# Skylarking/MARL

Hardware: AMD Instinct MI355X
Metric: env_steps_per_sec (higher is better)
Workload: dtype f32 (bf16x6 split products, fp32 accumulate)

## Files before the change

include/marl_hip.h:

```cpp
#ifndef MARL_HIP_H
#define MARL_HIP_H
#include <stddef.h>
#ifdef __cplusplus
extern "C" {
#endif

typedef struct {
  const float* p0; long ld0; int k0;
  const float* p1; long ld1; int k1;
  const int* idx; int nhot; int hot_w;
  int nid;
  const float* m0; long ldm0;
  long rpe0, bs0, off0;
  long rpei, bsi, offi;
  const int* emap0;
} marl_src_t;

typedef struct {
  int groups;
  long gs_x0, gs_x1, gs_w, gs_b, gs_y, gs_m0;
} marl_group_t;

typedef struct {
  const float *fc1_w, *fc1_b;
// ... 33 lines not shown
int marl_agent_unroll_bwd(const marl_agent_weights_t* w, const float* dq, const int* dq_idx,
                          const float* dq_val, const int* dq_idx2, const float* dq_val2, int dq_gdiv, const float* dhs,
                          const float* saved, const float* hs, float* dxp, float* dh0,
                          const marl_agent_grads_t* g, float* ws, size_t ws_bytes,
                          int B, int T, int N, int A, void* stream);

int marl_q_gather(const float* q, const int* idx, const float* avail, float mask_val, float* out,
                  long rows, int A, void* stream);
int marl_q_masked_max(const float* q, const float* avail, float mask_val, float* out_max, int* out_arg,
                      long rows, int A, void* stream);
int marl_q_double_select(const float* q_sel, const float* q_val, const float* avail, float mask_val,
                         float* out_val, int* out_arg, long rows, int A, void* stream);
int marl_q_scatter(float* dq, const int* idx1, const float* g1, const int* idx2, const float* g2,
                   long rows, int A, int gdiv, void* stream);
int marl_vec_add(const float* a, const float* b, float* out, long n, void* stream);
int marl_agent_sum(const float* in, long ld_in, float* out, long ld_out, long rows, int N, int D, void* stream);
int marl_agent_bcast(const float* in, long ld_in, float* out, long ld_out, long rows, int N, int D, int accumulate,
                     void* stream);

int marl_qmix_mix_fwd(const float* hy, long ldh, const float* b2, const float* w22, const float* b22, const float* q,
                      float* q_tot, long rows, int N, int E, void* stream);
int marl_qmix_mix_bwd(const float* hy, long ldh, const float* q, const float* dq_tot, const float* w22, float* dhy,
                      float* db2, float* dq, long rows, int N, int E, void* stream);
int marl_qmix_tail_fwd(const marl_src_t* s, long rows, int S, const float* Wb1, long ldb1, const float* bb1, const float* Wh,
                       long ldwh, const float* bh, float* hy, long ldhy, int c_b1, int c_h, void* stream);

typedef struct {
  const float *w1, *w1_b;
  const float *b1, *b1_b;
  const float *w2, *w2_b;
  const float *h, *h_b;
  const float *b2_w, *b2_b;
} marl_qmix_weights_t;
int marl_qmix_fused_supported(int N, int S, int E);
size_t marl_qmix_fused_workspace(long rows, int N, int S);
int marl_qmix_fused_fwd(const marl_qmix_weights_t* w, const marl_src_t* s, const float* q, float* q_tot,
                        long rows, int N, int S, int E, void* stream);
int marl_qmix_fused_bwd(const marl_qmix_weights_t* w, const marl_src_t* s, const float* q, const float* dq_tot,
                        float* dq, const marl_qmix_weights_t* grads, float* ws, size_t ws_bytes, long rows,
                        int N, int S, int E, void* stream);
int marl_qmix_fused_loss_bwd(const marl_qmix_weights_t* w, const marl_src_t* s, const float* q, const float* q_tot_tgt,
                             const float* r, const float* term, const float* padded, float gamma, float* q_tot,
                             float* dq, const marl_qmix_weights_t* grads, float* loss2, float* ws, size_t ws_bytes,
                             long rows, int N, int S, int E, void* stream);
int marl_qmix_fused_fwd_x6(const marl_qmix_weights_t* w, const marl_src_t* s, const float* q, float* q_tot,
                           long rows, int N, int S, int E, void* stream);
int marl_qmix_fused_bwd_x6(const marl_qmix_weights_t* w, const marl_src_t* s, const float* q, const float* dq_tot,
                           float* dq, const marl_qmix_weights_t* grads, float* ws, size_t ws_bytes, long rows,
                           int N, int S, int E, void* stream);
int marl_qmix_fused_loss_bwd_x6(const marl_qmix_weights_t* w, const marl_src_t* s, const float* q, const float* q_tot_tgt,
                                const float* r, const float* term, const float* padded, float gamma, float* q_tot,
                                float* dq, const marl_qmix_weights_t* grads, float* loss2, float* ws, size_t ws_bytes,
                                long rows, int N, int S, int E, void* stream);

int marl_qmix_wide_supported(int N, int S, int E);
const char* marl_qmix_wide_fwd_kernel(long rows, int N, int S, int flags);
size_t marl_qmix_wide_workspace(long rows, int N, int S, int backward);
int marl_qmix_wide_fwd(const marl_qmix_weights_t* w, const marl_src_t* s, const float* q, float* q_tot, float* ws,
                       size_t ws_bytes, long rows, int N, int S, int E, int flags, void* stream);
int marl_qmix_wide_bwd(const marl_qmix_weights_t* w, const marl_src_t* s, const float* q, const float* dq_tot, float* dq,
                       const marl_qmix_weights_t* grads, float* ws, size_t ws_bytes, long rows, int N, int S, int E,
                       int flags, void* stream);
int marl_qmix_wide_loss_bwd(const marl_qmix_weights_t* w, const marl_src_t* s, const float* q, const float* q_tot_tgt,
                            const float* r, const float* term, const float* padded, float gamma, float* q_tot, float* dq,
                            const marl_qmix_weights_t* grads, float* loss2, float* ws, size_t ws_bytes, long rows,
                            int N, int S, int E, int flags, void* stream);

typedef struct {
  const float *w1, *b1;
  const float *w2, *b2;
  const float *w3, *b3;
  long gs_w1, gs_b1, gs_w2, gs_b2, gs_w3, gs_b3;
} marl_mlp3_weights_t;
int marl_mlp3_supported(const marl_src_t* x, int K1, int H1, int H2, int N3, int groups);
int marl_mlp3_fwd(const marl_mlp3_weights_t* w, const marl_src_t* x, float* Y, long ldy, long gs_y,
                  long M, int K1, int N3, int groups, void* stream);
size_t marl_mlp3_bwd_workspace(long M, int K1, int N3, int groups);
int marl_mlp3_bwd(const marl_mlp3_weights_t* w, const marl_src_t* x, const float* dY, long lddy, long gs_dy,
                  const marl_mlp3_weights_t* grads, float* ws, size_t ws_bytes, long M, int K1, int N3,
                  int groups, void* stream);
size_t marl_mlp3_save_floats(long M, int three, int groups);
int marl_mlp3_needs_kept(const marl_src_t* x, int K1, int N3);
int marl_mlp3_fwd_save(const marl_mlp3_weights_t* w, const marl_src_t* x, float* Y, long ldy, long gs_y,
                       float* hsave, size_t hsave_floats, long M, int K1, int N3, int groups, void* stream);
int marl_mlp3_bwd_saved(const marl_mlp3_weights_t* w, const marl_src_t* x, const float* dY, long lddy, long gs_dy,
                        const marl_mlp3_weights_t* grads, float* ws, size_t ws_bytes, const float* hsave,
                        size_t hsave_floats, long M, int K1, int N3, int groups, void* stream);

int marl_agent_unroll_x6_supported(int B, int T, int N, int O, int A, int last_action, int reuse_network);
int marl_agent_unroll_x6_plain_r6(int B, int T, int N, int O, int A, int last_action, int reuse_network, int cu_budget);
int marl_agent_unroll_fwd_x6(const marl_agent_weights_t* w, const float* obs, long obs_bs, int obs_t0,
                             const int* ufed, long u_bs, int u_t0, const int* ep_len, const int* ep_map,
                             const float* h0, float* q, float* hs, float* h_last, float* saved, int B, int T, int N,
                             int O, int A, int last_action, int reuse_network, int cu_budget, float* gi_out,
                             const float* gi_in, void* stream);

#define MARL_UNROLL_SAVED 1
#define MARL_UNROLL_GI_OUT 2
#define MARL_UNROLL_GI_IN 4
#define MARL_UNROLL_HS 8
#define MARL_UNROLL_OBS_ALIGNED 16
#define MARL_UNROLL_H_ALIGNED 32
#define MARL_UNROLL_F32_PIPE 0
#define MARL_UNROLL_F32_MULTI 1
#define MARL_UNROLL_X6 2
#define MARL_UNROLL_X6_R6 3
#define MARL_UNROLL_IN_ELEMENT 0
#define MARL_UNROLL_IN_VECTOR 1
#define MARL_UNROLL_IN_HALF 2
#define MARL_UNROLL_IN_W2L 3
int marl_agent_unroll_fwd_plan(int x6, int B, int T, int N, int O, int A, int last_action, int reuse_network, int cu_budget,
                               int flags, int* plan);

int marl_agent_unroll_bwd_x6_supported(int B, int T, int N, int A, int sparse_dq);
size_t marl_agent_bwd_x6_workspace(int B, int N, int A);
int marl_agent_unroll_bwd_x6(const marl_agent_weights_t* w, const int* dq_idx, const float* dq_val, const int* dq_idx2,
                             const float* dq_val2, int dq_gdiv, const float* dhs, const float* saved, float* dxp, float* dh0,
                             const marl_agent_grads_t* g, float* ws, size_t ws_bytes, int B, int T, int N, int A, void* stream);

// ... 12 lines not shown
  const float *enc2_w, *enc2_b;
  const float* q0_w; long q0_ld; int q0_s;
  const float *q2_w, *q2_b;
  const float *q4_w, *q4_b;
} marl_qtran_weights_t;
int marl_qtran_supported(int N, int A, int AE);
int marl_qtran_head_fwd(const marl_qtran_weights_t* w, const float* hidden, const int* u, const float* sp, float* out,
                        float* s1, float* e2, float* y1, float* y2, long BT, int N, int A, int AE, void* stream);
int marl_qtran_head_fwd2(const marl_qtran_weights_t* w, const float* hidden, const int* u, const int* u2, const float* sp,
                         float* out, float* out2, float* s1, float* e2, float* y1, float* y2, long BT, int N, int A, int AE,
                         void* stream);
size_t marl_qtran_bwd_workspace(long BT, int AE);
int marl_qtran_head_bwd(const marl_qtran_weights_t* w, const float* hidden, const int* u, const float* d_out,
                        const float* y1, const float* y2, float* dy1, float* dy2, float* de2, float* dhidden,
                        int accumulate, float* d_enc0_w, float* d_enc0_b, float* d_enc2_b, float* ws, size_t ws_bytes,
                        long BT, int N, int A, int AE, void* stream);

int marl_qtran_state_parts_supported(int S);
int marl_qtran_state_parts(const marl_src_t* s, long BT, int S, int nsets, const float* W0, long ldw0, const float* b0, float* sp0,
                           const float* W1, long ldw1, const float* b1, float* sp1, void* stream);
int marl_qtran_wgrad_rows_supported(int S, int AE);
size_t marl_qtran_wgrad_rows_workspace(int S, int AE);
int marl_qtran_wgrad_rows(const marl_src_t* s, const float* s1, const float* e2, const float* y1, const float* y2,
                          const float* d_out, const float* dy1, const float* dy2, const float* de2, float* d_q0_w, long ld_q0,
                          float* d_q0_b, float* d_q2_w, float* d_q2_b, float* d_q4_w, float* d_q4_b, float* d_enc2_w, float* ws,
                          size_t ws_bytes, long BT, int S, int AE, void* stream);
#define MARL_QTRAN_PLAN_FWD 0
#define MARL_QTRAN_PLAN_FWD2 1
#define MARL_QTRAN_PLAN_BWD 2
#define MARL_QTRAN_PLAN_STATE_PARTS 3
#define MARL_QTRAN_PLAN_QMIX_TAIL 4
#define MARL_QTRAN_PLAN_WGRAD_ROWS 5
int marl_qtran_plan(int what, long BT, int N, int A, int AE, int S, int nsets, int* plan);

int marl_qplex_mix_fwd(const float* w_raw, const float* v, const float* q, const float* max_q,
                       const float* key, const float* ag, const float* ac, float* v_tot, float* a_tot,
                       float* lam_out, long rows, int N, int K, int weighted_head, int minus_one,
                       void* stream);
int marl_qplex_mix_bwd(const float* w_raw, const float* q, const float* max_q, const float* key,
                       const float* ag, const float* ac, const float* g, float* dq, float* dw_raw,
                       float* dv, float* dkey, float* dag, float* dac, long rows, int N, int K,
                       int weighted_head, int minus_one, void* stream);

int marl_first_terminated_len(const float* term, long ld, int E, int T, int* out, void* stream);

int marl_replay_gather(const long long* idx, int B, int T, int N, int A, const int* u_src, const float* r_src,
                       const float* term_src, const float* padded_src, const int* length_src, const int* won_src,
                       const float* avail_src, int* o_map, int* u, int* u_act, float* r, float* term, float* padded,
                       int* length, int* won, float* avail_next, float* avail_cur, void* stream);

int marl_td_loss(const float* q_tot, const float* q_tot_tgt, const float* r, const float* term,
                 const float* padded, float gamma, float* dq_tot, float* out2, float* ws, long rows,
                 void* stream);
int marl_qtran_loss(const float* jq, const float* jq_tgt, const float* v, const float* jq_hat,
                    const float* qsum_opt, const float* qsum_nopt, const float* r, const float* term,
                    const float* padded, float gamma, float lam_opt, float lam_nopt, float* d_jq,
                    float* d_v, float* d_qsum_opt, float* d_qsum_nopt, float* out4, float* ws, long rows,
                    void* stream);
size_t marl_loss_workspace(long rows);

int marl_qatten_supported(const marl_src_t* s, int N, int U, int H);
int marl_qatten_plan(long rows, int N, int U, int H, int* plan);
int marl_qatten_mix_fwd(const marl_src_t* s, const float* hy, long ldh, const float* q, float scale, float* q_tot,
                        long rows, int N, int U, int H, void* stream);
int marl_qatten_mix_bwd(const marl_src_t* s, const float* hy, long ldh, const float* q, float scale, const float* dq_tot,
                        float* dq, float* dhy, long lddh, long rows, int N, int U, int H, void* stream);
int marl_qatten_loss_bwd(const marl_src_t* s, const float* hy, long ldh, const float* q, float scale,
                         const float* q_tot_tgt, const float* r, const float* term, const float* padded, float gamma,
                         float* q_tot, float* dq, float* dhy, long lddh, float* dq_tot, float* out2, float* ws, long rows,
                         int N, int U, int H, void* stream);

int marl_lica_supported(int N, int A, int E);
int marl_lica_plan(long rows, int N, int A, int E, int* plan);
int marl_lica_mix_fwd(const float* hy, long ldh, const float* x, const int* u, float* q, long rows, int N, int A, int E,
                      void* stream);
int marl_lica_mix_bwd(const float* hy, long ldh, const float* x, const int* u, const float* dq, float* dhy, long lddh, float* dx,
                      long rows, int N, int A, int E, void* stream);
int marl_lica_loss_bwd(const float* hy, long ldh, const int* u, const float* q_tgt, const float* r, const float* term,
                       const float* padded, float gamma, float* q, float* dhy, long lddh, float* dq_tot, float* out2, float* ws,
                       long rows, int N, int A, int E, void* stream);

int marl_td_lambda_returns(const float* q_next_tot, const float* r, const float* term, const float* padded,
                           float gamma, float lambda, float* ret, int B, int T, void* stream);

int marl_iql_loss_bwd(const float* q, const int* u, const float* q_sel, const float* q_tgt, const float* avail_next,
                      const float* ret, const float* r, const float* term, const float* padded, float gamma, float mask_val,
                      float* dq_val, float* q_taken, float* q_next, float* out2, float* ws, int B, int T, int N, int A,
                      void* stream);
int marl_iql_select(const float* q, const int* u, const float* q_sel, const float* q_tgt, const float* avail_next,
                    const float* padded, float mask_val, float* q_taken, float* q_next_bnt, int B, int T, int N, int A,
                    void* stream);

int marl_policy_probs(const float* logits, const float* avail, float eps, float* pi, long rows, int A, void* stream);
int marl_policy_loss_bwd(const float* logits, const float* avail, const int* u, const float* G, const float* v,
                         const float* padded, float eps, float* dlogits, float* logp, float* out2, float* ws, long rows,
                         int N, int A, void* stream);
int marl_policy_loss_bwd_ex(const float* logits, const float* avail, const int* u, const float* G, const float* v,
                            const float* padded, float eps, float beta, float* dlogits, float* logp, float* ent, float* out3,
                            float* ws, long rows, int N, int A, void* stream);
int marl_policy_sample(const float* logits, const float* avail, long avail_es, const int* alive, float eps,
                       unsigned rseed, int env0, const int* tg, int tg0, int* act_out, long act_es,
                       int E, int N, int A, void* stream);

int marl_ppo_loss_bwd(const float* logits, const float* avail, const int* u, const float* adv, const float* logp_old,
                      const float* padded, float eps, float beta, float clip, float* dlogits, float* logp, float* ent,
                      float* out4, float* ws, long rows, int N, int A, void* stream);
int marl_masked_standardize(const float* x, const float* padded, float* out, float* stats3, float* ws, long rows, void* stream);

int marl_policy_probs_bwd(const float* logits, const float* avail, const float* gpi, const float* q_pi, const float* padded,
                          float eps, float beta, float* dlogits, float* ent, float* out3, float* ws, long rows, int N, int A,
                          void* stream);

int marl_coma_onehot_cols(const float* W, long ldw, int col0, float* Wt, int C, int D, void* stream);
int marl_coma_fc1_fwd(const float* pre_s, const float* Wt, const int* u, float* h1, int B, int T, int N, int A, int D,
                      void* stream);
size_t marl_coma_fc1_bwd_workspace(int B, int T, int N, int A, int D);
int marl_coma_fc1_bwd(const float* dh1, const float* h1, const int* u, float* dpre, float* dsum, float* dW, long lddw,
                      int col0, float* ws, size_t ws_bytes, int B, int T, int N, int A, int D, void* stream);
int marl_coma_q_taken(const float* q, const int* u, float* out, int shift, int B, int T, int N, int A, void* stream);
int marl_coma_loss_bwd(const float* logits, const float* avail, const float* q, const int* u, const float* G,
                       const float* padded, float eps, float beta, float* dlogits, float* dq, float* logp, float* ent,
                       float* adv, float* q_taken, float* out_c2, float* out_a3, float* ws, int B, int T, int N, int A,
                       void* stream);
// ... 187 lines not shown
```

marl_amd/algorithm/common.py:

```python
from __future__ import annotations

import copy
import numbers
import os
import warnings
import weakref

import numpy as np
import torch

from .. import ops, experiments
from ..hostutil import FlatParams, DeviceBatch, AsyncInt, Scratch, require_cuda
from ..network.mixer import x6_mode
from ..rollout import EpisodeBatch

MASK_BIG = -9999999.0
MASK_QTRAN_EVAL = -999999.0
N_STATS = 4


class FlatView:

    def __init__(self, flat, params, start):
        self.params = list(params)
        self.offsets = []
        off = 0
        for p in self.params:
            self.offsets.append(off)
            off += (p.numel() + 3) // 4 * 4
        self.n = off
        self.flat = flat[start:start + self.n]


class LearnerParams(FlatParams):

    def __init__(self, params, device):
        params = list(params)
        super().__init__(params, device, with_grad=False)
        self.gradx = torch.zeros(self.n + N_STATS, dtype=torch.float32, device=device)
        self.grad = self.gradx[:self.n]
        self.stats = self.gradx[self.n:]
        for p, off in zip(self.params, self.offsets):
            p.grad = self.grad[off:off + p.numel()].view(p.shape)

    def zero_grad(self):
        self.gradx.zero_()


class FusedOptimizer:

    def __init__(self, flat: LearnerParams, kind, lr, clip):
        if kind not in ("RMS", "Adam"):
            raise ValueError("optimizer {} not recognised.".format(kind))
        self.flat, self.kind, self.lr, self.clip = flat, kind, lr, clip
        dev = flat.flat.device
        self.s1 = torch.zeros(flat.n, device=dev)
        self.s2 = torch.zeros(flat.n, device=dev) if kind == "Adam" else None
        self.sumsq = torch.zeros(1, device=dev)
        self.t = 0
        self.param_groups = [{"params": flat.params, "lr": lr}]

    def zero_grad(self):
        self.flat.zero_grad()

    def step(self, den=None):
# ... 30 lines not shown
        for k, t in self._target_flats().items():
            sd[k] = t.detach().cpu().clone()
        return sd

    def load_resume_state(self, sd):
        if sd["alg"] != self.args.alg or sd["n_params"] != int(self._flat.n):
            raise ValueError("resume state of a different learner (%s, %d parameters)" % (sd["alg"], sd["n_params"]))
        self._flat.flat.copy_(sd["params"])
        for k, t in self._target_flats().items():
            t.copy_(sd[k])
        self.optimizer.load_state_dict(sd["optimizer"])
        self.sync_replicas()

    def save_resume(self, path):
        torch.save(self.resume_state(), path)

    def load_resume(self, path):
        self.load_resume_state(torch.load(path, map_location="cpu"))


class LossReadback:

    class Handle:
        __slots__ = ("buf", "event", "fn", "_v")

        def __init__(self, buf, event, fn):
            self.buf, self.event, self.fn, self._v = buf, event, fn, None

        def __float__(self):
            if self._v is None:
                self.event.synchronize()
                self._v = float(self.fn(self.buf))
            return self._v

    RING = 8

    def __init__(self, args):
        self.lazy = bool(getattr(args, "lazy_loss", False))
        self.slots, self.k = [], 0

    def read(self, stats, fn):
        if not self.lazy:
            return float(fn(stats.cpu()))
        if len(self.slots) < self.RING:
            self.slots.append(torch.empty(stats.numel(), dtype=stats.dtype).pin_memory())
        buf = self.slots[self.k % self.RING]
        self.k += 1
        buf.copy_(stats, non_blocking=True)
        ev = torch.cuda.Event()
        ev.record()
        return LossReadback.Handle(buf, ev, fn)


def td_lambda_of(args):
    lam = getattr(args, "td_lambda", None)
    if lam is None:
        return None
    if isinstance(lam, bool) or not isinstance(lam, numbers.Real) or not 0.0 <= lam <= 1.0:
        raise ValueError("td_lambda must be None or a number in [0, 1], got %r" % (lam,))
    return float(lam)


class Learner(ResumeMixin):
    _full_len_streak = 0
    n_stats, den_slot = 2, 1
    extra_nets = ()
    launch_ahead = True
    replay_graphs = True

    def _begin(self, mac, args, name):
        self.td_lambda = td_lambda_of(args)
        self._td_dbg = {}
        self.max_episode_len = args.episode_limit
        self.gamma = args.gamma
        self.lr = args.lr
        self.model_dir = args.model_dir + '/' + args.alg + '/' + args.map
        self.args = args
        self.device = require_cuda(name)

        self.eval_net = mac
        self.eval_net.cuda()
        self.target_net = copy.deepcopy(mac)

    def _ready(self, needs_avail):
        args = self.args
        self.optimizer = FusedOptimizer(self._flat, args.optimizer, self.lr, args.grad_norm_clip)
        self._buf = Scratch()
        self.reducer = GradReducer()
        self.pair = PairedUnroll(x6=x6_mode(args))
        self.loss_readback = LossReadback(args)
        self.graphs = GraphedUpdate.from_args(args) if self.replay_graphs else None
        self.needs_avail = needs_avail
        self.last_stats = None
        self.sync_replicas()

    def _update_targets(self):
        self.target_net.agent._flat.flat.copy_(self.eval_net.agent._flat.flat)
        if self.mixer is not None and self.mixer._flat.n:
            self.target_mixer._flat.flat.copy_(self.mixer._flat.flat)

    def _g(self, name, shape, dt=torch.float32):
        return self._buf.get(name, shape, self.device, dt)

    def _td_inputs(self, db, q_next_tot):
        lam = self.td_lambda = td_lambda_of(self.args)
        if lam is None:
            self._td_dbg = {}
            return db.r, self.gamma
        G = self._g("td_ret", (db.B * db.T,))
        ops.td_lambda_returns(q_next_tot, db.r, db.term, db.padded, self.gamma, lam, G, db.B, db.T)
        self._td_dbg = {"td_targets": G}
        return G, 0.0

    def get_max_episode_len(self, batch):
        T = DeviceBatch.first_terminated_len(torch.as_tensor(np.asarray(batch['terminated'])), self.args.episode_limit)
        for key in batch.keys():
            batch[key] = batch[key][:, :T]
        return batch, T

    def _device_batch(self, rec, index, small):
        term = (small if small is not None else rec).term
        if not (term.is_cuda and term.dtype == torch.float32 and term.shape[0] > 0) or self._full_len_streak < 2 \
                or not self.launch_ahead:
            db = DeviceBatch.from_record_auto(rec, self.args, reducer=self.reducer, index=index, small=small)
            full = db.T == min(rec.T, self.args.episode_limit)
            self._full_len_streak = self._full_len_streak + 1 if full else 0
            return db
        db, pending = DeviceBatch.from_record_begin(rec, self.args, reducer=self.reducer, index=index, small=small)
        self.max_episode_len = db.T
        self._forward_backward(db)
        T = pending()
        if T == db.T:
            return None
        self._full_len_streak = 0
        return DeviceBatch.from_record(rec, self.args, T=T, index=index, small=small)

    def train(self, batch, train_step):
        ring = batch.ring if isinstance(batch, EpisodeBatch) else None
        if self.graphs is not None and ring is not None and self.graphs.run(self, ring, batch.index):
            db = None
        elif isinstance(batch, DeviceBatch):
            db = batch
        elif ring is not None:
            prep = self.graphs.prepared if self.graphs is not None else None
            if prep is not None:
                self.graphs.prepared = None
                db = DeviceBatch.from_record(ring, self.args, T=prep[1], index=batch.index, small=prep[0])
            else:
                small = ring.select_small(batch.index, avail_cur=self.needs_avail)
                db = self._device_batch(ring, batch.index, small)
        elif isinstance(batch, EpisodeBatch) and batch.record is not None:
            db = self._device_batch(batch.record, None, None)
        else:
            T = None
            if self.reducer.enabled:
                T = DeviceBatch.first_terminated_len(torch.as_tensor(np.asarray(batch['terminated'])),
                                                     self.args.episode_limit, reducer=self.reducer)
            db = DeviceBatch.from_dict(batch, self.args, self.device, T=T)
        if db is not None:
            self.max_episode_len = db.T
            self._forward_backward(db)
        return self._finish_update(train_step)

    def _loss_fn(self):
        return lambda s: s[0] / s[1]

    def _finish_update(self, train_step):
        self.reducer.allreduce_(self._flat.gradx)
        stats = self._flat.stats
        self.optimizer.step(den=stats[self.den_slot:self.den_slot + 1])
        if train_step > 0 and train_step % self.args.target_update_cycle == 0:
            self._update_targets()
        self.last_stats = stats
        return self.loss_readback.read(stats[:self.n_stats], self._loss_fn())

    def _file_nets(self):
        return (("mixer",) if self.mixer is not None else ()) + self.extra_nets

    def save_models(self, train_step):
        num = str(train_step // self.args.save_cycle)
        if not os.path.exists(self.model_dir):
            os.makedirs(self.model_dir)
        self.eval_net.save_models(self.model_dir + '/' + num + '_rnn_net_params.pkl')
        for name in self._file_nets():
            torch.save({k: v.detach().cpu() for k, v in getattr(self, name).state_dict().items()},
                       self.model_dir + '/' + num + '_' + name + '_net_params.pkl')

    def load_models(self):
        paths = [self.model_dir + '/' + name + '_net_params.pkl' for name in ("rnn",) + self._file_nets()]
        if not os.path.exists(paths[0]):
            raise Exception("No model!")
        self.eval_net.load_models(paths[0])
        for name, path in zip(self._file_nets(), paths[1:]):
            getattr(self, name).load_state_dict(torch.load(path, map_location='cpu'))
        self.sync_replicas()
        print('Successfully load the model: ' + ' and '.join(paths))


def agent_backward(mac, db, which, saved, hs, dq, dhs, buf, dq_idx=None, dq_val=None, dq_idx2=None, dq_val2=None, dq_gdiv=1):
    args = mac.args
    B, T, N, A, O = db.B, db.T, db.N, db.A, db.O
    H = args.rnn_hidden_dim
    M = B * T * N
# ... 86 lines not shown
        with torch.cuda.stream(self.side):
            side()
        main()
        cur.wait_stream(self.side)

    def _step_us(self, rt):
        if self.x6:
            return 1.5 if rt <= 1 else 2.75 if rt <= 2 else 1.74 * rt
        return 3.3 if rt <= 1 else 1.3 + 2.1 * rt

    def chain_split(self, rows, T, obs_dim):
        if not self.chain or not self.applies(rows, T):
            return None
        if self.forced_split is not None:
            return (self.forced_split, 256 - self.forced_split) if self.forced_split > 0 else None
        tiles = (rows + 15) // 16
        cap = 8 if self.x6 else max(1, min(8, 2048 // (4 * max(obs_dim, 4))))
        ceil = lambda a, b: -(-a // b)
        plain = self._step_us(ceil(tiles, 128)) + 0.6 * self._step_us(ceil(tiles, 256))
        best = None
        for cu_a in (128, 144, 160, 176, 192):
            cu_b = 256 - cu_a
            rt_a, rt_b = ceil(tiles, cu_a), ceil(tiles, cu_b)
            if rt_a > cap or rt_b > cap:
                continue
            cost = max(1.6 * self._step_us(rt_a), self._step_us(rt_b))
            if best is None or cost < best[0]:
                best = (cost, cu_a, cu_b)
        if best is None or best[0] > 0.9 * plain:
            return None
        return best[1], best[2]

    def run_chain(self, rows, T, obs_dim, first, cont, second):
        split = self.chain_split(rows, T, obs_dim) if cont is not None else None
        if split is None:
            self.run(rows, T, first, second)
            if cont is not None:
                cont(256)
            return
        cu_a, cu_b = split
        self._fork(lambda: (first(cu_a), cont(cu_a)), lambda: second(cu_b))


class GraphedUpdate:

    WARMUP = 2
    AUTO_MAX_EPISODES = 1536

    def __init__(self, auto=False):
        self.entries = {}
        self.disabled = False
        self.auto = bool(auto)
        self.replays = 0

    @staticmethod
    def from_args(args):
        mode = getattr(args, "hip_graph", None)
        if mode is None or mode == "auto":
            return GraphedUpdate(auto=True)
        return GraphedUpdate() if mode else None

    SCHEDULE_ARGS = ("gemm_mode", "mixer_dtype", "mixer_wgrad_dtype", "double_q", "no_loss_fold", "lazy_loss", "gamma",
                     "two_hyper_layers", "last_action", "reuse_network", "td_lambda")

    @staticmethod
    def _schedule_key(args):
        return (experiments.generation,) + tuple(repr(getattr(args, k, None)) for k in GraphedUpdate.SCHEDULE_ARGS)

    def run(self, learner, ring, index):
        self.prepared = None
        if self.disabled:
            return False
        args = learner.args
        if self.auto and int(index.numel()) > self.AUTO_MAX_EPISODES:
            return False
        if ring.T != args.episode_limit or int(index.numel()) != int(args.batch_size):
            return False
        key = (id(ring), int(index.numel()), ring.T)
        e = self.entries.get(key)
        if e is not None and e["ring"]() is not ring:
            e = None
        dev = ring.obs.device
        if e is None:
            idx = index.to(device=dev, dtype=torch.long).clone()
            small = ring.select_small(idx, avail_cur=getattr(learner, "needs_avail", False))
            db = DeviceBatch.from_record(ring, args, T=min(ring.T, args.episode_limit), index=idx, small=small)
            fused = getattr(small, "avail_next", None) is not None and db.T == ring.T
            e = self.entries[key] = dict(ring=weakref.ref(ring), idx=idx, small=small, db=db, calls=0, graph=None, streak=0,
                                         fused=fused, avail_next=None if fused else db.avail_next.clone(),
                                         u_act=None if fused else db.u_act.clone())
            if not fused:
                db.avail_next, db.u_act = e["avail_next"], e["u_act"]
            e["T"] = db.T
        idx, small, db = e["idx"], e["small"], e["db"]
        idx.copy_(index)
        db.o_map.copy_(idx)
        ring.select_small(idx, out=small)
        if e["graph"] is not None and (e["ws_gen"] != ops.WS.gen or e["sched_key"] != self._schedule_key(args)):
            e["graph"], e["ws_keep"], e["calls"] = None, None, 0
        pending = None
        term = small.term
        if e["graph"] is not None and e["streak"] >= 2 and term.is_cuda and term.dtype == torch.float32 and term.shape[0] > 0:
            out = ops.first_terminated_len(term, args.episode_limit)
            r = learner.reducer
            if r is not None and r.enabled:
                r.dist.all_reduce(out, op=r.dist.ReduceOp.MAX, group=r.group)
            pending = AsyncInt(out)
            T = e["T"]
        else:
            T = DeviceBatch.first_terminated_len(term, args.episode_limit, reducer=learner.reducer)
            if T != e["T"]:
                e["streak"] = 0
                self.prepared = (small, T)
                return False
            e["streak"] += 1
        if not e["fused"]:
            torch.clamp(small.u[:, :T], min=0, out=e["u_act"])
            e["avail_next"].view(small.E, T, small.N, small.A).copy_(small.avail_next[:, :T] if small.avail is None else small.avail[:, 1:T + 1])
        if getattr(small, "avail_cur", None) is None:
            db.__dict__.pop("_avail", None)
# ... 32 lines not shown
```

marl_amd/algorithm/q_learner.py:

```python
from __future__ import annotations

import copy

import numpy as np
import torch

from .. import ops, experiments
from ..hostutil import flatten_module
from ..network.mixer import VDNMixer, QMixMixer, DMAQer, QattenMixer
from .common import MASK_BIG, LearnerParams, FlatView, Learner, agent_backward


class QLearner(Learner):
    def __init__(self, mac, args):
        self._begin(mac, args, "QLearner")
        if args.alg == 'vdn':
            self.mixer = VDNMixer(args)
        elif args.alg == 'qmix':
            self.mixer = QMixMixer(args)
        elif args.alg == 'qplex':
            self.mixer = DMAQer(args)
        elif args.alg == 'qatten':
            self.mixer = QattenMixer(args)
        else:
            raise ValueError("Mixer {} not recognised.".format(args.alg))
        self.target_mixer = copy.deepcopy(self.mixer)
        self.params = list(mac.parameters()) + list(self.mixer.parameters())
        self.cuda()
        self._ready(needs_avail=args.alg == 'qplex')

    def sync_replicas(self):
        o = self.optimizer
        self.reducer.broadcast_(self._flat.flat, self.target_net.agent._flat.flat,
                                self.target_mixer._flat.flat if self.target_mixer._flat.n else None, o.s1, o.s2)

    def cuda(self):
        dev = self.device
        self.mixer.to(dev)
        self.target_mixer.to(dev)
        self.eval_net.agent.to(dev)
        self._flat = LearnerParams(self.params, dev)
        self.eval_net.agent._flat = FlatView(self._flat.flat, self.eval_net.agent.parameters(), 0)
        self.mixer._flat = FlatView(self._flat.flat, self.mixer.parameters(), self.eval_net.agent._flat.n)
        self.eval_net._dev = dev
        self.target_net._dev = dev
        self.target_net.agent.to(dev)
        flatten_module(self.target_net.agent, dev)
        flatten_module(self.target_mixer, dev)

    def _unrolls(self, db, keep_hs=False):
        a, g = self.args, self._g
        B, T, N, A, H = db.B, db.T, db.N, db.A, a.rnn_hidden_dim
        q_evals, saved = g("q_evals", (B, T, N, A)), g("saved", ops.saved_shape(T, B, N))
        h_last, h_scr = g("h_last", (B * N, H)), g("h_scr", (B * N, H))
        q_tgt, q_en = g("q_tgt", (B, T, N, A)), g("q_en", (B, T, N, A))
        hs = hs_en = hs_tgt = None
        if keep_hs:
            hs, hs_tgt = g("hs", (B, T, N, H)), g("hs_tgt", (B, T, N, H))
            hs_en = g("hs_en", (B, T, N, H)) if a.double_q else None
        (oc, oc_bs, oc_t0), (on, on_bs, on_t0) = db.o_cur, db.o_next

        emap = getattr(db, 'o_map', None)
        cont, gi = None, None
        if a.double_q:
            shifted = on is oc and on_bs == oc_bs and on_t0 == oc_t0 + 1
            split = self.pair.chain_split(B * N, T, a.obs_shape)
            if shifted and ((self.eval_net.unroll_x6(B, T, oc) and experiments.get("fwd_xs") != 0) or
                            ops.agent_unroll_reuse_supported(B, T, N, a.obs_shape, A, split[0] if split else 256)):
                gi = g("gi", ops.saved_shape(T, B, N, planes=3))
            cont = lambda cu: self.eval_net.unroll(on, on_bs, on_t0, db.u_fed, db.u_bs, 0, B, T, q_en, hs_en, h_scr, None, h0=h_last,
                                                   ep_len=db.ep_len, ep_map=emap, cu_budget=cu, gi_in=gi)
        self.pair.run_chain(B * N, T, a.obs_shape,
                            lambda cu: self.eval_net.unroll(oc, oc_bs, oc_t0, db.u_fed, db.u_bs, -1, B, T, q_evals, hs, h_last, saved,
                                                            h0=None, ep_len=db.ep_len, ep_map=emap, cu_budget=cu, gi_out=gi),
                            cont,
                            lambda cu: self.target_net.unroll(on, on_bs, on_t0, db.u_fed, db.u_bs, 0, B, T, q_tgt, hs_tgt, None, None,
                                                              h0=None, ep_len=db.ep_len, ep_map=emap, cu_budget=cu))
        return q_evals, q_en, q_tgt, saved, (hs, hs_en, hs_tgt)

    def _select(self, db, q_evals, q_en, q_tgt):
        R, A, g = db.B * db.T * db.N, db.A, self._g
        q_chosen, q_tgt_chosen = g("q_chosen", (R,)), g("q_tgt_chosen", (R,))
        ops.q_gather(q_evals, db.u_act.reshape(-1), q_chosen, R, A)
        cur_max = None
        if self.args.double_q:
            cur_max = g("cur_max", (R,), torch.int32)
            ops.q_double_select(q_en, q_tgt, db.avail_next, MASK_BIG, q_tgt_chosen, cur_max, R, A)
        else:
            ops.q_masked_max(q_tgt, db.avail_next, MASK_BIG, q_tgt_chosen, None, R, A)
        return q_chosen, q_tgt_chosen, cur_max

    def _mix(self, db, q_evals, q_tgt, q_chosen, q_tgt_chosen, cur_max):
        a, g = self.args, self._g
        N, BT, A = db.N, db.B * db.T, db.A
        R = BT * N
        ctx, fold = {}, False
        qc, qtc = q_chosen.view(BT, N), q_tgt_chosen.view(BT, N)
        if a.alg == 'qplex':
            max_q = g("max_q", (R,))
            ops.q_masked_max(q_evals, db.avail, MASK_BIG, max_q, None, R, A)
            v_tot, a_tot = self.mixer.hip_forward(qc, db.s, BT, u_idx=db.u_taken.reshape(-1), max_q=max_q.view(BT, N), ctx=ctx)
            q_tot = g("q_tot", (BT,))
            ops.vec_add(v_tot, a_tot, q_tot, BT)
            if a.double_q:
                tgt_max = g("tgt_max", (R,))
                ops.q_masked_max(q_tgt, db.avail_next, MASK_BIG, tgt_max, None, R, A)
                vt, at = self.target_mixer.hip_forward(qtc, db.s_next, BT, u_idx=cur_max, max_q=tgt_max.view(BT, N), tag="t")
                q_tot_tgt = g("q_tot_tgt", (BT,))
                ops.vec_add(vt, at, q_tot_tgt, BT)
            else:
                q_tot_tgt, _ = self.target_mixer.hip_forward(qtc, db.s_next, BT, tag="t")
        else:
            fold = a.alg in ('qmix', 'qatten') and getattr(self.mixer, "loss_backward_fused", None) is not None and \
                self.mixer.loss_backward_fused(db.s) and not getattr(a, "no_loss_fold", False)
            q_tot = g("q_tot", (BT,)) if fold else self.mixer.hip_forward(qc, db.s, BT, ctx=ctx)
            q_tot_tgt = self.target_mixer.hip_forward(qtc, db.s_next, BT, tag="t")
        return q_tot, q_tot_tgt, ctx, fold

    def _loss_backward(self, db, q_chosen, q_tot, q_tot_tgt, ctx, fold):
        BT = db.B * db.T
        r, gamma = self._td_inputs(db, q_tot_tgt)
        if fold:
            return self.mixer.hip_loss_backward(q_chosen.view(BT, db.N), db.s, BT, q_tot_tgt, r, db.term, db.padded, gamma,
                                                self._flat.stats[:2], q_tot=q_tot)
        dq_tot = self._g("dq_tot", (BT,))
        ops.td_loss(q_tot, q_tot_tgt, r, db.term, db.padded, gamma, dq_tot, self._flat.stats[:2], BT)
        return self.mixer.hip_backward(ctx, dq_tot, BT)

    def _forward_backward(self, db):
        q_evals, q_en, q_tgt, saved, _ = self._unrolls(db)
        q_chosen, q_tgt_chosen, cur_max = self._select(db, q_evals, q_en, q_tgt)
        q_tot, q_tot_tgt, ctx, fold = self._mix(db, q_evals, q_tgt, q_chosen, q_tgt_chosen, cur_max)
        self._flat.zero_grad()
        dq_chosen = self._loss_backward(db, q_chosen, q_tot, q_tot_tgt, ctx, fold)
        agent_backward(self.eval_net, db, "cur", saved, None, None, None, self._buf,
                       dq_idx=db.u_act.reshape(-1), dq_val=dq_chosen.reshape(-1).contiguous())
        self._dbg = dict(q_evals=q_evals, q_targets=q_tgt, q_tot=q_tot, q_tot_target=q_tot_tgt, **self._td_dbg)

    def get_q_and_q_tot_table(self):
        one = {'o': np.ones((1, 1, 2, 1)), 's': np.ones((1, 1, 1)), 'o_next': np.ones((1, 1, 2, 1)),
               'u_onehot': np.zeros((1, 1, 2, 3)), 'avail_u': np.ones((1, 1, 2, 3))}
        self.eval_net.init_hidden(1)
        q_values, _ = self.eval_net.get_current_q_values(one, 1)
        qv = q_values.cpu()
        q_table_i, q_table_j = qv[0, 0, 0].numpy(), qv[0, 0, 1].numpy()
        q_tot_table = np.zeros((3, 3))
        s = torch.ones(1, 1, 1)
        for i in range(3):
            for j in range(3):
                chosen = torch.stack((qv[:, :, 0, i], qv[:, :, 1, j]), dim=1).view(1, 1, 2)
                if self.args.alg == 'qplex':
                    v_tot = self.mixer(chosen, s, is_v=True)
                    onehot = torch.zeros(1, 1, 2, 3)
                    onehot[0, 0, 0, i] = 1
                    onehot[0, 0, 1, j] = 1
                    a_tot = self.mixer(chosen, s, actions=onehot, max_q_i=qv.max(dim=3)[0], is_v=False)
                    q_tot_table[i, j] = float(v_tot.item() + a_tot.item())
                else:
                    q_tot_table[i, j] = self.mixer(chosen, s).item()
        return q_tot_table, q_table_i, q_table_j
```

marl_amd/common/replaybuffer.py:

```python
from __future__ import annotations

import threading

import numpy as np
import torch

from ..env.synthetic_smac import EpisodeRecord
from ..rollout import EpisodeBatch
from ..hostutil import h2d_async


class ReplayBuffer:
    def __init__(self, args):
        self.args = args
        self.n_actions = args.n_actions
        self.n_agents = args.n_agents
        self.state_shape = args.state_shape
        self.obs_shape = args.obs_shape
        self.size = args.buffer_size
        self.episode_limit = args.episode_limit
        self.current_idx = 0
        self.current_size = 0
        self.buffers = None
        self.record = None
# ... 16 lines not shown

    def next_slot_record(self, E, T, N, O, S, A, device):
        if self.buffers is not None:
            return None
        with self.lock:
            i0 = self._peek_contiguous(E)
            if i0 is None:
                return None
            if self.record is None:
                self.record = EpisodeRecord(self.size, T, N, O, S, A, device)
            r = self.record
            if (r.T, r.N, r.O, r.S, r.A) != (T, N, O, S, A):
                return None
            view = r.slice(i0, i0 + E)
            view.sink_slot = i0
            return view

    def store_episode(self, episode_batch):
        rec = getattr(episode_batch, "record", None)
        batch_size = rec.E if rec is not None else episode_batch['o'].shape[0]
        with self.lock:
            idxs = self._get_storage_idx(inc=batch_size)
            if rec is not None and self.buffers is None:
                if self.record is None:
                    self.record = EpisodeRecord(self.size, rec.T, rec.N, rec.O, rec.S, rec.A, rec.obs.device)
                first = int(np.atleast_1d(idxs)[0])
                if rec.obs.data_ptr() == self.record.obs[first].data_ptr() and getattr(rec, "sink_slot", -1) == first:
                    return
                if getattr(rec, "sink_slot", None) is not None:
                    rec = rec.clone()
                idx_t = torch.as_tensor(np.atleast_1d(idxs), dtype=torch.long, device=rec.obs.device)
                rec.copy_into(self.record, idx_t)
                return
            if self.record is not None:
                raise ValueError("this ReplayBuffer holds device records; store EpisodeBatch objects")
            if self.buffers is None:
                self._alloc_host()
            src = episode_batch.numpy() if isinstance(episode_batch, EpisodeBatch) else episode_batch
            for k in self.buffers:
                v = src[k]
                self.buffers[k][idxs] = v.cpu().numpy() if isinstance(v, torch.Tensor) else v

    def sample(self, batch_size, exclude=None):
        if exclude is not None and exclude[0] < self.current_size:
            lo, cnt = int(exclude[0]), int(min(exclude[1], self.current_size - exclude[0]))
            if self.current_size - cnt <= 0:
                raise ValueError("every stored episode is being overwritten: nothing to sample")
            idx = np.random.randint(0, self.current_size - cnt, batch_size)
            idx = np.where(idx >= lo, idx + cnt, idx)
        else:
            idx = np.random.randint(0, self.current_size, batch_size)
        if self.record is not None:
            idx_t = h2d_async(idx, self.record.obs.device, torch.long)
            return EpisodeBatch(ring=self.record, index=idx_t)
        return {k: self.buffers[k][idx] for k in self.buffers}

    def _get_storage_idx(self, inc=None):
        inc = inc or 1
        if self.current_idx + inc <= self.size:
            idx = np.arange(self.current_idx, self.current_idx + inc)
            self.current_idx += inc
        elif self.current_idx < self.size:
            overflow = inc - (self.size - self.current_idx)
            idx = np.concatenate([np.arange(self.current_idx, self.size), np.arange(0, overflow)])
            self.current_idx = overflow
        else:
            idx = np.arange(0, inc)
            self.current_idx = inc
        self.current_size = min(self.size, self.current_size + inc)
        if inc == 1:
            idx = idx[0]
        return idx
```

marl_amd/csrc/mixers.hip:

```cpp
#include "common.h"
#include "sums.h"
#include "row_tile.h"
#include "../../include/marl_hip.h"

namespace {
namespace rt = row_tile;

constexpr int TPB = 256;
static_assert(TPB == SUMS_TPB, "the loss kernels launch sums.h's workgroup size");
inline int nblk(long n, int cap = 65535 * 16) {
  long b = (n + TPB - 1) / TPB;
  if (b > cap) b = cap;
  if (b < 1) b = 1;
  return (int)b;
}

__global__ void q_gather_kernel(const float* q, const int* idx, const float* avail, float mask_val, float* out,
                                long rows, int A) {
  for (long r = (long)blockIdx.x * TPB + threadIdx.x; r < rows; r += (long)gridDim.x * TPB) {
    const int a = idx[r];
    float v = 0.f;
    if (a >= 0) v = (avail && avail[r * A + a] == 0.f) ? mask_val : q[r * A + a];
    out[r] = v;
  }
// ... 318 lines not shown
    tile_in(ags, ag + r0 * KN, nr * KN, (long)QR * KN);
    tile_in(acs, ac + r0 * KN, nr * KN, (long)QR * KN);
    tile_in(keys, key + r0 * K, nr * K, (long)QR * K);
    for (int e = threadIdx.x; e < nr * N; e += TPB) {
      const int rl = e / N;
      const long gi = r0 * N + e;
      const float gr = g[r0 + rl];
      const float wr = w_raw[gi];
      const float w = fabsf(wr) + 1e-10f;
      const float qi = q[gi];
      dq[gi] = weighted ? gr * w : gr;
      dw_raw[gi] = weighted ? gr * qi * (wr > 0.f ? 1.f : (wr < 0.f ? -1.f : 0.f)) : 0.f;
      dv[gi] = weighted ? gr : 0.f;
      const float mi = max_q[gi];
      float adv;
      {
#pragma clang fp contract(off)
        adv = weighted ? (w * qi - w * mi) : (qi - mi);
      }
      dls[e] = gr * adv;
    }
    __syncthreads();
    for (int e = threadIdx.x; e < nr * K; e += TPB) {
      const int rl = e / K;
      const float kr = keys[e];
      const float kk = fabsf(kr) + 1e-10f;
      const float sg = kr > 0.f ? 1.f : (kr < 0.f ? -1.f : 0.f);
      float dk = 0.f;
      for (int i = 0; i < N; ++i) {
        const float dlam = dls[rl * N + i];
        const float sa = sigmoidf_(ags[e * N + i]);
        const float sc = sigmoidf_(acs[e * N + i]);
        dk += dlam * sa * sc * sg;
        ags[e * N + i] = dlam * kk * sc * sa * (1.f - sa);
        acs[e * N + i] = dlam * kk * sa * sc * (1.f - sc);
      }
      keys[e] = dk;
    }
    __syncthreads();
    tile_out(dag + r0 * KN, ags, nr * KN);
    tile_out(dac + r0 * KN, acs, nr * KN);
    tile_out(dkey + r0 * K, keys, nr * K);
    __syncthreads();
  }
}

inline int qplex_tile_rows(int N, int K, const void* a, const void* b, const void* c) {
  if (!aligned16(a) || !aligned16(b) || !aligned16(c)) return 0;
  for (int qr = 128; qr >= 32; qr >>= 1)
    if ((size_t)qr * (2 * K * N + K + 2 * N) * 4 <= 64 * 1024) return qr;
  return 0;
}

__global__ void td_loss_kernel(const float* q_tot, const float* q_tgt, const float* r, const float* term,
                               const float* padded, float gamma, float* dq_tot, float* ws, long rows) {
  float acc[2] = {0.f, 0.f};
  for (long i = (long)blockIdx.x * TPB + threadIdx.x; i < rows; i += (long)gridDim.x * TPB) {
    const float mask = 1.f - padded[i];
    const float target = r[i] + gamma * q_tgt[i] * (1.f - term[i]);
    const float td = target - q_tot[i];
    const float mtd = mask * td;
    acc[0] += mtd * mtd;
    acc[1] += mask;
    dq_tot[i] = -2.f * mask * mtd;
  }
  block_partials<2>(acc, ws);
}

__global__ void qtran_loss_kernel(const float* jq, const float* jq_tgt, const float* v, const float* jq_hat,
                                  const float* qs_opt, const float* qs_nopt, const float* r, const float* term,
                                  const float* padded, float gamma, float lam_opt, float lam_nopt, float* d_jq,
                                  float* d_v, float* d_qs_opt, float* d_qs_nopt, float* ws, long rows) {
  float acc[4] = {0.f, 0.f, 0.f, 0.f};
  for (long i = (long)blockIdx.x * TPB + threadIdx.x; i < rows; i += (long)gridDim.x * TPB) {
    const float mask = 1.f - padded[i];
    const float y = r[i] + gamma * jq_tgt[i] * (1.f - term[i]);
    const float td = (jq[i] - y) * mask;
    const float opt = (qs_opt[i] - jq_hat[i] + v[i]) * mask;
    float nraw = qs_nopt[i] - jq[i] + v[i];
    nraw = nraw < 0.f ? nraw : 0.f;
    const float nopt = nraw * mask;
    acc[0] += td * td; acc[1] += opt * opt; acc[2] += nopt * nopt; acc[3] += mask;
    d_jq[i] = 2.f * mask * td;
    const float go = lam_opt * 2.f * mask * opt, gn = lam_nopt * 2.f * mask * nopt;
    d_v[i] = go + gn;
    d_qs_opt[i] = go;
    d_qs_nopt[i] = gn;
  }
  block_partials<4>(acc, ws);
}

}

extern "C" int marl_q_gather(const float* q, const int* idx, const float* avail, float mask_val, float* out,
                             long rows, int A, void* stream) {
  if (rows <= 0) return 0;
  hipLaunchKernelGGL(q_gather_kernel, dim3(nblk(rows)), dim3(TPB), 0, (hipStream_t)stream, q, idx, avail, mask_val,
                     out, rows, A);
  MARL_CHECK_LAUNCH();
  return 0;
}

extern "C" int marl_q_masked_max(const float* q, const float* avail, float mask_val, float* out_max, int* out_arg,
                                 long rows, int A, void* stream) {
  if (rows <= 0) return 0;
  const rt::Plan pl = rt::plan(rows, A, 2, 64 * 1024, 2048, {q, avail});
  if (pl.tiled && pl.vec && rows >= 4096) {
    hipLaunchKernelGGL(q_masked_max_tiled_kernel, dim3((unsigned)pl.blocks), dim3(256), pl.lds_bytes, (hipStream_t)stream, q, avail,
                       mask_val, out_max, out_arg, rows, A);
    MARL_CHECK_LAUNCH();
    return 0;
  }
  hipLaunchKernelGGL(q_masked_max_kernel, dim3(nblk(rows)), dim3(TPB), 0, (hipStream_t)stream, q, avail, mask_val,
                     out_max, out_arg, rows, A);
  MARL_CHECK_LAUNCH();
  return 0;
}
// ... 163 lines not shown
  for (int i = blockIdx.y * 1024 + threadIdx.x; i < TNA && i < (blockIdx.y + 1) * 1024; i += TPB) ao[i] = av[i];
  if (a.avail_cur) {
    const int NA = a.N * a.A;
    const long live = (long)a.length_src[e] * NA;
    const float* ac = av - NA;
    float* co = a.avail_cur + (long)b * TNA;
    for (int i = blockIdx.y * 1024 + threadIdx.x; i < TNA && i < (blockIdx.y + 1) * 1024; i += TPB) co[i] = i < live ? ac[i] : 0.f;
  }
  if (blockIdx.y != 0) return;
  const int TN = a.T * a.N;
  for (int i = threadIdx.x; i < TN; i += TPB) {
    const int v = a.u_src[e * TN + i];
    a.u[(long)b * TN + i] = v;
    a.u_act[(long)b * TN + i] = v < 0 ? 0 : v;
  }
  for (int i = threadIdx.x; i < a.T; i += TPB) {
    a.r[(long)b * a.T + i] = a.r_src[e * a.T + i];
    a.term[(long)b * a.T + i] = a.term_src[e * a.T + i];
    a.padded[(long)b * a.T + i] = a.padded_src[e * a.T + i];
  }
  if (threadIdx.x == 0) {
    a.o_map[b] = (int)e;
    a.length[b] = a.length_src[e];
    a.won[b] = a.won_src[e];
  }
}
}

extern "C" int marl_replay_gather(const long long* idx, int B, int T, int N, int A, const int* u_src, const float* r_src,
                                  const float* term_src, const float* padded_src, const int* length_src,
                                  const int* won_src, const float* avail_src, int* o_map, int* u, int* u_act, float* r,
                                  float* term, float* padded, int* length, int* won, float* avail_next, float* avail_cur,
                                  void* stream) {
  if (B <= 0 || T <= 0) return 0;
  GatherArgs a;
  a.idx = idx; a.u_src = u_src; a.length_src = length_src; a.won_src = won_src;
  a.r_src = r_src; a.term_src = term_src; a.padded_src = padded_src; a.avail_src = avail_src;
  a.o_map = o_map; a.u = u; a.u_act = u_act; a.length = length; a.won = won;
  a.r = r; a.term = term; a.padded = padded; a.avail_next = avail_next; a.avail_cur = avail_cur;
  a.B = B; a.T = T; a.N = N; a.A = A;
  const int chunks = (T * N * A + 1023) / 1024;
  hipLaunchKernelGGL(replay_gather_kernel, dim3((unsigned)B, (unsigned)(chunks > 0 ? chunks : 1)), dim3(TPB), 0, (hipStream_t)stream, a);
  MARL_CHECK_LAUNCH();
  return 0;
}

extern "C" size_t marl_loss_workspace(long rows) { return (size_t)rt::PARTIAL_ROWS * 4 * sizeof(float); }

extern "C" int marl_td_loss(const float* q_tot, const float* q_tot_tgt, const float* r, const float* term,
                            const float* padded, float gamma, float* dq_tot, float* out2, float* ws, long rows,
                            void* stream) {
  if (rows <= 0) return 0;
  const int nb = rt::partial_blocks(rows);
  hipLaunchKernelGGL(td_loss_kernel, dim3(nb), dim3(TPB), 0, (hipStream_t)stream, q_tot, q_tot_tgt, r, term, padded,
                     gamma, dq_tot, ws, rows);
  MARL_CHECK_LAUNCH();
  hipLaunchKernelGGL(finish_sums_kernel, dim3(1), dim3(TPB), 0, (hipStream_t)stream, (const float*)ws, nb, 2, out2);
  MARL_CHECK_LAUNCH();
  return 0;
}

extern "C" int marl_qtran_loss(const float* jq, const float* jq_tgt, const float* v, const float* jq_hat,
                               const float* qsum_opt, const float* qsum_nopt, const float* r, const float* term,
                               const float* padded, float gamma, float lam_opt, float lam_nopt, float* d_jq,
                               float* d_v, float* d_qsum_opt, float* d_qsum_nopt, float* out4, float* ws, long rows,
                               void* stream) {
  if (rows <= 0) return 0;
  const int nb = rt::partial_blocks(rows);
  hipLaunchKernelGGL(qtran_loss_kernel, dim3(nb), dim3(TPB), 0, (hipStream_t)stream, jq, jq_tgt, v, jq_hat, qsum_opt,
                     qsum_nopt, r, term, padded, gamma, lam_opt, lam_nopt, d_jq, d_v, d_qsum_opt, d_qsum_nopt, ws,
                     rows);
  MARL_CHECK_LAUNCH();
  hipLaunchKernelGGL(finish_sums_kernel, dim3(1), dim3(TPB), 0, (hipStream_t)stream, (const float*)ws, nb, 4, out4);
  MARL_CHECK_LAUNCH();
  return 0;
}
```

marl_amd/csrc/qatten.hip:

```cpp
#include "common.h"
#include "sums.h"
#include "row_tile.h"
#include "../../include/marl_hip.h"

#pragma clang fp contract(off)

namespace {
namespace rt = row_tile;

constexpr int TPB = SUMS_TPB;
constexpr int MAXN = 16, MAXU = 64, MAXH = 8;
constexpr int MAX_TILE = 64;
constexpr size_t LDS_CAP = 76 * 1024;

enum { MODE_FWD = 0, MODE_BWD = 1, MODE_LOSS = 2 };

struct Tile { int TR, SP, HP; size_t lds; };
inline Tile tile_of(int N, int U, int H) {
  Tile t;
  t.SP = (N * U) | 1;
  t.HP = (H * U + H + 1) | 1;
  const size_t row = (size_t)(2 + t.SP + t.HP + N + H * N + H + N + 1) * sizeof(float);
  long tr = (long)(LDS_CAP / row);
  if (tr > MAX_TILE) tr = MAX_TILE;
  if (tr > TPB / H) tr = TPB / H;
  t.TR = (int)(tr < 1 ? 1 : tr);
  t.lds = row * t.TR;
  return t;
}

struct QaArgs {
  ConcatSrc s;
  const float* hy; long ldh;
  const float* q;
  float scale;
  const float* g_in;
  const float *q_tgt, *r, *term, *padded;
  float gamma;
  float* q_tot;
  float* dq;
  float* dhy; long lddh;
  float* dq_tot;
  float* ws;
  long rows;
  int N, U, H, TR, SP, HP;
};

struct Chunk { int lo, cnt; bool vec; };
__device__ __forceinline__ Chunk chunk_of(const float* g, int n, int j) {
  int head = (int)((4 - ((reinterpret_cast<uintptr_t>(g) >> 2) & 3)) & 3);
  head = head < n ? head : n;
  Chunk c;
  c.lo = j ? head + 4 * (j - 1) : 0;
  c.cnt = j ? (n - c.lo < 4 ? n - c.lo : 4) : head;
  if (c.cnt < 0) c.cnt = 0;
  c.vec = j && c.cnt == 4;
  return c;
}
__device__ __forceinline__ int chunks_of(int n) { return 1 + (n + 3) / 4; }

template <class F>
__device__ __forceinline__ void tile_in(float* lds, int pitch, const float* base, F off_of, int n, int nr) {
  const int CH = chunks_of(n), items = nr * CH;
  for (int it0 = threadIdx.x; it0 < items; it0 += 4 * TPB) {
    f32x4 v[4];
    Chunk c[4];
    int at[4];
#pragma unroll
    for (int u = 0; u < 4; ++u) {
      const int it = it0 + u * TPB;
      c[u].cnt = 0; c[u].lo = 0; c[u].vec = false; at[u] = 0;
      v[u] = (f32x4){0.f, 0.f, 0.f, 0.f};
      if (it < items) {
        const int rl = it / CH, j = it - rl * CH;
        const long off = off_of(rl);
        const float* g = base + (off < 0 ? 0 : off);
        c[u] = chunk_of(g, n, j);
        at[u] = rl * pitch + c[u].lo;
        if (off >= 0) {
          if (c[u].vec) v[u] = *reinterpret_cast<const f32x4*>(g + c[u].lo);
          else
#pragma unroll
            for (int e = 0; e < 4; ++e) if (e < c[u].cnt) v[u][e] = g[c[u].lo + e];
        }
      }
    }
#pragma unroll
    for (int u = 0; u < 4; ++u)
#pragma unroll
      for (int e = 0; e < 4; ++e) if (e < c[u].cnt) lds[at[u] + e] = v[u][e];
  }
}
__device__ __forceinline__ void tile_out(float* g0, long ld, const float* lds, int pitch, int n, int nr) {
  const int CH = chunks_of(n), items = nr * CH;
  for (int it = threadIdx.x; it < items; it += TPB) {
    const int rl = it / CH, j = it - rl * CH;
    float* g = g0 + rl * ld;
    const Chunk c = chunk_of(g, n, j);
    const float* d = lds + rl * pitch + c.lo;
    if (c.vec) *reinterpret_cast<f32x4*>(g + c.lo) = (f32x4){d[0], d[1], d[2], d[3]};
    else
      for (int e = 0; e < c.cnt; ++e) g[c.lo + e] = d[e];
  }
}

__device__ __forceinline__ float head_fwd(const float* p, const float* u, const float* q, float scale, int N, int U, float (&lam)[MAXN]) {
#pragma unroll
  for (int i = 0; i < MAXN; ++i) lam[i] = 0.f;
#pragma unroll 4
  for (int k = 0; k < U; ++k) {
    const float pk = p[k];
#pragma unroll
    for (int i = 0; i < MAXN; ++i)
      if (i < N) lam[i] += pk * u[i * U + k];
  }
  float mx = 0.f;
#pragma unroll
  for (int i = 0; i < MAXN; ++i)
    if (i < N) {
      lam[i] = scale * lam[i];
      mx = (i == 0 || lam[i] > mx) ? lam[i] : mx;
    }
  float sum = 0.f;
#pragma unroll
  for (int i = 0; i < MAXN; ++i)
    if (i < N) { lam[i] = expf(lam[i] - mx); sum += lam[i]; }
  float y = 0.f;
#pragma unroll
  for (int i = 0; i < MAXN; ++i)
    if (i < N) { lam[i] = lam[i] / sum; y += lam[i] * q[i]; }
  return y;
}

__device__ __forceinline__ float head_bwd(float* p, const float* u, const float* q, float scale, int N, int U, float g, float w, float y,
                                          float (&lam)[MAXN]) {
  const float ga = g * fabsf(w);
#pragma unroll
  for (int i = 0; i < MAXN; ++i)
    if (i < N) lam[i] = ga * lam[i] * (q[i] - y);
#pragma unroll 4
  for (int k = 0; k < U; ++k) {
    float d = 0.f;
#pragma unroll
    for (int i = 0; i < MAXN; ++i)
      if (i < N) d += lam[i] * u[i * U + k];
    p[k] = scale * d;
  }
  return g * y * (w > 0.f ? 1.f : (w < 0.f ? -1.f : 0.f));
}

template <int MODE>
__global__ __launch_bounds__(TPB) void qatten_kernel(QaArgs a) {
  extern __shared__ __attribute__((aligned(16))) float qa_smem[];
  const int N = a.N, U = a.U, H = a.H, TR = a.TR, SP = a.SP, HP = a.HP;
  const int NU = N * U, HU = H * U;
  long* Ro = reinterpret_cast<long*>(qa_smem);
  float* Ss = qa_smem + 2 * TR;
  float* Hs = Ss + (size_t)TR * SP;
  float* Qs = Hs + (size_t)TR * HP;
  float* WL = Qs + TR * N;
  float* Ys = WL + TR * H * N;
  float* Dq = Ys + TR * H;
  float* Gs = Dq + TR * N;
  const int tid = threadIdx.x;
  float acc[2] = {0.f, 0.f};
  for (long r0 = (long)blockIdx.x * TR; r0 < a.rows; r0 += (long)gridDim.x * TR) {
    const int nr = (int)(a.rows - r0 < TR ? a.rows - r0 : TR);
    for (int rl = tid; rl < nr; rl += TPB) {
      const ConcatRow cr = concat_row(a.s, r0 + rl);
      Ro[rl] = cr.ok0 ? cr.r0 * a.s.ld0 : -1;
    }
    __syncthreads();
    tile_in(Ss, SP, a.s.p0, [&](int rl) { return Ro[rl]; }, NU, nr);
    tile_in(Hs, HP, a.hy + r0 * a.ldh, [&](int rl) { return rl * a.ldh; }, HU + H + 1, nr);
    for (int e = tid; e < nr * N; e += TPB) Qs[e] = a.q[r0 * N + e];
    __syncthreads();
    const bool act = tid < nr * H;
    const int rl = tid / H, h = tid - rl * H;
    float lam[MAXN];
    float y = 0.f, w = 0.f;
    if (act) {
      y = head_fwd(Hs + rl * HP + h * U, Ss + rl * SP, Qs + rl * N, a.scale, N, U, lam);
      w = Hs[rl * HP + HU + h];
      Ys[tid] = y;
      if (MODE != MODE_FWD) {
        const float aw = fabsf(w);
#pragma unroll
        for (int i = 0; i < MAXN; ++i)
          if (i < N) WL[tid * N + i] = aw * lam[i];
      }
    }
    __syncthreads();
    if (tid < nr) {
      const long r = r0 + tid;
      float g = 0.f;
      if (MODE != MODE_BWD) {
        float qt = 0.f;
        for (int hh = 0; hh < H; ++hh) qt += fabsf(Hs[tid * HP + HU + hh]) * Ys[tid * H + hh];
        qt += Hs[tid * HP + HU + H];
        if (a.q_tot) a.q_tot[r] = qt;
        if (MODE == MODE_LOSS) {
#pragma clang fp contract(fast)
          const float mask = 1.f - a.padded[r];
          const float target = a.r[r] + a.gamma * a.q_tgt[r] * (1.f - a.term[r]);
          const float td = target - qt;
          const float mtd = mask * td;
          acc[0] += mtd * mtd;
          acc[1] += mask;
          g = -2.f * mask * mtd;
          a.dq_tot[r] = g;
        }
      } else {
        g = a.g_in[r];
      }
      if (MODE != MODE_FWD) Gs[tid] = g;
    }
    if (MODE != MODE_FWD) {
      __syncthreads();
      if (act) Hs[rl * HP + HU + h] = head_bwd(Hs + rl * HP + h * U, Ss + rl * SP, Qs + rl * N, a.scale, N, U, Gs[rl], w, y, lam);
      for (int e = tid; e < nr * N; e += TPB) {
        const int row = e / N, i = e - row * N;
        float ai = 0.f;
        for (int hh = 0; hh < H; ++hh) ai += WL[(row * H + hh) * N + i];
        Dq[e] = Gs[row] * ai;
      }
      __syncthreads();
      tile_out(a.dhy + r0 * a.lddh, a.lddh, Hs, HP, HU + H, nr);
      for (int e = tid; e < nr * N; e += TPB) a.dq[r0 * N + e] = Dq[e];
    }
    __syncthreads();
  }
  if (MODE == MODE_LOSS) block_partials<2>(acc, a.ws);
}

inline bool shape_ok(int N, int U, int H) { return N >= 1 && N <= MAXN && U >= 1 && U <= MAXU && H >= 1 && H <= MAXH; }
inline bool src_ok(const marl_src_t* s, int N, int U) {
  return s && s->p0 && s->k0 >= N * U && s->ld0 >= N * U && !s->k1 && !s->nhot && !s->nid && !s->m0 && s->rpe0 >= 0 &&
         (!s->emap0 || s->rpe0 > 0) && (reinterpret_cast<uintptr_t>(s->p0) & 3) == 0;
}
inline ConcatSrc state_src(const marl_src_t* s) {
  ConcatSrc c = {};
  c.p0 = s->p0; c.ld0 = s->ld0; c.k0 = s->k0;
  c.rpe0 = s->rpe0; c.bs0 = s->bs0; c.off0 = s->off0;
  c.fd0 = make_fastdiv((unsigned)(s->rpe0 > 0 ? s->rpe0 : 1));
  c.fdi = make_fastdiv(1); c.fdn = make_fastdiv(1);
  c.emap0 = s->emap0;
  return c;
}
inline int grid_of(long rows, int TR) {
  const long t = (rows + TR - 1) / TR;
  return (int)(t > rt::PARTIAL_ROWS ? rt::PARTIAL_ROWS : t);
}

template <int MODE>
int launch(QaArgs& a, const marl_src_t* s, hipStream_t stream) {
  if (!shape_ok(a.N, a.U, a.H) || !src_ok(s, a.N, a.U) || a.rows >= (1L << 31) || !a.hy || !a.q || a.ldh < a.H * a.U + a.H + 1)
    return (int)hipErrorInvalidValue;
  if (MODE != MODE_FWD && (!a.dq || !a.dhy || a.lddh < a.H * a.U + a.H)) return (int)hipErrorInvalidValue;
  const Tile t = tile_of(a.N, a.U, a.H);
  a.s = state_src(s);
  a.TR = t.TR; a.SP = t.SP; a.HP = t.HP;
  const void* fn = (const void*)qatten_kernel<MODE>;
  hipError_t e = hipFuncSetAttribute(fn, hipFuncAttributeMaxDynamicSharedMemorySize, (int)t.lds);
  if (e != hipSuccess) return (int)e;
  void* kargs[] = {(void*)&a};
  e = hipLaunchKernel(fn, dim3((unsigned)grid_of(a.rows, t.TR)), dim3(TPB), kargs, t.lds, stream);
  if (e != hipSuccess) return (int)e;
  MARL_CHECK_LAUNCH();
  return 0;
}

}

extern "C" int marl_qatten_supported(const marl_src_t* s, int N, int U, int H) { return shape_ok(N, U, H) && src_ok(s, N, U) ? 1 : 0; }

extern "C" int marl_qatten_plan(long rows, int N, int U, int H, int* plan) {
  if (!shape_ok(N, U, H) || rows >= (1L << 31)) return (int)hipErrorInvalidValue;
  for (int i = 0; i < 4; ++i) plan[i] = 0;
  if (rows <= 0) return 0;
  const Tile t = tile_of(N, U, H);
  plan[0] = t.TR;
  plan[1] = grid_of(rows, t.TR);
  plan[2] = (int)t.lds;
  const long tiles = (rows + t.TR - 1) / t.TR;
  plan[3] = (int)((tiles + plan[1] - 1) / plan[1]);
  return 0;
}

extern "C" int marl_qatten_mix_fwd(const marl_src_t* s, const float* hy, long ldh, const float* q, float scale, float* q_tot,
                                   long rows, int N, int U, int H, void* stream) {
  if (rows <= 0) return 0;
  if (!q_tot) return (int)hipErrorInvalidValue;
  QaArgs a = {};
  a.hy = hy; a.ldh = ldh; a.q = q; a.scale = scale; a.q_tot = q_tot; a.rows = rows; a.N = N; a.U = U; a.H = H;
  return launch<MODE_FWD>(a, s, (hipStream_t)stream);
}

extern "C" int marl_qatten_mix_bwd(const marl_src_t* s, const float* hy, long ldh, const float* q, float scale, const float* dq_tot,
                                   float* dq, float* dhy, long lddh, long rows, int N, int U, int H, void* stream) {
  if (rows <= 0) return 0;
  if (!dq_tot) return (int)hipErrorInvalidValue;
  QaArgs a = {};
  a.hy = hy; a.ldh = ldh; a.q = q; a.scale = scale; a.g_in = dq_tot; a.dq = dq; a.dhy = dhy; a.lddh = lddh;
  a.rows = rows; a.N = N; a.U = U; a.H = H;
  return launch<MODE_BWD>(a, s, (hipStream_t)stream);
}

extern "C" int marl_qatten_loss_bwd(const marl_src_t* s, const float* hy, long ldh, const float* q, float scale,
                                    const float* q_tot_tgt, const float* r, const float* term, const float* padded, float gamma,
                                    float* q_tot, float* dq, float* dhy, long lddh, float* dq_tot, float* out2, float* ws, long rows,
                                    int N, int U, int H, void* stream) {
  if (rows <= 0) return 0;
  if (!q_tot_tgt || !r || !term || !padded || !dq_tot || !out2 || !ws) return (int)hipErrorInvalidValue;
  QaArgs a = {};
  a.hy = hy; a.ldh = ldh; a.q = q; a.scale = scale; a.q_tgt = q_tot_tgt; a.r = r; a.term = term; a.padded = padded; a.gamma = gamma;
  a.q_tot = q_tot; a.dq = dq; a.dhy = dhy; a.lddh = lddh; a.dq_tot = dq_tot; a.ws = ws;
  a.rows = rows; a.N = N; a.U = U; a.H = H;
  const int rc = launch<MODE_LOSS>(a, s, (hipStream_t)stream);
  if (rc) return rc;
  hipLaunchKernelGGL(finish_sums_kernel, dim3(1), dim3(TPB), 0, (hipStream_t)stream, (const float*)ws, grid_of(rows, a.TR), 2, out2);
  MARL_CHECK_LAUNCH();
  return 0;
}
```

marl_amd/csrc/qmix_fused.hip:

```cpp
#include "x6.h"
#include "../../include/marl_hip.h"

namespace {

constexpr int E = 32;
constexpr int KCQ = 8;
constexpr int SS = 128 + 4;
constexpr int NAG = 5;
constexpr int PP = 136;

struct QmixArgs {
  const float *W[4], *Bv[4];
  const float *wb2, *bb2;
  ConcatSrc s;
  const float* q;
  const float* g;
  float* q_tot;
  float* dq;
  float* ws;
  const float *lr, *lterm, *lpadded, *lq_tgt;
  float gamma;
  long rows;
  int N, S, C;
};

__host__ __device__ inline long qmix_slab_floats(int C, int S) { return (long)C * (S + 1) + (E + 1) + 2; }

template <int CTRL>
__device__ __forceinline__ float dpp(float v) {
  return __builtin_bit_cast(float, __builtin_amdgcn_update_dpp(0, __builtin_bit_cast(int, v), CTRL, 0xf, 0xf, true));
}
constexpr int DPP_XOR1 = 0xB1, DPP_XOR2 = 0x4E;
constexpr int DPP_HALF_MIRROR = 0x141, DPP_MIRROR = 0x140;
constexpr int DPP_ROR4 = 0x124, DPP_ROR8 = 0x128;
template <int EW>
__device__ __forceinline__ float group_sum(float v) {
  if (EW == 4) v += dpp<DPP_ROR4>(v);
  v += dpp<DPP_ROR8>(v);
  return v;
}
template <int EW>
__device__ __forceinline__ float e_sum(float v) {
  v += dpp<DPP_XOR1>(v);
  v += dpp<DPP_XOR2>(v);
  if (EW == 8) v += dpp<DPP_HALF_MIRROR>(v);
  return v;
}
__device__ __forceinline__ float row_sum(float v) {
  v += dpp<DPP_XOR1>(v);
  v += dpp<DPP_XOR2>(v);
  v += dpp<DPP_HALF_MIRROR>(v);
  v += dpp<DPP_MIRROR>(v);
  return v;
}
__device__ __forceinline__ float sign_clamp(float x, float lo) { return __builtin_amdgcn_fmed3f(x * 0x1p126f, lo, 1.0f); }

template <bool BWD, int NW, bool LOSS = false, bool X6 = false>
__global__ __launch_bounds__(64 * NW, 2) void qmix_fused_kernel(QmixArgs a) {
  static_assert(!LOSS || BWD, "the loss is folded into the backward kernel");
  static_assert(!X6 || NW == 8, "the split variant runs eight waves (two column tiles per wave: 96 registers of pre-split weights)");
  constexpr int QNT = 64 * NW, EW = 32 / NW, GPT = 16 / EW, TPW = 8 / GPT, LT = TPW - 1;
  constexpr int SRAW = X6 ? 2 * 3 * 16 * PP * 2 : 2 * 16 * SS * 4;
  __shared__ __attribute__((aligned(16))) char Sraw[SRAW];
  float (*Ss)[16 * SS] = reinterpret_cast<float (*)[16 * SS]>(Sraw);
  short* const Sp = reinterpret_cast<short*>(Sraw);
  constexpr int PLN = 16 * PP, PBUF = 3 * PLN;
  constexpr int KR = (X6 && BWD) ? (LOSS ? 2 : 3) : 4;
  constexpr int KL = 4 - KR;
  __shared__ __attribute__((aligned(16))) i32x4 WL[KL ? NW * TPW * KL * 3 * 64 : 1];
  __shared__ __attribute__((aligned(16))) float Qt2[2][8][16];
  __shared__ __attribute__((aligned(16))) float QT[NW][16];
  __shared__ __attribute__((aligned(16))) float DQP[NW][NAG][16];
  __shared__ __attribute__((aligned(16))) float Gs2[2][16];
  __shared__ __attribute__((aligned(16))) float Ls2[2][4][16];
  const int tid = threadIdx.x, lane = tid & 63, wave = tid >> 6;
  const int q4 = lane >> 4, m = lane & 15;
  const int el = m & (EW - 1), gl = m / EW, e = EW * wave + el;
  const int N = a.N, S = a.S, C = a.C, NE = N * E;
  const bool ones = S < 128;

  f32x4 wq[X6 ? 1 : TPW][X6 ? 1 : KCQ];
  F3 wq6[X6 ? TPW : 1][X6 ? KR : 1];
  float bias[TPW];
  int grp[TPW];
#pragma unroll
  for (int c = 0; c < TPW; ++c) {
    const int g = GPT * c + gl;
    grp[c] = g;
    const float *Wp = nullptr, *Bp = nullptr;
    if (g < NAG) { if (g < N) { Wp = a.W[0] + (long)(g * E + e) * S; Bp = a.Bv[0] + g * E + e; } }
    else { Wp = a.W[g - NAG + 1] + (long)e * S; Bp = a.Bv[g - NAG + 1] + e; }
    bias[c] = Bp ? *Bp : 0.f;
    if (X6) {
#pragma unroll
      for (int kc = 0; kc < 4; ++kc) {
        float v[8];
#pragma unroll
        for (int jj = 0; jj < 8; ++jj) {
          const int kk = 32 * kc + 8 * q4 + jj;
          v[jj] = (Wp && kk < S) ? Wp[kk] : 0.f;
        }
        const F3 f = split8((f32x4){v[0], v[1], v[2], v[3]}, (f32x4){v[4], v[5], v[6], v[7]});
        if (kc < KR) wq6[c][kc < KR ? kc : 0] = f;
        else { i32x4* wl = WL + (((wave * TPW + c) * (KL ? KL : 1) + (kc - KR)) * 3) * 64 + lane; wl[0] = f.h; wl[64] = f.m; wl[128] = f.l; }
      }
    } else {
#pragma unroll
      for (int kc = 0; kc < KCQ; ++kc)
#pragma unroll
        for (int i = 0; i < 4; ++i) {
          const int kk = 16 * kc + 4 * q4 + i;
          wq[c][kc][i] = (Wp && kk < S) ? Wp[kk] : 0.f;
// ... 41 lines not shown
  const FastDiv fd = a.s.fd0;
  const int* emap = a.s.emap0;
  const float* sp0 = a.s.p0 + (fc4 < S ? fc4 : 0);
  const long ld = a.s.ld0, blk = (long)a.s.bs0 * a.s.ld0;
  auto map_one = [&](int tile, int i, int& pe, int& pw) {
    unsigned row = (unsigned)tile * 16u + (unsigned)(fr + (QNT / 32) * i);
    row = row < last_row ? row : last_row;
    const unsigned ep = rpe ? fastdiv(row, fd) : 0u;
    pw = (int)(row - ep * rpe) + roff;
    pe = (int)ep;
    if (emap) pe = emap[ep];
  };
  auto map_issue = [&](int tile) {
    map_one(tile, 0, pe0, pw0);
    if (NPF > 1) map_one(tile, 1, pe1, pw1);
  };
  auto fetch_one = [&](int pe, int pw) {
    f32x4 v = *reinterpret_cast<const f32x4*>(sp0 + ((long)pe * blk + (long)pw * ld));
    if (BWD) {
#pragma unroll
      for (int j = 0; j < 4; ++j) v[j] = (ones_lane && j == ones_j) ? 1.f : v[j];
    }
    return v;
  };
  auto fetch = [&](int) {
    pf[0] = fetch_one(pe0, pw0);
    if (NPF > 1) pf[NPF - 1] = fetch_one(pe1, pw1);
  };
  auto stash = [&](int buf) {
#pragma unroll
    for (int i = 0; i < NPF; ++i) {
      if (X6) {
        const F3h f = split4(pf[i]);
        short* p = Sp + buf * PBUF + (fr + (QNT / 32) * i) * PP + fc4;
        *reinterpret_cast<i32x2*>(p) = f.h;
        *reinterpret_cast<i32x2*>(p + PLN) = f.m;
        *reinterpret_cast<i32x2*>(p + 2 * PLN) = f.l;
      } else *reinterpret_cast<f32x4*>(&Ss[buf][(fr + (QNT / 32) * i) * SS + fc4]) = pf[i];
    }
  };
  float pq = 0.f, pg = 0.f, pl[4] = {0.f, 0.f, 0.f, 0.f};
  const int qr = tid / N, qn = tid - qr * N;
  auto fetch_qg = [&](int tile) {
    pq = 0.f; pg = 0.f;
    if (tid < 16 * N) {
      const int row = tile * 16 + qr;
      if (row < nrows) pq = a.q[(unsigned)(row * N + qn)];
    }
    if (BWD && tid >= 192 && tid < 208) {
      const int row = tile * 16 + (tid - 192);
      if (LOSS) {
        pl[0] = pl[1] = pl[3] = 0.f; pl[2] = 1.f;
        if (row < nrows) { pl[0] = a.lr[row]; pl[1] = a.lterm[row]; pl[2] = a.lpadded[row]; pl[3] = a.lq_tgt[row]; }
      } else if (row < nrows) pg = a.g[row];
    }
  };
  auto flush_dq = [&](int prow0) {
    if (tid < 16 * N) {
      float v = 0.f;
#pragma unroll
      for (int w = 0; w < NW; ++w) v += DQP[w][qn][qr];
      if (prow0 + qr < nrows) a.dq[(unsigned)((prow0 + qr) * N + qn)] = v;
    }
  };
  int tile = blockIdx.x;
  if (tile < tiles) {
    map_issue(tile); fetch(tile); fetch_qg(tile);
    if (tile + (int)gridDim.x < tiles) map_issue(tile + gridDim.x);
    stash(0);
  }
  int buf = 0;
  int prow0 = -1;
  ST_DECL(8);
  __syncthreads();
  for (; tile < tiles; tile += gridDim.x, buf ^= 1) {
    const int row0 = tile * 16;
    if (tid < 16 * N) Qt2[buf][qn][qr] = pq;
    if (BWD && tid >= 192 && tid < 208) {
      if (LOSS) {
#pragma unroll
        for (int k = 0; k < 4; ++k) Ls2[buf][k][tid - 192] = pl[k];
      } else Gs2[buf][tid - 192] = pg;
    }
    const int nt = tile + gridDim.x;
    if (nt < tiles) {
      fetch(nt); fetch_qg(nt);
      if (nt + (int)gridDim.x < tiles) map_issue(nt + gridDim.x);
    }
    ST_MARK(0);
    WG_BARRIER();
    ST_MARK(1);
    if (BWD && prow0 >= 0) flush_dq(prow0);
    f32x4 acc[TPW];
#pragma unroll
    for (int c = 0; c < TPW; ++c) acc[c] = (f32x4){bias[c], bias[c], bias[c], bias[c]};
    if (X6) {
      f32x4 accb[TPW];
#pragma unroll
      for (int c = 0; c < TPW; ++c) accb[c] = (f32x4){0.f, 0.f, 0.f, 0.f};
      const short* sp = Sp + buf * PBUF + m * PP + 8 * q4;
#pragma unroll
      for (int kc = 0; kc < 4; ++kc) {
        F3 xa;
        xa.h = *reinterpret_cast<const i32x4*>(sp + 32 * kc);
        xa.m = *reinterpret_cast<const i32x4*>(sp + PLN + 32 * kc);
        xa.l = *reinterpret_cast<const i32x4*>(sp + 2 * PLN + 32 * kc);
        F3 wk[TPW];
#pragma unroll
        for (int c = 0; c < TPW; ++c) {
          if (kc < KR) wk[c] = wq6[c][kc < KR ? kc : 0];
          else { const i32x4* wl = WL + (((wave * TPW + c) * (KL ? KL : 1) + (kc - KR)) * 3) * 64 + lane; wk[c].h = wl[0]; wk[c].m = wl[64]; wk[c].l = wl[128]; }
        }
#define OP(p_, q_) _Pragma("unroll") for (int c = 0; c < TPW; ++c) { if (kc & 1) accb[c] = mm(xa.p_, wk[c].q_, accb[c]); else acc[c] = mm(xa.p_, wk[c].q_, acc[c]); }
        OP(m, m) OP(h, l) OP(l, h) OP(h, m) OP(m, h) OP(h, h)
#undef OP
      }
#pragma unroll
      for (int c = 0; c < TPW; ++c) acc[c] += accb[c];
    } else {
      const float* sr = &Ss[buf][m * SS + 4 * q4];
#pragma unroll
      for (int kc = 0; kc < KCQ; ++kc) {
        const f32x4 a4 = *reinterpret_cast<const f32x4*>(sr + 16 * kc);
#pragma unroll
        for (int i = 0; i < 4; ++i)
#pragma unroll
          for (int c = 0; c < TPW; ++c) acc[c] = mfma16(a4[i], wq[c][kc][i], acc[c]);
      }
    }
    ST_MARK(2);
    __builtin_amdgcn_sched_barrier(0);
    f32x4 qv[TPW];
    f32x4 p = {0.f, 0.f, 0.f, 0.f};
#pragma unroll
    for (int c = 0; c <= MT; ++c) {
      qv[c] = *reinterpret_cast<const f32x4*>(&Qt2[buf][grp[c]][4 * q4]);
#pragma unroll
      for (int i = 0; i < 4; ++i) {
        const float av = acc[c][i];
        const float x = c < MT ? fabsf(av) : __builtin_bit_cast(float, __builtin_bit_cast(unsigned, av) & absmask);
        p[i] = c == 0 ? x * qv[c][i] : fmaf(x, qv[c][i], p[i]);
      }
    }
    f32x4 ex, hid, t4;
#pragma unroll
    for (int i = 0; i < 4; ++i) {
      p[i] = group_sum<EW>(p[i]);
      ex[i] = __expf(p[i]);
      hid[i] = p[i] > 0.f ? p[i] : ex[i] - 1.f;
      const float z = is6 ? fabsf(acc[LT][i]) : fmaxf(acc[LT][i], 0.f);
      t4[i] = row_sum(z * (is6 ? hid[i] : cw));
    }
    if (m == 0) *reinterpret_cast<f32x4*>(&QT[wave][4 * q4]) = t4;
    ST_MARK(3);
    WG_BARRIER();
    ST_MARK(4);
    if (!BWD) {
      if (tid < 16) {
        float tot = 0.f;
#pragma unroll
        for (int w = 0; w < NW; ++w) tot += QT[w][tid];
        if (row0 + tid < nrows) a.q_tot[row0 + tid] = tot + bb2;
      }
      ST_MARK(5);
    } else {
      f32x4 qt = *reinterpret_cast<const f32x4*>(&QT[0][4 * q4]);
#pragma unroll
      for (int w = 1; w < NW; ++w) qt += *reinterpret_cast<const f32x4*>(&QT[w][4 * q4]);
      f32x4 gr;
      if (LOSS) {
        const f32x4 lr = *reinterpret_cast<const f32x4*>(&Ls2[buf][0][4 * q4]);
        const f32x4 lt = *reinterpret_cast<const f32x4*>(&Ls2[buf][1][4 * q4]);
        const f32x4 lp = *reinterpret_cast<const f32x4*>(&Ls2[buf][2][4 * q4]);
        const f32x4 lq = *reinterpret_cast<const f32x4*>(&Ls2[buf][3][4 * q4]);
#pragma unroll
        for (int i = 0; i < 4; ++i) {
          qt[i] += bb2;
          const float mask = 1.f - lp[i];
          const float target = lr[i] + a.gamma * lq[i] * (1.f - lt[i]);
          const float mtd = mask * (target - qt[i]);
          gr[i] = -2.f * mask * mtd;
          acc_ln += mtd * mtd; acc_lm += mask;
        }
        if (a.q_tot && wave == 0 && m == 0) {
          if (row0 + 16 <= nrows) *reinterpret_cast<f32x4*>(&a.q_tot[row0 + 4 * q4]) = qt;
          else {
#pragma unroll
            for (int i = 0; i < 4; ++i) if (row0 + 4 * q4 + i < nrows) a.q_tot[row0 + 4 * q4 + i] = qt[i];
          }
        }
      } else gr = *reinterpret_cast<const f32x4*>(&Gs2[buf][4 * q4]);
      f32x4 dpre, dhy[TPW];
#pragma unroll
      for (int i = 0; i < 4; ++i) {
        const float w2 = group_sum<EW>(is6 ? fabsf(acc[LT][i]) : 0.f);
        dpre[i] = gr[i] * w2 * (p[i] > 0.f ? 1.f : ex[i]);
        acc_wb2 += gr[i] * fmaxf(acc[LT][i], 0.f);
        acc_bb2 += gr[i];
      }
#pragma unroll
      for (int c = 0; c < TPW; ++c) {
        const bool lo_all = GPT * c + GPT - 1 <= NAG, hi_all = GPT * c > NAG;
#pragma unroll
        for (int i = 0; i < 4; ++i) {
          float x, y;
          if (lo_all) { x = qv[c][i]; y = dpre[i]; }
          else if (hi_all) { x = gr[i]; y = is6 ? hid[i] : wb2e; }
          else {
            const bool lo = grp[c] <= NAG;
            x = lo ? qv[c][i] : gr[i];
            y = lo ? dpre[i] : (is6 ? hid[i] : wb2e);
          }
          dhy[c][i] = (x * y) * sign_clamp(acc[c][i], lo_c[c]);
        }
        if (!ones) sbW[c] += dhy[c][0] + dhy[c][1] + dhy[c][2] + dhy[c][3];
        if (GPT * c < NAG) {
          f32x4 d4;
#pragma unroll
          for (int i = 0; i < 4; ++i) d4[i] = e_sum<EW>(fabsf(acc[c][i]) * dpre[i]);
          if (el == 0 && grp[c] < N) *reinterpret_cast<f32x4*>(&DQP[wave][grp[c]][4 * q4]) = d4;
        }
      }
      ST_MARK(5);
      __builtin_amdgcn_sched_barrier(0);
      if (X6) {
        typedef __attribute__((address_space(3))) s16x4 lds_s16x4;
        F3h dA[TPW];
#pragma unroll
        for (int c = 0; c < TPW; ++c) dA[c] = split4(dhy[c]);
        const short* tb = Sp + buf * PBUF + (4 * q4 + (m >> 2)) * PP + 4 * (m & 3);
#pragma unroll
        for (int kc = 0; kc < KCQ; ++kc) {
          F3h sb;
          sb.h = __builtin_bit_cast(i32x2, __builtin_amdgcn_ds_read_tr16_b64_v4i16((lds_s16x4*)(tb + 16 * kc)));
          sb.m = __builtin_bit_cast(i32x2, __builtin_amdgcn_ds_read_tr16_b64_v4i16((lds_s16x4*)(tb + PLN + 16 * kc)));
// ... 113 lines not shown
  c.idx = nullptr; c.nhot = 0; c.hot_w = 0; c.nid = 0; c.m0 = nullptr; c.ldm0 = 0;
  c.rpe0 = s->rpe0; c.bs0 = s->bs0; c.off0 = s->off0; c.rpei = 0; c.bsi = 0; c.offi = 0;
  c.fd0 = make_fastdiv((unsigned)(s->rpe0 > 0 ? s->rpe0 : 1));
  c.fdi = make_fastdiv(1); c.fdn = make_fastdiv(1);
  c.emap0 = s->emap0;
  return c;
}

inline int fill(QmixArgs& a, const marl_qmix_weights_t* w, const marl_src_t* s, const float* q, long rows, int N, int S) {
  a.W[0] = w->w1; a.Bv[0] = w->w1_b; a.W[1] = w->b1; a.Bv[1] = w->b1_b; a.W[2] = w->w2; a.Bv[2] = w->w2_b;
  a.W[3] = w->h; a.Bv[3] = w->h_b; a.wb2 = w->b2_w; a.bb2 = w->b2_b;
  a.s = state_src(s);
  if (a.s.k0 != S || s->k1 || s->nhot || s->nid || s->m0 || (a.s.ld0 % 4) || ((uintptr_t)a.s.p0 & 15)) return 1;
  a.q = q; a.rows = rows; a.N = N; a.S = S; a.C = N * E + 3 * E;
  return 0;
}

inline unsigned grid_for(long rows, int per_cu = 1) {
  long tiles = (rows + 15) / 16;
  return (unsigned)(tiles < 256 * per_cu ? tiles : 256 * per_cu);
}

}

extern "C" int marl_qmix_fused_supported(int N, int S, int Eq) { return supported(N, S, Eq) ? 1 : 0; }

extern "C" size_t marl_qmix_fused_workspace(long rows, int N, int S) {
  return (size_t)grid_for(rows) * qmix_slab_floats(N * E + 3 * E, S) * sizeof(float);
}

static int qmix_fwd_impl(const marl_qmix_weights_t* w, const marl_src_t* s, const float* q, float* q_tot,
                         long rows, int N, int S, int Eq, bool x6, void* stream) {
  if (rows <= 0) return 0;
  if (!supported(N, S, Eq)) return (int)hipErrorInvalidValue;
  QmixArgs a;
  if (fill(a, w, s, q, rows, N, S)) return (int)hipErrorInvalidValue;
  a.g = nullptr; a.q_tot = q_tot; a.dq = nullptr; a.ws = nullptr;
  a.lr = a.lterm = a.lpadded = a.lq_tgt = nullptr; a.gamma = 0.f;
  if (x6) hipLaunchKernelGGL((qmix_fused_kernel<false, 8, false, true>), dim3(grid_for(rows, 1)), dim3(512), 0, (hipStream_t)stream, a);
  else hipLaunchKernelGGL((qmix_fused_kernel<false, 4>), dim3(grid_for(rows, 2)), dim3(256), 0, (hipStream_t)stream, a);
  MARL_CHECK_LAUNCH();
  return 0;
}
extern "C" int marl_qmix_fused_fwd(const marl_qmix_weights_t* w, const marl_src_t* s, const float* q, float* q_tot,
                                   long rows, int N, int S, int Eq, void* stream) {
  return qmix_fwd_impl(w, s, q, q_tot, rows, N, S, Eq, false, stream);
}
extern "C" int marl_qmix_fused_fwd_x6(const marl_qmix_weights_t* w, const marl_src_t* s, const float* q, float* q_tot,
                                      long rows, int N, int S, int Eq, void* stream) {
  return qmix_fwd_impl(w, s, q, q_tot, rows, N, S, Eq, true, stream);
}

static int qmix_bwd_launch(QmixArgs& a, const marl_qmix_weights_t* grads, float* loss2, float* ws, long rows, int N, int S,
                           bool loss, bool x6, hipStream_t st) {
  const unsigned nwg = grid_for(rows);
  if (x6) {
    if (loss) hipLaunchKernelGGL((qmix_fused_kernel<true, 8, true, true>), dim3(nwg), dim3(512), 0, st, a);
    else hipLaunchKernelGGL((qmix_fused_kernel<true, 8, false, true>), dim3(nwg), dim3(512), 0, st, a);
  } else if (loss) hipLaunchKernelGGL((qmix_fused_kernel<true, 8, true>), dim3(nwg), dim3(512), 0, st, a);
  else hipLaunchKernelGGL((qmix_fused_kernel<true, 8, false>), dim3(nwg), dim3(512), 0, st, a);
  MARL_CHECK_LAUNCH();
  QmixRedArgs r;
  r.ws = ws; r.nwg = (int)nwg; r.N = N; r.S = S; r.C = a.C; r.loss2 = loss2;
  r.dW[0] = const_cast<float*>(grads->w1); r.dB[0] = const_cast<float*>(grads->w1_b);
  r.dW[1] = const_cast<float*>(grads->b1); r.dB[1] = const_cast<float*>(grads->b1_b);
  r.dW[2] = const_cast<float*>(grads->w2); r.dB[2] = const_cast<float*>(grads->w2_b);
  r.dW[3] = const_cast<float*>(grads->h); r.dB[3] = const_cast<float*>(grads->h_b);
  r.dwb2 = const_cast<float*>(grads->b2_w); r.dbb2 = const_cast<float*>(grads->b2_b);
  const long slab = qmix_slab_floats(a.C, S);
  hipLaunchKernelGGL(qmix_fused_reduce_kernel, dim3((unsigned)((slab + 63) / 64)), dim3(64 * RSG), 0, st, r);
  MARL_CHECK_LAUNCH();
  return 0;
}

static int qmix_bwd_impl(const marl_qmix_weights_t* w, const marl_src_t* s, const float* q, const float* dq_tot, float* dq,
                         const marl_qmix_weights_t* grads, float* ws, size_t ws_bytes, long rows, int N, int S, int Eq, bool x6,
                         void* stream) {
  if (rows <= 0) return 0;
  if (!supported(N, S, Eq)) return (int)hipErrorInvalidValue;
  if (ws_bytes < marl_qmix_fused_workspace(rows, N, S)) return (int)hipErrorInvalidValue;
  QmixArgs a;
  if (fill(a, w, s, q, rows, N, S)) return (int)hipErrorInvalidValue;
  a.g = dq_tot; a.q_tot = nullptr; a.dq = dq; a.ws = ws;
  a.lr = a.lterm = a.lpadded = a.lq_tgt = nullptr; a.gamma = 0.f;
  return qmix_bwd_launch(a, grads, nullptr, ws, rows, N, S, false, x6, (hipStream_t)stream);
}
extern "C" int marl_qmix_fused_bwd(const marl_qmix_weights_t* w, const marl_src_t* s, const float* q,
                                   const float* dq_tot, float* dq, const marl_qmix_weights_t* grads, float* ws,
                                   size_t ws_bytes, long rows, int N, int S, int Eq, void* stream) {
  return qmix_bwd_impl(w, s, q, dq_tot, dq, grads, ws, ws_bytes, rows, N, S, Eq, false, stream);
}
extern "C" int marl_qmix_fused_bwd_x6(const marl_qmix_weights_t* w, const marl_src_t* s, const float* q,
                                      const float* dq_tot, float* dq, const marl_qmix_weights_t* grads, float* ws,
                                      size_t ws_bytes, long rows, int N, int S, int Eq, void* stream) {
  return qmix_bwd_impl(w, s, q, dq_tot, dq, grads, ws, ws_bytes, rows, N, S, Eq, true, stream);
}

static int qmix_loss_bwd_impl(const marl_qmix_weights_t* w, const marl_src_t* s, const float* q,
                              const float* q_tot_tgt, const float* r, const float* term, const float* padded,
                              float gamma, float* q_tot, float* dq, const marl_qmix_weights_t* grads,
                              float* loss2, float* ws, size_t ws_bytes, long rows, int N, int S, int Eq, bool x6,
                              void* stream) {
  if (rows <= 0) return 0;
  if (!supported(N, S, Eq) || !q_tot_tgt || !r || !term || !padded || !loss2) return (int)hipErrorInvalidValue;
  if (reinterpret_cast<uintptr_t>(q_tot) & 15) return (int)hipErrorInvalidValue;
  if (ws_bytes < marl_qmix_fused_workspace(rows, N, S)) return (int)hipErrorInvalidValue;
  QmixArgs a;
  if (fill(a, w, s, q, rows, N, S)) return (int)hipErrorInvalidValue;
  a.g = nullptr; a.q_tot = q_tot; a.dq = dq; a.ws = ws;
  a.lr = r; a.lterm = term; a.lpadded = padded; a.lq_tgt = q_tot_tgt; a.gamma = gamma;
  return qmix_bwd_launch(a, grads, loss2, ws, rows, N, S, true, x6, (hipStream_t)stream);
}
extern "C" int marl_qmix_fused_loss_bwd(const marl_qmix_weights_t* w, const marl_src_t* s, const float* q,
                                        const float* q_tot_tgt, const float* r, const float* term, const float* padded,
                                        float gamma, float* q_tot, float* dq, const marl_qmix_weights_t* grads,
                                        float* loss2, float* ws, size_t ws_bytes, long rows, int N, int S, int Eq,
                                        void* stream) {
  return qmix_loss_bwd_impl(w, s, q, q_tot_tgt, r, term, padded, gamma, q_tot, dq, grads, loss2, ws, ws_bytes, rows, N, S, Eq, false, stream);
}
extern "C" int marl_qmix_fused_loss_bwd_x6(const marl_qmix_weights_t* w, const marl_src_t* s, const float* q,
                                           const float* q_tot_tgt, const float* r, const float* term, const float* padded,
                                           float gamma, float* q_tot, float* dq, const marl_qmix_weights_t* grads,
                                           float* loss2, float* ws, size_t ws_bytes, long rows, int N, int S, int Eq,
                                           void* stream) {
  return qmix_loss_bwd_impl(w, s, q, q_tot_tgt, r, term, padded, gamma, q_tot, dq, grads, loss2, ws, ws_bytes, rows, N, S, Eq, true, stream);
}
```

marl_amd/csrc/qmix_wide.hip:

```cpp
#include "common.h"
#include <cstdlib>
#include "../../include/marl_hip.h"

namespace {

constexpr int E = 32;
constexpr int NW = 8;

typedef __bf16 bf16x8_t __attribute__((ext_vector_type(8)));

struct WideArgs {
  const float* Wp;
  const float* Bc;
  const float *wb2, *bb2;
  ConcatSrc s;
  const float* q;
  const float* g;
  float* q_tot;
  float* dq;
  float* dhy;
  float* slab;
  const float *lr, *lterm, *lpadded, *lq_tgt;
  float gamma;
  long rows;
  int N, S, C, NCT, KC;
};

struct PackArgs {
  const float* W[4]; const float* Bv[4];
  float* Wp; float* Bc;
  int N, S, C, NCT, KC, bf;
};

__device__ __forceinline__ void seg_of(int col, int NE, int& seg, int& r) {
  if (col < NE) { seg = 0; r = col; }
  else if (col < NE + E) { seg = 1; r = col - NE; }
  else if (col < NE + 2 * E) { seg = 2; r = col - NE - E; }
  else { seg = 3; r = col - NE - 2 * E; }
}

__global__ __launch_bounds__(256) void qmix_pack_kernel(PackArgs a) {
  const int NE = a.N * E;
  const long total = (long)a.NCT * a.KC * 64;
  for (long e = (long)blockIdx.x * 256 + threadIdx.x; e < total; e += (long)gridDim.x * 256) {
    const int l = (int)(e & 63);
    const long tc = e >> 6;
    const int ct = (int)(tc / a.KC), kc = (int)(tc - (long)ct * a.KC);
    const int col = 16 * ct + (l & 15), qq = l >> 4;
    int seg = 0, r = 0;
    const bool okc = col < a.C;
    if (okc) seg_of(col, NE, seg, r);
    const float* Wr = okc ? a.W[seg] + (long)r * a.S : nullptr;
    if (a.bf) {
      bf16x8_t v;
#pragma unroll
      for (int j = 0; j < 8; ++j) {
        const int k = 32 * kc + 8 * qq + j;
        v[j] = (__bf16)((okc && k < a.S) ? Wr[k] : 0.f);
      }
      *reinterpret_cast<bf16x8_t*>(a.Wp + e * 4) = v;
    } else {
      f32x4 v;
#pragma unroll
      for (int i = 0; i < 4; ++i) {
        const int k = 16 * kc + 4 * qq + i;
        v[i] = (okc && k < a.S) ? Wr[k] : 0.f;
      }
      *reinterpret_cast<f32x4*>(a.Wp + e * 4) = v;
    }
  }
  for (int c = blockIdx.x * 256 + threadIdx.x; c < a.C; c += gridDim.x * 256) {
    int seg, r;
    seg_of(c, NE, seg, r);
    a.Bc[c] = a.Bv[seg][r];
  }
}

__device__ __forceinline__ float sgn(float x) { return x > 0.f ? 1.f : (x < 0.f ? -1.f : 0.f); }
__device__ __forceinline__ float sum16(float v) {
  v += __shfl_xor(v, 1, 64); v += __shfl_xor(v, 2, 64); v += __shfl_xor(v, 4, 64); v += __shfl_xor(v, 8, 64);
  return v;
}
template <int CTRL>
__device__ __forceinline__ float dpp_f(float v) {
  return __builtin_bit_cast(float, __builtin_amdgcn_update_dpp(0, __builtin_bit_cast(int, v), CTRL, 0xf, 0xf, true));
}
__device__ __forceinline__ float row_sum16(float v) {
  v += dpp_f<0xB1>(v);
  v += dpp_f<0x4E>(v);
  v += dpp_f<0x141>(v);
  v += dpp_f<0x140>(v);
  return v;
}
__device__ __forceinline__ float sum32(float v) { v = sum16(v); v += __shfl_xor(v, 16, 64); return v; }

constexpr int NCTM = 26;
constexpr int RB = 16 * NW;

__host__ __device__ inline size_t wide_lds(int NCT) {
  return (size_t)(2 * NCT * 256 + RB * 16 + RB + 4 * RB + NW * (E + 3)) * 4;
}

template <bool BWD, bool BF, int NCTT, bool LOSS = false>
__global__ __launch_bounds__(64 * NW, 2) void qmix_wide_kernel(WideArgs a) {
  static_assert(!LOSS || BWD, "the loss is folded into the backward kernel");
  extern __shared__ __attribute__((aligned(16))) float smem[];
  const int tid = threadIdx.x, lane = tid & 63, wave = __builtin_amdgcn_readfirstlane(tid >> 6);
  const int q4 = lane >> 4, m = lane & 15;
  const int S = a.S, C = a.C, KC = a.KC;
  const int NCT = NCTT > 0 ? NCTT : a.NCT;
  const int N = NCTT > 0 ? (NCTT - 6) / 2 : a.N;
  float* Wl[2] = {smem, smem + NCT * 256};
  float* Qs = smem + 2 * NCT * 256;
  float* Gs = Qs + RB * 16;
  float* Ls = Gs + RB;
  float* red = Ls + 4 * RB;
  const f32x4* Wp4 = reinterpret_cast<const f32x4*>(a.Wp);
  const int witems = NCT * 64;
  const int S4x4 = ((S + 3) >> 2) * 4;
  const float wb2lo = a.wb2[m], wb2hi = a.wb2[16 + m];
  const float bb2 = a.bb2[0];
  float acc_wb2[2] = {0.f, 0.f}, acc_bb2 = 0.f;
  float acc_ln = 0.f, acc_lm = 0.f;
  const long nblk = (a.rows + RB - 1) / RB;

  f32x4 wpf[4];
  auto wfetch = [&](int kc) {
#pragma unroll
    for (int i = 0; i < 4; ++i) {
      int e = tid + 64 * NW * i;
      if (e > witems - 1) e = witems - 1;
      wpf[i] = Wp4[((long)(e >> 6) * KC + kc) * 64 + (e & 63)];
    }
  };
  auto wstash = [&](int b) {
#pragma unroll
    for (int i = 0; i < 4; ++i) {
      const int e = tid + 64 * NW * i;
      if (e < witems) *reinterpret_cast<f32x4*>(Wl[b] + e * 4) = wpf[i];
    }
  };

  for (long blk = blockIdx.x; blk < nblk; blk += gridDim.x) {
    const long row0 = blk * RB;
    const long rowm = row0 + 16 * wave + m;
    const long rowc = rowm < a.rows ? rowm : a.rows - 1;
    const ConcatRow cr = concat_row(a.s, rowc);
    const float* srow = a.s.p0 + cr.r0 * a.s.ld0;
    auto aload = [&](f32x4 (&v)[2], int kc) __attribute__((always_inline)) {
      if (BF) {
        const int k0 = 32 * kc + 8 * q4;
        v[0] = k0 < S4x4 ? *reinterpret_cast<const f32x4*>(srow + k0) : (f32x4){0.f, 0.f, 0.f, 0.f};
        v[1] = k0 + 4 < S4x4 ? *reinterpret_cast<const f32x4*>(srow + k0 + 4) : (f32x4){0.f, 0.f, 0.f, 0.f};
      } else {
        const int k0 = 16 * kc + 4 * q4;
        v[0] = k0 < S4x4 ? *reinterpret_cast<const f32x4*>(srow + k0) : (f32x4){0.f, 0.f, 0.f, 0.f};
      }
    };
    for (int e = tid; e < RB * N; e += 64 * NW) {
      const long row = row0 + e / N;
      Qs[(e / N) * 16 + e % N] = row < a.rows ? a.q[row * N + e % N] : 0.f;
    }
    if (BWD && tid < RB) {
      const long row = row0 + tid;
      if (LOSS) {
        const bool ok = row < a.rows;
        Ls[tid] = ok ? a.lr[row] : 0.f; Ls[RB + tid] = ok ? a.lterm[row] : 0.f;
        Ls[2 * RB + tid] = ok ? a.lpadded[row] : 1.f; Ls[3 * RB + tid] = ok ? a.lq_tgt[row] : 0.f;
      } else Gs[tid] = row < a.rows ? a.g[row] : 0.f;
    }

    f32x4 acc[NCTM];
#pragma unroll
    for (int ct = 0; ct < NCTM; ++ct) {
      const float bv = ct < NCT ? a.Bc[16 * ct + m] : 0.f;
      acc[ct] = (f32x4){bv, bv, bv, bv};
    }
    f32x4 a0[2], a1[2], a2[2], a3[2];
    const int KCm = KC - 1;
    wfetch(0);
    aload(a0, 0);
    aload(a1, 1 < KCm ? 1 : KCm);
    aload(a2, 2 < KCm ? 2 : KCm);
    wstash(0);
    if (KC > 1) wfetch(1);
    auto mac = [&](const f32x4 (&av)[2], int b) __attribute__((always_inline)) {
      const float* wl = Wl[b] + lane * 4;
      if (BF) {
        bf16x8_t a8;
        const bf16x4_t lo = __builtin_convertvector(av[0], bf16x4_t), hi = __builtin_convertvector(av[1], bf16x4_t);
#pragma unroll
        for (int i = 0; i < 4; ++i) { a8[i] = lo[i]; a8[4 + i] = hi[i]; }
#pragma unroll
        for (int ct = 0; ct < NCTM; ++ct)
          if (ct < NCT) {
            const bf16x8_t w8 = *reinterpret_cast<const bf16x8_t*>(wl + ct * 256);
            acc[ct] = __builtin_amdgcn_mfma_f32_16x16x32_bf16(a8, w8, acc[ct], 0, 0, 0);
          }
      } else {
#pragma unroll
        for (int ct = 0; ct < NCTM; ++ct)
          if (ct < NCT) {
            const f32x4 w4 = *reinterpret_cast<const f32x4*>(wl + ct * 256);
            acc[ct] = mfma16x4(av[0], w4, acc[ct]);
          }
      }
    };
#define WIDE_STEP(CUR, NXT3, c_)                                                    \
    if ((c_) < KC) {                                                                \
      WG_BARRIER();           \
      if ((c_) + 1 < KC) wstash(((c_) + 1) & 1);                                    \
      if ((c_) + 2 < KC) wfetch((c_) + 2);                                          \
      aload(NXT3, (c_) + 3 < KCm ? (c_) + 3 : KCm);                                 \
      mac(CUR, (c_) & 1);                                                           \
    }
    for (int kc = 0; kc < KC; kc += 4) {
      WIDE_STEP(a0, a3, kc)
      WIDE_STEP(a1, a0, kc + 1)
      WIDE_STEP(a2, a1, kc + 2)
      WIDE_STEP(a3, a2, kc + 3)
    }
// ... 9 lines not shown
      if (ct < 2 * N) {
#pragma unroll
        for (int i = 0; i < 4; ++i) pa[ct & 1][i] += qrow[i * 16 + (ct >> 1)] * fabsf(acc[ct][i]);
      }
    f32x4 tb1[2], tw2[2], th[2];
#pragma unroll
    for (int ct = 0; ct < NCTM; ++ct) {
      const int rel = ct - 2 * N;
      if (rel == 0) tb1[0] = acc[ct]; else if (rel == 1) tb1[1] = acc[ct];
      else if (rel == 2) tw2[0] = acc[ct]; else if (rel == 3) tw2[1] = acc[ct];
      else if (rel == 4) th[0] = acc[ct]; else if (rel == 5) th[1] = acc[ct];
    }
    float dpre[2][4], hidv[2][4], tot[4], gr[4] = {0.f, 0.f, 0.f, 0.f};
    auto mix_pass = [&](const bool with_grad) __attribute__((always_inline)) {
#pragma unroll
      for (int i = 0; i < 4; ++i) tot[i] = 0.f;
#pragma unroll
      for (int h = 0; h < 2; ++h)
#pragma unroll
        for (int i = 0; i < 4; ++i) {
          const float ae = pa[h][i] + tb1[h][i];
          const float ex = __expf(ae);
          const float hid = ae > 0.f ? ae : ex - 1.f;
          const float w2 = fabsf(tw2[h][i]), hb = fmaxf(th[h][i], 0.f);
          tot[i] += hid * w2 + hb * (h ? wb2hi : wb2lo);
          if (with_grad) {
            dpre[h][i] = gr[i] * w2 * (ae > 0.f ? 1.f : ex);
            hidv[h][i] = hid;
            acc_wb2[h] += gr[i] * hb;
          }
        }
    };
    const long rbase = row0 + 16 * wave + 4 * q4;
    if (BWD && !LOSS) {
#pragma unroll
      for (int i = 0; i < 4; ++i) gr[i] = Gs[16 * wave + 4 * q4 + i];
    }
    mix_pass(BWD && !LOSS);
    if (!BWD) {
#pragma unroll
      for (int i = 0; i < 4; ++i) {
        const float t = sum16(tot[i]);
        if (m == 0 && rbase + i < a.rows) a.q_tot[rbase + i] = t + bb2;
      }
    } else {
      if (LOSS) {
#pragma unroll
        for (int i = 0; i < 4; ++i) {
          const int rl = 16 * wave + 4 * q4 + i;
          const float qt = sum16(tot[i]) + bb2;
          const float mask = 1.f - Ls[2 * RB + rl];
          const float target = Ls[rl] + a.gamma * Ls[3 * RB + rl] * (1.f - Ls[RB + rl]);
          const float mtd = mask * (target - qt);
          gr[i] = -2.f * mask * mtd;
          if (m == 0) {
            acc_ln += mtd * mtd; acc_lm += mask;
            if (a.q_tot && rbase + i < a.rows) a.q_tot[rbase + i] = qt;
          }
        }
        mix_pass(true);
      }
#pragma unroll
      for (int i = 0; i < 4; ++i)
        if (m == 0) acc_bb2 += gr[i];
#pragma unroll
      for (int ct = 0; ct < NCTM; ++ct) {
        if (ct >= NCT) continue;
        const int rel = ct - 2 * N, h = ct & 1;
        f32x4 v;
        if (rel < 0) {
          float dqp[4];
#pragma unroll
          for (int i = 0; i < 4; ++i) {
            const float o = acc[ct][i];
            v[i] = qrow[i * 16 + (ct >> 1)] * dpre[h][i] * sgn(o);
            dqp[i] = fabsf(o) * dpre[h][i];
          }
          if (h == 1) {
#pragma unroll
            for (int i = 0; i < 4; ++i) {
              const float t = sum16(dqp[i] + fabsf(acc[ct - 1 < 0 ? 0 : ct - 1][i]) * dpre[0][i]);
              if (m == 0 && rbase + i < a.rows) a.dq[(rbase + i) * N + (ct >> 1)] = t;
            }
          }
        } else if (rel < 2) {
#pragma unroll
          for (int i = 0; i < 4; ++i) v[i] = dpre[h][i];
        } else if (rel < 4) {
#pragma unroll
          for (int i = 0; i < 4; ++i) v[i] = gr[i] * hidv[h][i] * sgn(acc[ct][i]);
        } else {
#pragma unroll
          for (int i = 0; i < 4; ++i) v[i] = acc[ct][i] > 0.f ? gr[i] * (h ? wb2hi : wb2lo) : 0.f;
        }
#pragma unroll
        for (int i = 0; i < 4; ++i)
          if (rbase + i < a.rows) a.dhy[(rbase + i) * C + 16 * ct + m] = v[i];
      }
    }
    WG_BARRIER();
  }
  if (BWD) {
#pragma unroll
    for (int h = 0; h < 2; ++h) {
      acc_wb2[h] += __shfl_xor(acc_wb2[h], 16, 64);
      acc_wb2[h] += __shfl_xor(acc_wb2[h], 32, 64);
    }
    acc_bb2 += __shfl_xor(acc_bb2, 16, 64);
    acc_bb2 += __shfl_xor(acc_bb2, 32, 64);
// ... 486 lines not shown
    else if (k == 16 * a.KT) a.dB[seg][r] += s;
  } else if (e < n1 + E + 3) {
    const long t = e - n1;
    if (t < E) a.dwb2[t] += s;
    else if (t == E) a.dbb2[0] += s;
    else if (a.loss2) a.loss2[t - E - 1] += s;
  }
}

inline bool supported(int N, int S, int Eq) {
  const int C = N * E + 3 * E;
  return Eq == E && N >= 1 && N <= 16 && C <= 16 * NCTM && S >= 4 && S <= 384;
}
inline ConcatSrc state_src(const marl_src_t* s) {
  ConcatSrc c;
  c.p0 = s->p0; c.ld0 = s->ld0; c.k0 = s->k0; c.p1 = nullptr; c.ld1 = 0; c.k1 = 0;
  c.idx = nullptr; c.nhot = 0; c.hot_w = 0; c.nid = 0; c.m0 = nullptr; c.ldm0 = 0;
  c.rpe0 = s->rpe0; c.bs0 = s->bs0; c.off0 = s->off0; c.rpei = 0; c.bsi = 0; c.offi = 0;
  c.fd0 = make_fastdiv((unsigned)(s->rpe0 > 0 ? s->rpe0 : 1));
  c.fdi = make_fastdiv(1); c.fdn = make_fastdiv(1);
  c.emap0 = s->emap0;
  return c;
}
inline bool src_ok(const marl_src_t* s, int S) {
  return s->p0 && s->k0 == S && !s->k1 && !s->nhot && !s->nid && !s->m0 && (s->ld0 % 4 == 0) && s->ld0 >= (S + 3) / 4 * 4 &&
         ((reinterpret_cast<uintptr_t>(s->p0) & 15) == 0);
}
inline int kc_of(int S, bool bf) { return bf ? (S + 31) / 32 : (S + 15) / 16; }
inline size_t packed_floats(int N, int S) {
  const int C = N * E + 3 * E, NCT = (C + 15) / 16;
  return (size_t)NCT * ((S + 15) / 16) * 256 + (size_t)((C + 3) / 4 * 4);
}
inline int wg_groups(int C) { return ((C + 15) / 16 + WNT - 1) / WNT; }
inline int wg_slabs(long rows) { long n = (rows + 8 * WCH - 1) / (8 * WCH); if (n > 64) n = 64; return (int)(n < 1 ? 1 : n); }
inline unsigned grid_for(long rows) {
  const long nblk = (rows + RB - 1) / RB;
  return (unsigned)(nblk < 256 ? nblk : 256);
}

int pack(const marl_qmix_weights_t* w, int N, int S, bool bf, float* ws, hipStream_t st, WideArgs& a) {
  PackArgs p;
  p.W[0] = w->w1; p.Bv[0] = w->w1_b; p.W[1] = w->b1; p.Bv[1] = w->b1_b; p.W[2] = w->w2; p.Bv[2] = w->w2_b;
  p.W[3] = w->h; p.Bv[3] = w->h_b;
  p.N = N; p.S = S; p.C = N * E + 3 * E; p.NCT = (p.C + 15) / 16; p.KC = kc_of(S, bf); p.bf = bf ? 1 : 0;
  p.Wp = ws; p.Bc = ws + (size_t)p.NCT * ((S + 15) / 16) * 256;
  const long total = (long)p.NCT * p.KC * 64;
  hipLaunchKernelGGL(qmix_pack_kernel, dim3((unsigned)((total + 255) / 256)), dim3(256), 0, st, p);
  MARL_CHECK_LAUNCH();
  a.Wp = p.Wp; a.Bc = p.Bc; a.wb2 = w->b2_w; a.bb2 = w->b2_b;
  a.N = N; a.S = S; a.C = p.C; a.NCT = p.NCT; a.KC = p.KC;
  return 0;
}

template <typename K>
int launch_main(K fn, const WideArgs& a, unsigned grid, bool bf, hipStream_t st) {
  (void)bf;
  const size_t lds = wide_lds(a.NCT);
  if (lds > 160 * 1024) return (int)hipErrorInvalidValue;
  hipError_t e = hipFuncSetAttribute((const void*)fn, hipFuncAttributeMaxDynamicSharedMemorySize, (int)lds);
  if (e != hipSuccess) return (int)e;
  void* kargs[] = {(void*)&a};
  e = hipLaunchKernel((const void*)fn, dim3(grid), dim3(64 * NW), kargs, lds, st);
  if (e != hipSuccess) return (int)e;
  MARL_CHECK_LAUNCH();
  return 0;
}

}

ST_DEFINE_SETTER(marl_debug_stamps_wide)

extern "C" int marl_qmix_wide_supported(int N, int S, int Eq) { return supported(N, S, Eq) ? 1 : 0; }

extern "C" size_t marl_qmix_wide_workspace(long rows, int N, int S, int backward) {
  const int C = N * E + 3 * E;
  size_t f = packed_floats(N, S);
  if (backward) {
    const int KT = (S + 15) / 16;
    f += (size_t)rows * C + (size_t)wg_slabs(rows) * C * (16 * KT + 1) + (size_t)256 * (E + 3) + 64;
  }
  return f * sizeof(float);
}

extern "C" const char* marl_qmix_wide_fwd_kernel(long rows, int N, int S, int flags) {
  const bool bf = (flags & 1) != 0;
  const bool res_off = !marl_switches()->wide_res;
  if (bf && N == 10 && (S + 31) / 32 == 11 && rows >= 128L * 16 * 16 && !res_off) return "qmix_wide_res_fwd_kernel";
  return "qmix_wide_kernel<false";
}

extern "C" int marl_qmix_wide_fwd(const marl_qmix_weights_t* w, const marl_src_t* s, const float* q, float* q_tot,
                                  float* ws, size_t ws_bytes, long rows, int N, int S, int Eq, int flags, void* stream) {
  if (rows <= 0) return 0;
  if (!supported(N, S, Eq) || !src_ok(s, S)) return (int)hipErrorInvalidValue;
  if (ws_bytes < marl_qmix_wide_workspace(rows, N, S, 0) || (reinterpret_cast<uintptr_t>(ws) & 15)) return (int)hipErrorInvalidValue;
  const bool bf = (flags & 1) != 0;
  hipStream_t st = (hipStream_t)stream;
  const bool res_off = !marl_switches()->wide_res;
  WideArgs a = {};
  int rc = pack(w, N, S, bf, ws, st, a);
  if (rc) return rc;
  a.s = state_src(s); a.q = q; a.q_tot = q_tot; a.rows = rows;
  const unsigned grid = grid_for(rows);
  if (bf && N == 10 && a.KC == 11 && rows >= 128L * 16 * 16 && !res_off) {
    const size_t lds = (size_t)(13 * 11 * 256 + NW * 256 + 13 * 16) * 4;
    hipError_t e = hipMemsetAsync(q_tot, 0, (size_t)rows * sizeof(float), st);
    if (e != hipSuccess) return (int)e;
    e = hipFuncSetAttribute((const void*)qmix_wide_res_fwd_kernel<13, 11>, hipFuncAttributeMaxDynamicSharedMemorySize, (int)lds);
    if (e != hipSuccess) return (int)e;
    void* kargs[] = {(void*)&a};
    e = hipLaunchKernel((const void*)qmix_wide_res_fwd_kernel<13, 11>, dim3(256), dim3(64 * NW), kargs, lds, st);
    if (e != hipSuccess) return (int)e;
    MARL_CHECK_LAUNCH();
    return 0;
  }
  if (a.NCT == NCTM) return bf ? launch_main(qmix_wide_kernel<false, true, NCTM>, a, grid, true, st)
                               : launch_main(qmix_wide_kernel<false, false, NCTM>, a, grid, false, st);
  return bf ? launch_main(qmix_wide_kernel<false, true, 0>, a, grid, true, st)
            : launch_main(qmix_wide_kernel<false, false, 0>, a, grid, false, st);
}

struct WideLoss { const float *q_tot_tgt, *r, *term, *padded; float gamma; float* q_tot; float* loss2; };

static int wide_bwd_impl(const marl_qmix_weights_t* w, const marl_src_t* s, const float* q, const float* dq_tot, const WideLoss* L,
                         float* dq, const marl_qmix_weights_t* grads, float* ws, size_t ws_bytes, long rows,
                         int N, int S, int Eq, int flags, void* stream) {
  if (rows <= 0) return 0;
  if (!supported(N, S, Eq) || !src_ok(s, S)) return (int)hipErrorInvalidValue;
  if (ws_bytes < marl_qmix_wide_workspace(rows, N, S, 1) || (reinterpret_cast<uintptr_t>(ws) & 15)) return (int)hipErrorInvalidValue;
  const bool bf = (flags & 1) != 0;
  hipStream_t st = (hipStream_t)stream;
  WideArgs a = {};
  int rc = pack(w, N, S, bf, ws, st, a);
  if (rc) return rc;
  const int C = a.C, KT = (S + 15) / 16;
  float* dhy = ws + (packed_floats(N, S) + 15) / 16 * 16;
  const int nslab = wg_slabs(rows);
  float* wslab = dhy + (size_t)rows * C;
  float* bslab = wslab + (size_t)nslab * C * (16 * KT + 1);
  a.s = state_src(s); a.q = q; a.g = dq_tot; a.dq = dq; a.dhy = dhy; a.slab = bslab; a.rows = rows;
  if (L) { a.lr = L->r; a.lterm = L->term; a.lpadded = L->padded; a.lq_tgt = L->q_tot_tgt; a.gamma = L->gamma; a.q_tot = L->q_tot; }
  const unsigned grid = grid_for(rows);
  if (L) {
    if (a.NCT == NCTM) rc = bf ? launch_main(qmix_wide_kernel<true, true, NCTM, true>, a, grid, true, st)
                               : launch_main(qmix_wide_kernel<true, false, NCTM, true>, a, grid, false, st);
    else rc = bf ? launch_main(qmix_wide_kernel<true, true, 0, true>, a, grid, true, st)
                 : launch_main(qmix_wide_kernel<true, false, 0, true>, a, grid, false, st);
  } else {
    if (a.NCT == NCTM) rc = bf ? launch_main(qmix_wide_kernel<true, true, NCTM>, a, grid, true, st)
                               : launch_main(qmix_wide_kernel<true, false, NCTM>, a, grid, false, st);
    else rc = bf ? launch_main(qmix_wide_kernel<true, true, 0>, a, grid, true, st)
                 : launch_main(qmix_wide_kernel<true, false, 0>, a, grid, false, st);
  }
  if (rc) return rc;
  WideWgArgs g;
  g.dhy = dhy; g.s = a.s; g.ws = wslab; g.rows = rows; g.S = S; g.C = C; g.KT = KT; g.nslab = nslab;
  if (bf && (flags & 2)) {
    size_t lds = (size_t)2 * WCH * (wgb_gb() + wgb_xb(KT)) + 2 * WCH * sizeof(long);
    const size_t red = (size_t)WCH * 16 * WNT * sizeof(float);
    if (lds < red) lds = red;
    hipError_t e = hipFuncSetAttribute((const void*)qmix_wide_wgrad_bf16_kernel, hipFuncAttributeMaxDynamicSharedMemorySize, (int)lds);
    if (e != hipSuccess) return (int)e;
    hipLaunchKernelGGL(qmix_wide_wgrad_bf16_kernel, dim3(nslab, wg_groups(C)), dim3(64 * NW), lds, st, g);
    MARL_CHECK_LAUNCH();
  } else {
    const size_t lds = (size_t)2 * WCH * (wg_gp() + wg_xp(KT)) * sizeof(float) + 2 * WCH * sizeof(long);
    hipError_t e = hipFuncSetAttribute((const void*)qmix_wide_wgrad_kernel, hipFuncAttributeMaxDynamicSharedMemorySize, (int)lds);
    if (e != hipSuccess) return (int)e;
    hipLaunchKernelGGL(qmix_wide_wgrad_kernel, dim3(nslab, wg_groups(C)), dim3(64 * NW), lds, st, g);
    MARL_CHECK_LAUNCH();
  }
  WideRedArgs r;
  r.ws = wslab; r.slab2 = bslab; r.nslab = nslab; r.nwg = (int)grid; r.N = N; r.S = S; r.C = C; r.KT = KT;
  r.loss2 = L ? L->loss2 : nullptr;
  r.dW[0] = const_cast<float*>(grads->w1); r.dB[0] = const_cast<float*>(grads->w1_b);
  r.dW[1] = const_cast<float*>(grads->b1); r.dB[1] = const_cast<float*>(grads->b1_b);
  r.dW[2] = const_cast<float*>(grads->w2); r.dB[2] = const_cast<float*>(grads->w2_b);
  r.dW[3] = const_cast<float*>(grads->h); r.dB[3] = const_cast<float*>(grads->h_b);
  r.dwb2 = const_cast<float*>(grads->b2_w); r.dbb2 = const_cast<float*>(grads->b2_b);
  const long total = (long)C * (16 * KT + 1) + E + 3;
  hipLaunchKernelGGL(qmix_wide_reduce_kernel, dim3((unsigned)((total + 63) / 64)), dim3(64 * RSG), 0, st, r);
  MARL_CHECK_LAUNCH();
  return 0;
}

extern "C" int marl_qmix_wide_bwd(const marl_qmix_weights_t* w, const marl_src_t* s, const float* q, const float* dq_tot,
                                  float* dq, const marl_qmix_weights_t* grads, float* ws, size_t ws_bytes, long rows,
                                  int N, int S, int Eq, int flags, void* stream) {
  return wide_bwd_impl(w, s, q, dq_tot, nullptr, dq, grads, ws, ws_bytes, rows, N, S, Eq, flags, stream);
}

extern "C" int marl_qmix_wide_loss_bwd(const marl_qmix_weights_t* w, const marl_src_t* s, const float* q, const float* q_tot_tgt,
                                       const float* r, const float* term, const float* padded, float gamma, float* q_tot,
                                       float* dq, const marl_qmix_weights_t* grads, float* loss2, float* ws, size_t ws_bytes,
                                       long rows, int N, int S, int Eq, int flags, void* stream) {
  if (!q_tot_tgt || !r || !term || !padded || !loss2) return (int)hipErrorInvalidValue;
  WideLoss L = {q_tot_tgt, r, term, padded, gamma, q_tot, loss2};
  return wide_bwd_impl(w, s, q, nullptr, &L, dq, grads, ws, ws_bytes, rows, N, S, Eq, flags, stream);
}
```

marl_amd/experiments.py:

```python
from __future__ import annotations

import contextlib
import os
import warnings

LIB_DEFAULTS = {"fwd_xs": 1, "fwd_w2l": 1, "bwd_pipe_max_rt": 4, "wgrad_tall": 1, "wide_res": 1, "rollout_v1": 0, "unroll_r6": 1}
HOST_DEFAULTS = {"no_pair": 0, "no_chain": 0, "chain_split": None, "mlp3_keep": 1, "x6_bwd_min_wg": 1, "force_reducer": 0}


def _env_int(name, default):
    v = os.environ.get("MARL_" + name.upper())
    if v is None or v == "":
        return default
    try:
        return int(v)
    except ValueError:
        warnings.warn("MARL_%s=%r ignored (want an integer)" % (name.upper(), v))
        return default


_lib_values = {k: _env_int(k, d) for k, d in LIB_DEFAULTS.items()}
_host_values = {k: _env_int(k, d) for k, d in HOST_DEFAULTS.items()}
if _host_values["chain_split"] is not None and not (_host_values["chain_split"] == 0 or
                                                      (8 <= _host_values["chain_split"] <= 248 and _host_values["chain_split"] % 8 == 0)):
    warnings.warn("MARL_CHAIN_SPLIT=%r ignored (want 0 or a multiple of 8 in 8..248)" % _host_values["chain_split"])
    _host_values["chain_split"] = None
_applied = None
generation = 0


def apply(lib):
    global _applied
    _applied = lib
    for k, v in _lib_values.items():
        if v != LIB_DEFAULTS[k]:
            rc = lib.marl_experiment_set(k.encode(), int(v))
            assert rc == 0, "marl_experiment_set(%s) failed" % k


def get(name):
    if name in _host_values:
        return _host_values[name]
    if name in _lib_values:
        if _applied is not None:
            _lib_values[name] = int(_applied.marl_experiment_get(name.encode()))
        return _lib_values[name]
    raise KeyError(name)


def set(name, value):
    global generation
    generation += 1
    if name in _host_values:
        _host_values[name] = value
        return
    if name not in _lib_values:
        raise KeyError(name)
    _lib_values[name] = int(value)
    from . import _lib
    rc = _lib.load().marl_experiment_set(name.encode(), int(value))
# ... 14 lines not shown
```

marl_amd/hostutil.py:

```python
from __future__ import annotations

import weakref

import numpy as np
import torch
import torch.nn as nn

from . import ops


def require_cuda(what="the MARL hot path"):
    if not torch.cuda.is_available():
        raise RuntimeError("%s runs only on the MI355X HIP kernels (no CPU fallback); "
                           "torch.cuda.is_available() is False" % what)
    return torch.device("cuda", torch.cuda.current_device())


class FlatParams:

    def __init__(self, params, device, with_grad=True):
        self.params = list(params)
        self.offsets = []
        off = 0
        for p in self.params:
            self.offsets.append(off)
            off += (p.numel() + 3) // 4 * 4
        n = off
        self.flat = torch.zeros(n, dtype=torch.float32, device=device)
        self.grad = torch.zeros(n, dtype=torch.float32, device=device) if with_grad else None
        for p, off in zip(self.params, self.offsets):
            k = p.numel()
            self.flat[off:off + k].copy_(p.data.reshape(-1).to(device=device, dtype=torch.float32))
            p.data = self.flat[off:off + k].view(p.shape)
            if with_grad:
                p.grad = self.grad[off:off + k].view(p.shape)
        self.n = n

    def zero_grad(self):
        self.grad.zero_()


class Scratch:

    def __init__(self):
        self.d = {}

    def get(self, name, shape, device, dtype=torch.float32, zero=False):
        key = (name, tuple(shape), dtype)
        t = self.d.get(key)
        if t is None or t.device != device:
            t = (torch.zeros if zero else torch.empty)(*shape, dtype=dtype, device=device)
            self.d[key] = t
        return t

    def get_flat(self, name, n, device):
        key = (name, "flat")
        t = self.d.get(key)
        if t is None or t.device != device or t.numel() < n:
            if t is not None:
                ops.WS.retire()
            t = torch.empty(max(int(n), 1), dtype=torch.float32, device=device)
            self.d[key] = t
        return t

    def get_rows(self, name, rows, width, device):
        ld = (width + 3) // 4 * 4
        return self.get(name, (rows, ld), device)[:, :width]


_STRUCTS = weakref.WeakKeyDictionary()


def _struct_hit(owner, name, tensors=None):
    c = _STRUCTS.get(owner, {}).get(name)
    if c is not None and [q.data_ptr() for q in (c[0] if tensors is None else tensors)] == c[1]:
        return c[2]
    return None


def _struct_store(owner, name, tensors, w):
    _STRUCTS.setdefault(owner, {})[name] = (tensors, [q.data_ptr() if q.is_cuda else None for q in tensors], w)
    return w


def cached_struct(owner, name, tensors, build):
    tensors = list(tensors)
    w = _struct_hit(owner, name, tensors)
    return w if w is not None else _struct_store(owner, name, tensors, build())


def cached_module_struct(module, name, build, buffers=False):
    w = _struct_hit(module, name)
    if w is not None:
        return w
    if next(module.parameters()).device.type != "cuda":
        module.to(require_cuda("RNNQNet"))
    tracked = dict(module.named_parameters())
    for v in tracked.values():
        if not v.data.is_contiguous():
            v.data = v.data.contiguous()
    tensors = {k: v.data for k, v in tracked.items()}
    if buffers:
        tracked.update(module.named_buffers())
        tensors.update(module.named_buffers())
    return _struct_store(module, name, list(tracked.values()), build(tensors))

# ... 57 lines not shown
        ev = torch.cuda.Event()
        ev.record()
        slot[1] = ev
        return out


_PINNED = _PinnedRing()


def h2d_async(arr, device, dtype):
    if torch.device(device).type != "cuda":
        return torch.as_tensor(np.asarray(arr), dtype=dtype, device=device)
    return _PINNED.to_device(arr, device, dtype)


class AsyncInt:
    _side = {}
    _bufs = {}

    def __init__(self, dev_tensor):
        cur = torch.cuda.current_stream()
        key = dev_tensor.device
        side = AsyncInt._side.get(key)
        if side is None:
            side = AsyncInt._side[key] = torch.cuda.Stream(device=key)
            AsyncInt._bufs[key] = [[torch.empty(1, dtype=dev_tensor.dtype).pin_memory() for _ in range(8)], 0]
        ring = AsyncInt._bufs[key]
        self.buf = ring[0][ring[1] % 8]
        ring[1] += 1
        ready = torch.cuda.Event()
        ready.record(cur)
        with torch.cuda.stream(side):
            side.wait_event(ready)
            self.buf.copy_(dev_tensor, non_blocking=True)
            self.done = torch.cuda.Event()
            self.done.record(side)

    def wait(self):
        self.done.synchronize()
        return int(self.buf[0])


def onehot_to_index(u_onehot):
    s = u_onehot.sum(-1)
    idx = u_onehot.argmax(-1).to(torch.int32)
    return torch.where(s > 0, idx, torch.full_like(idx, -1)).contiguous()


class DeviceBatch:

    def __init__(self):
        self.extra = {}
        self.ep_len = None

    @staticmethod
    def first_terminated_len(term, episode_limit, reducer=None):
        dist_on = reducer is not None and reducer.enabled
        if term.is_cuda and term.dtype == torch.float32 and term.shape[0] > 0:
            out = ops.first_terminated_len(term, episode_limit)
            if dist_on:
                reducer.dist.all_reduce(out, op=reducer.dist.ReduceOp.MAX, group=reducer.group)
            m = int(out.item())
            return m if m > 0 else episode_limit
        t = (term.reshape(term.shape[0], -1)[:, :episode_limit] == 1)
        anyt = t.any(dim=1)
        first = t.to(torch.int32).argmax(dim=1) + 1
        m = int(torch.where(anyt, first, torch.zeros_like(first)).max().item()) if t.shape[0] > 0 else 0
        if dist_on:
            m = reducer.max_int(m, torch.device("cuda", torch.cuda.current_device()) if torch.cuda.is_available()
                                else torch.device("cpu"))
        return m if m > 0 else episode_limit

    @classmethod
    def from_dict(cls, batch, args, device, T=None):
        self = cls()
        N, O, S, A = args.n_agents, args.obs_shape, args.state_shape, args.n_actions
        term_full = to_dev(batch["terminated"], device)
        if T is None:
            T = cls.first_terminated_len(term_full, args.episode_limit)
        B = term_full.shape[0]
        self.B, self.T, self.N, self.O, self.S, self.A = B, T, N, O, S, A
        cut = lambda k, dt=torch.float32: to_dev(batch[k][:, :T], device, dt)
        o, o_next = cut("o"), cut("o_next")
        self.o_cur = (o, T * N, 0)
        self.o_next = (o_next, T * N, 0)
        def rows16(x):
            x = x.view(B * T, S)
            if S % 4 == 0:
                return x
            buf = torch.zeros(B * T, (S + 3) // 4 * 4, dtype=x.dtype, device=x.device)
            buf[:, :S] = x
            return buf[:, :S]
        self.s = rows16(cut("s"))
        self.s_next = rows16(cut("s_next"))
        self.u_act = cut("u", torch.int32).view(B, T, N)
        if "u_idx" in batch:
            self.u_fed = cut("u_idx", torch.int32).view(B, T, N)
        else:
            self.u_fed = onehot_to_index(cut("u_onehot")).view(B, T, N)
        self.u_bs = T * N
        self.u_taken = self.u_fed
        self.r = cut("r").view(B * T)
        self.term = term_full[:, :T].contiguous().view(B * T)
        self.padded = cut("padded").view(B * T)
        self.avail = cut("avail_u").view(B * T * N, A)
        self.avail_next = cut("avail_u_next").view(B * T * N, A)
# ... 107 lines not shown
```

marl_amd/network/mixer.py:

```python
from __future__ import annotations

import os

import numpy as np
import torch
import torch.nn as nn

from .. import ops
from ..hostutil import Lin, Scratch, cached_struct, lin_of, require_cuda, to_dev, onehot_to_index


class _Precision:

    def _bf16(self):
        return getattr(self.args, "mixer_dtype", "fp32") == "bf16"

    def _x6mode(self):
        return x6_mode(self.args)

    def _wgrad_bf16(self):
        return self._bf16() and getattr(self.args, "mixer_wgrad_dtype", "bf16") != "fp32"

    def _lin(self, module):
        return lin_of(module, self._bf16())
# ... 103 lines not shown
            ops.qmix_wide_fwd(self._fused_struct(), xs, q, qtot, rows, N, a.state_shape, E, bf16=self._bf16())
            if ctx is not None:
                ctx.update(q=q, s=s, wide=True)
            return qtot
        wid = N * E + 3 * E
        hy = self._s.get("hy" + tag, (rows, wid), dev)
        b2 = self._s.get("b2" + tag, (rows, 1), dev)
        qtot = self._s.get("qtot" + tag, (rows,), dev)
        hw1 = hw2 = None
        if a.two_hyper_layers:
            kept, hid = {}, {}
            for name, seq, cols in (("w1", self.hyper_w1, slice(0, N * E)), ("w2", self.hyper_w2, slice(N * E + E, N * E + 2 * E))):
                wh = self._fused_hyper(seq, xs)
                if wh is not None:
                    w, G, n3g = wh
                    hs = None
                    if ctx is not None:
                        hs = kept[name] = self._s.get_flat("hs_" + name, ops.mlp3_save_floats(rows, False, G), dev)
                    ops.mlp3_fwd(w, xs, hy[:, cols], rows, a.state_shape, n3g, G, hsave=hs)
                    continue
                l0, l2 = _linears(seq)
                hbuf = hid[name] = self._s.get("h" + name + tag, (rows, HH), dev)
                self._lin(l0).fwd(xs, hbuf, rows, act=1)
                self._lin(l2).fwd(ops.src(hbuf), hy[:, cols], rows)
            hw1, hw2 = hid.get("w1"), hid.get("w2")
        else:
            self._lin(self.hyper_w1).fwd(xs, hy[:, :N * E], rows)
            self._lin(self.hyper_w2).fwd(xs, hy[:, N * E + E:N * E + 2 * E], rows)
        b20, b22 = _linears(self.hyper_b2)
        tail = self._tail_ok(s)
        if tail:
            ops.qmix_tail_fwd(s, rows, a.state_shape, self.hyper_b1.weight.data, self.hyper_b1.bias.data, b20.weight.data,
                              b20.bias.data, hy, N * E, N * E + 2 * E)
            ops.qmix_mix_fwd(hy, None, q, qtot, rows, N, E, w22=b22.weight.data, b22=b22.bias.data)
        else:
            self._lin(self.hyper_b1).fwd(xs, hy[:, N * E:N * E + E], rows)
            self._lin(b20).fwd(xs, hy[:, N * E + 2 * E:], rows, act=1)
            self._lin(b22).fwd(ops.src(hy[:, N * E + 2 * E:]), b2, rows)
            ops.qmix_mix_fwd(hy, b2, q, qtot, rows, N, E)
        if ctx is not None:
            ctx.update(hy=hy, q=q, s=s, hw1=hw1, hw2=hw2, kept=kept if a.two_hyper_layers else {}, tail=tail)
        return qtot

    def _tail_ok(self, s):
        a = self.args
        return (not self._bf16() and not getattr(self, "no_fused", False)
                and ops.qmix_tail_supported(a.state_shape, a.qmix_hidden_dim, s)
                and self.hyper_b1.weight.data.data_ptr() % 4 == 0)

    def loss_backward_fused(self, s):
        xs = ops.src(s)
        return self._fused_ok(xs) or self._wide_ok(xs)

    def hip_loss_backward(self, q, s, rows, q_tot_tgt, r, term, padded, gamma, loss2, q_tot=None):
        a = self.args
        N, E = a.n_agents, a.qmix_hidden_dim
        dq = self._s.get("dq", (rows, N), q.device)
        xs = ops.src(s)
        if self._fused_ok(xs):
            ops.qmix_fused_loss_bwd(self._fused_struct(), xs, q, q_tot_tgt, r, term, padded, gamma, q_tot, dq,
                                    self._fused_struct(grad=True), loss2, rows, N, a.state_shape, E, x6=self._x6mode())
        else:
            ops.qmix_wide_loss_bwd(self._fused_struct(), xs, q, q_tot_tgt, r, term, padded, gamma, q_tot, dq,
                                   self._fused_struct(grad=True), loss2, rows, N, a.state_shape, E, bf16=self._bf16(),
                                   wgrad_bf16=self._wgrad_bf16())
        return dq

    def hip_backward(self, ctx, dq_tot, rows):
        a = self.args
        N, E, HH = a.n_agents, a.qmix_hidden_dim, a.hyper_hidden_dim
        if ctx.get("fused"):
            q, s = ctx["q"], ctx["s"]
            dq = self._s.get("dq", (rows, N), q.device)
            ops.qmix_fused_bwd(self._fused_struct(), ops.src(s), q, dq_tot, dq,
                               self._fused_struct(grad=True), rows, N, a.state_shape, E, x6=self._x6mode())
            return dq
        if ctx.get("wide"):
            q, s = ctx["q"], ctx["s"]
            dq = self._s.get("dq", (rows, N), q.device)
            ops.qmix_wide_bwd(self._fused_struct(), ops.src(s), q, dq_tot, dq, self._fused_struct(grad=True), rows, N,
                              a.state_shape, E, bf16=self._bf16(), wgrad_bf16=self._wgrad_bf16())
            return dq
        hy, q, s = ctx["hy"], ctx["q"], ctx["s"]
        dev = q.device
        dhy = self._s.get("dhy", hy.shape, dev)
        db2 = self._s.get("db2", (rows, 1), dev)
        dq = self._s.get("dq", (rows, N), dev)
        b20, b22 = _linears(self.hyper_b2)
        ops.qmix_mix_bwd(hy, q, dq_tot, dhy, db2, dq, rows, N, E, w22=b22.weight.data if ctx.get("tail") else None)
        xs = ops.src(s)
        hb, dhb = hy[:, N * E + 2 * E:], dhy[:, N * E + 2 * E:]
        self._lin(b22).wgrad(db2, ops.src(hb), rows)
        if not ctx.get("tail"):
            self._lin(b22).bwd_x(db2, dhb, rows)
        self._lin(b20).wgrad(dhb, xs, rows, Yact=hb)
        self._lin(self.hyper_b1).wgrad(dhy[:, N * E:N * E + E], xs, rows)
        if a.two_hyper_layers:
            for name, seq, hbuf, cols in (("w1", self.hyper_w1, ctx["hw1"], slice(0, N * E)),
                                          ("w2", self.hyper_w2, ctx["hw2"], slice(N * E + E, N * E + 2 * E))):
                hs = ctx["kept"].get(name)
                if hs is not None:
                    wh, gh = self._fused_hyper(seq, xs), self._fused_hyper(seq, xs, grad=True)
                    if wh is None or gh is None:
                        raise RuntimeError("QMixMixer: the fused hypernet head %r kept its activations in the forward but its "
                                           "backward cannot be launched (.grad tensors missing / not contiguous / not 16-byte "
                                           "aligned, or MARL_MLP3_KEEP changed between forward and backward)" % name)
                    w, G, n3g = wh
                    ops.mlp3_bwd(w, xs, dhy[:, cols], gh[0], rows, a.state_shape, n3g, G, hsave=hs)
                    continue
                l0, l2 = _linears(seq)
                self._lin(l2).wgrad(dhy[:, cols], ops.src(hbuf), rows)
                dh = self._s.get("dhw", (rows, HH), dev)
                self._lin(l2).bwd_x(dhy[:, cols], dh, rows)
                self._lin(l0).wgrad(dh, xs, rows, Yact=hbuf)
        else:
            self._lin(self.hyper_w1).wgrad(dhy[:, :N * E], xs, rows)
            self._lin(self.hyper_w2).wgrad(dhy[:, N * E + E:N * E + 2 * E], xs, rows)
        return dq
# ... 326 lines not shown
        self._lin(w0).fwd(xs, hw, rows, act=1)
        self._lin(w2).fwd(ops.src(hw), hy[:, H * U:H * U + H], rows)
        c0, c2 = _linears(self.const)
        self._lin(c0).fwd(xs, hc, rows, act=1)
        self._lin(c2).fwd(ops.src(hc), hy[:, H * U + H:], rows)
        return dict(s=s, hy=hy, hq=hq, e=e, hw=hw, hc=hc)

    def _dense_backward(self, ctx, dhy, dc, rows):
        N, U, H, D, HE = self._dims()
        dev = dhy.device
        xs = ops.src(ctx["s"])
        for seq, hbuf, dout, width in ((self.const, ctx["hc"], dc.view(rows, 1), D),
                                       (self.head_weight, ctx["hw"], dhy[:, H * U:H * U + H], HE)):
            l0, l2 = _linears(seq)
            self._lin(l2).wgrad(dout, ops.src(hbuf), rows)
            dh = self._s.get("dh%d" % width, (rows, width), dev)
            self._lin(l2).bwd_x(dout, dh, rows)
            self._lin(l0).wgrad(dh, xs, rows, Yact=hbuf)
        de = self._s.get("de", (rows, D), dev)
        dhq = self._s.get("dh%d" % HE, (rows, HE), dev)
        for h in range(H):
            q0, q2 = _linears(self.query[h])
            hq_h, e_h, dp_h = ctx["hq"][:, h * HE:(h + 1) * HE], ctx["e"][:, h * D:(h + 1) * D], dhy[:, h * U:(h + 1) * U]
            self._key(h).wgrad(e_h, ops.src(dp_h), rows)
            self._key(h).fwd(ops.src(dp_h), de, rows)
            self._lin(q2).wgrad(de, ops.src(hq_h), rows)
            self._lin(q2).bwd_x(de, dhq, rows)
            self._lin(q0).wgrad(dhq, xs, rows, Yact=hq_h)

    def hip_forward(self, q, s, rows, ctx=None, tag="e"):
        N, U, H, D, HE = self._dims()
        kept = self._dense_forward(s, rows, tag)
        qtot = self._s.get("qtot" + tag, (rows,), q.device)
        ops.qatten_mix_fwd(ops.src(s), kept["hy"], q, self._scale(), qtot, rows, N, U, H)
        if ctx is not None:
            ctx.update(kept, q=q)
        return qtot

    def _grad_rows(self, rows, dev):
        N, U, H, D, HE = self._dims()
        return self._s.get("dq", (rows, N), dev), self._s.get_rows("dhy", rows, H * U + H, dev)

    def hip_backward(self, ctx, dq_tot, rows):
        N, U, H, D, HE = self._dims()
        dq, dhy = self._grad_rows(rows, dq_tot.device)
        ops.qatten_mix_bwd(ops.src(ctx["s"]), ctx["hy"], ctx["q"], self._scale(), dq_tot, dq, dhy, rows, N, U, H)
        self._dense_backward(ctx, dhy, dq_tot, rows)
        return dq

    def loss_backward_fused(self, s):
        N, U, H, D, HE = self._dims()
        return ops.qatten_supported(s, N, U, H)

    def hip_loss_backward(self, q, s, rows, q_tot_tgt, r, term, padded, gamma, loss2, q_tot=None):
        N, U, H, D, HE = self._dims()
        ctx = self._dense_forward(s, rows, "e")
        dq, dhy = self._grad_rows(rows, q.device)
        dq_tot = self._s.get("dq_tot", (rows,), q.device)
        ops.qatten_loss_bwd(ops.src(s), ctx["hy"], q, self._scale(), q_tot_tgt, r, term, padded, gamma, q_tot, dq, dhy, dq_tot, loss2,
                            rows, N, U, H)
        self._dense_backward(ctx, dhy, dq_tot, rows)
        return dq

    def forward(self, q_values, states):
        dev = require_cuda("QattenMixer")
        self.to(dev)
        B = q_values.shape[0]
        q = to_dev(q_values, dev).reshape(-1, self.args.n_agents)
        s = to_dev(states, dev).reshape(-1, self.state_dim)
        return self.hip_forward(q, s, q.shape[0]).clone().view(B, -1, 1)


class _QtranFusedHead:

    def _qt_dims(self):
        a = self.args
        A = self._qt_actions()
        AE = a.rnn_hidden_dim + A
        return a.n_agents, A, AE, (AE + 15) // 16 * 16, a.state_shape

    def _qt_ok(self, hidden):
        a = self.args
        N, A, AE, _, _ = self._qt_dims()
        return (not self._bf16() and not getattr(self, "no_fused", False) and a.rnn_hidden_dim == 64
                and a.qtran_hidden_dim == 64 and ops.qtran_supported(N, A, AE) and hidden.is_contiguous()
                and hidden.data_ptr() % 16 == 0)

    def _qt_struct(self):
        layers = zip(("enc0", "enc2", "q0", "q2", "q4"), self._qt_layers())
        t = {k + "." + a: getattr(l, a).data for k, l in layers for a in ("weight", "bias")}
        baked = [t[name] for _, name, _ in ops.QTRAN_FIELDS]
        return cached_struct(self, "qtran", baked, lambda: ops.qtran_weights(t, self.args.state_shape))

    def state_part(self, s, BT, tag="e", other=None):
        q0 = self._qt_layers()[2]
        S = self.args.state_shape
        sp = self._s.get("sp" + tag, (BT, q0.out_features), s.device)
        heads = [(self, sp)]
        if other is not None:
            heads.append((other, other._s.get("sp" + tag, (BT, q0.out_features), s.device)))
        if ops.qtran_state_parts_supported(S, s) and not self._bf16():
            sets = []
            for net, out in heads:
                l0 = net._qt_layers()[2]
                sets.append((l0.weight.data, l0.bias.data, out))
            ops.qtran_state_parts(s, BT, S, sets)
        else:
            for net, out in heads:
                l0 = net._qt_layers()[2]
                Lin(l0.weight.data[:, :S], l0.bias, net._bf16()).fwd(ops.src(s), out, BT)
        return sp if other is None else (sp, heads[1][1])

    def _qt_forward(self, s, hidden, u_idx, BT, ctx, tag, sp, u_idx2=None):
# ... 217 lines not shown
```

marl_amd/ops.py:

```python
from __future__ import annotations

import collections
import ctypes as C

import torch

from . import _lib
from ._lib import (MarlSrc, MarlGroup, MarlAgentWeights, MarlAgentGrads, MarlQmixWeights, MarlMlp3Weights,
                   MarlQtranWeights, MarlRtwWeights, MarlWorldWeights, MarlWorldGrads, MarlMaicWeights, MarlMaicGrads, MarlMaicInfer,
                   MarlMaicInferGrads, MarlCommnetWeights, MarlCommnetGrads, MarlG2anetWeights, MarlG2anetGrads, MarlRecord,
                   check)


def _p(t):
    return None if t is None else C.c_void_p(t.data_ptr())


def _stream():
    return C.c_void_p(torch.cuda.current_stream().cuda_stream)


def _f32(t):
    assert t.dtype == torch.float32 and t.is_cuda, "expected a CUDA float32 tensor"
    return t
# ... 322 lines not shown


def qmix_mix_bwd(hy, q, dq_tot, dhy, db2, dq, rows, N, E, w22=None):
    assert dhy.stride(0) == hy.stride(0)
    check(_lib.load().marl_qmix_mix_bwd(_p(_f32(hy)), hy.stride(0), _p(_f32(q)), _p(_f32(dq_tot)), _p(w22), _p(_f32(dhy)),
                                        _p(_f32(db2)), _p(_f32(dq)), rows, N, E, _stream()), "marl_qmix_mix_bwd")


def qmix_tail_supported(S, E, s):
    return E == 32 and qtran_state_parts_supported(S, s)


def qmix_tail_fwd(s, rows, S, b1_w, b1_b, h_w, h_b, hy, c_b1, c_h):
    assert b1_w.stride(1) == 1 and h_w.stride(1) == 1 and b1_w.stride(0) == h_w.stride(0) and hy.stride(1) == 1
    x = src(s)
    check(_lib.load().marl_qmix_tail_fwd(C.byref(x), rows, S, _p(_f32(b1_w)), b1_w.stride(0), _p(_f32(b1_b)), _p(_f32(h_w)),
                                         h_w.stride(0), _p(_f32(h_b)), _p(_f32(hy)), hy.stride(0), c_b1, c_h, _stream()),
          "marl_qmix_tail_fwd")


def qplex_mix_fwd(w_raw, v, q, max_q, key, ag, ac, v_tot, a_tot, lam_out, rows, N, K, weighted, minus_one):
    check(_lib.load().marl_qplex_mix_fwd(_p(w_raw), _p(v), _p(q), _p(max_q), _p(key), _p(ag), _p(ac), _p(v_tot),
                                         _p(a_tot), _p(lam_out), rows, N, K, int(weighted), int(minus_one), _stream()),
          "marl_qplex_mix_fwd")


def qplex_mix_bwd(w_raw, q, max_q, key, ag, ac, g, dq, dw_raw, dv, dkey, dag, dac, rows, N, K, weighted, minus_one):
    check(_lib.load().marl_qplex_mix_bwd(_p(w_raw), _p(q), _p(max_q), _p(key), _p(ag), _p(ac), _p(g), _p(dq),
                                         _p(dw_raw), _p(dv), _p(dkey), _p(dag), _p(dac), rows, N, K, int(weighted),
                                         int(minus_one), _stream()), "marl_qplex_mix_bwd")


def qatten_supported(s, N, U, H):
    x = s if isinstance(s, MarlSrc) else src(s)
    return bool(_lib.load().marl_qatten_supported(C.byref(x), N, U, H))


def qatten_plan(rows, N, U, H):
    plan = (C.c_int * 4)()
    check(_lib.load().marl_qatten_plan(rows, N, U, H, plan), "marl_qatten_plan")
    return tuple(plan)


def qatten_mix_fwd(s, hy, q, scale, q_tot, rows, N, U, H):
    check(_lib.load().marl_qatten_mix_fwd(C.byref(s), _p(_f32(hy)), hy.stride(0), _p(_f32(q)), float(scale), _p(_f32(q_tot)), rows,
                                          N, U, H, _stream()), "marl_qatten_mix_fwd")


def qatten_mix_bwd(s, hy, q, scale, dq_tot, dq, dhy, rows, N, U, H):
    check(_lib.load().marl_qatten_mix_bwd(C.byref(s), _p(_f32(hy)), hy.stride(0), _p(_f32(q)), float(scale), _p(_f32(dq_tot)),
                                          _p(_f32(dq)), _p(_f32(dhy)), dhy.stride(0), rows, N, U, H, _stream()), "marl_qatten_mix_bwd")


def qatten_loss_bwd(s, hy, q, scale, q_tot_tgt, r, term, padded, gamma, q_tot, dq, dhy, dq_tot, out2, rows, N, U, H):
    lib = _lib.load()
    ws = WS.get("loss", lib.marl_loss_workspace(rows), q.device)
    check(lib.marl_qatten_loss_bwd(C.byref(s), _p(_f32(hy)), hy.stride(0), _p(_f32(q)), float(scale), _p(_f32(q_tot_tgt)),
                                   _p(_f32(r)), _p(_f32(term)), _p(_f32(padded)), float(gamma), _p(q_tot), _p(_f32(dq)),
                                   _p(_f32(dhy)), dhy.stride(0), _p(_f32(dq_tot)), _p(_f32(out2)), _p(ws), rows, N, U, H, _stream()),
          "marl_qatten_loss_bwd")


def lica_supported(N, A, E):
    return bool(_lib.load().marl_lica_supported(N, A, E))


def lica_plan(rows, N, A, E):
    plan = (C.c_int * 4)()
    check(_lib.load().marl_lica_plan(rows, N, A, E, plan), "marl_lica_plan")
    return tuple(plan)


def _lica_in(x, u):
    return _p(None if x is None else _f32(x)), _p(None if u is None else _i32(u))


def lica_mix_fwd(hy, x, u, q, rows, N, A, E):
    px, pu = _lica_in(x, u)
    check(_lib.load().marl_lica_mix_fwd(_p(_f32(hy)), hy.stride(0), px, pu, _p(_f32(q)), rows, N, A, E, _stream()), "marl_lica_mix_fwd")


def lica_mix_bwd(hy, x, u, dq, dhy, dx, rows, N, A, E):
    px, pu = _lica_in(x, u)
    check(_lib.load().marl_lica_mix_bwd(_p(_f32(hy)), hy.stride(0), px, pu, _p(_f32(dq)), _p(None if dhy is None else _f32(dhy)),
                                        0 if dhy is None else dhy.stride(0), _p(None if dx is None else _f32(dx)), rows, N, A, E,
                                        _stream()), "marl_lica_mix_bwd")


def lica_loss_bwd(hy, u, q_tgt, r, term, padded, gamma, q, dhy, dq_tot, out2, rows, N, A, E):
    lib = _lib.load()
    ws = WS.get("loss", lib.marl_loss_workspace(rows), hy.device)
    check(lib.marl_lica_loss_bwd(_p(_f32(hy)), hy.stride(0), _p(_i32(u)), _p(_f32(q_tgt)), _p(_f32(r)), _p(_f32(term)),
                                 _p(_f32(padded)), float(gamma), _p(_f32(q)), _p(_f32(dhy)), dhy.stride(0), _p(_f32(dq_tot)),
                                 _p(_f32(out2)), _p(ws), rows, N, A, E, _stream()), "marl_lica_loss_bwd")


_FT_OUT = {}


def replay_gather(idx, src, out):
    assert idx.dtype == torch.int64 and idx.is_cuda and idx.is_contiguous()
    B, T, N, A = int(idx.numel()), src.T, src.N, src.A
    for t in (src.u, src.r, src.term, src.padded, src.length, src.won, src.avail, out.u, out.u_act, out.r, out.term, out.padded,
              out.length, out.won, out.avail_next, out.o_map):
        assert t.is_cuda and t.is_contiguous()
    assert src.u.dtype == torch.int32 and src.length.dtype == torch.int32 and src.won.dtype == torch.int32
    check(_lib.load().marl_replay_gather(_p(idx), B, T, N, A, _p(src.u), _p(_f32(src.r)), _p(_f32(src.term)), _p(_f32(src.padded)),
                                         _p(src.length), _p(src.won), _p(_f32(src.avail)), _p(_i32(out.o_map)), _p(_i32(out.u)),
                                         _p(_i32(out.u_act)), _p(_f32(out.r)), _p(_f32(out.term)), _p(_f32(out.padded)),
                                         _p(_i32(out.length)), _p(_i32(out.won)), _p(_f32(out.avail_next)),
                                         _p(getattr(out, "avail_cur", None)), _stream()),
          "marl_replay_gather")


def first_terminated_len(term, T):
    t2 = term.reshape(term.shape[0], -1)
    assert t2.dtype == torch.float32 and t2.is_cuda and t2.stride(1) == 1
    ring = _FT_OUT.get(t2.device)
    if ring is None:
        ring = _FT_OUT[t2.device] = [torch.zeros(8, dtype=torch.int32, device=t2.device), 0]
    out = ring[0][ring[1] % 8:ring[1] % 8 + 1]
    ring[1] += 1
    check(_lib.load().marl_first_terminated_len(_p(t2), t2.stride(0), t2.shape[0], min(T, t2.shape[1]), _p(out), _stream()),
          "marl_first_terminated_len")
    return out


def td_loss(q_tot, q_tgt, r, term, padded, gamma, dq_tot, out2, rows):
    lib = _lib.load()
    ws = WS.get("loss", lib.marl_loss_workspace(rows), q_tot.device)
    check(lib.marl_td_loss(_p(_f32(q_tot)), _p(_f32(q_tgt)), _p(_f32(r)), _p(_f32(term)), _p(_f32(padded)),
                           float(gamma), _p(_f32(dq_tot)), _p(_f32(out2)), _p(ws), rows, _stream()), "marl_td_loss")


def qtran_loss(jq, jq_tgt, v, jq_hat, qs_opt, qs_nopt, r, term, padded, gamma, lam_opt, lam_nopt,
               d_jq, d_v, d_qso, d_qsn, out4, rows):
    lib = _lib.load()
    ws = WS.get("loss", lib.marl_loss_workspace(rows), jq.device)
    check(lib.marl_qtran_loss(_p(jq), _p(jq_tgt), _p(v), _p(jq_hat), _p(qs_opt), _p(qs_nopt), _p(r), _p(term),
                              _p(padded), float(gamma), float(lam_opt), float(lam_nopt), _p(d_jq), _p(d_v), _p(d_qso),
                              _p(d_qsn), _p(out4), _p(ws), rows, _stream()), "marl_qtran_loss")


def td_lambda_returns(q_next_tot, r, term, padded, gamma, lam, out, B, T):
    lib = _lib.load()
    for t in (q_next_tot, r, term, padded, out):
        assert _f32(t).is_contiguous() and t.numel() >= B * T, "td_lambda_returns: contiguous (B, T) float32 arrays"
    check(lib.marl_td_lambda_returns(_p(q_next_tot), _p(r), _p(term), _p(padded), float(gamma), float(lam), _p(out),
                                     int(B), int(T), _stream()), "marl_td_lambda_returns")
    return out


def _iql_rows(B, T, N, A, per_row_a, per_row, per_step):
    R = B * T * N
    for t, n in [(x, R * A) for x in per_row_a] + [(x, R) for x in per_row] + [(x, B * T) for x in per_step]:
        assert t is None or (t.is_cuda and t.is_contiguous() and t.numel() >= n), "iql: contiguous device arrays of the rows' sizes"


def iql_loss_bwd(q, u, q_sel, q_tgt, avail_next, ret, r, term, padded, gamma, mask_val, dq_val, out2, B, T, N, A,
                 q_taken=None, q_next=None):
    lib = _lib.load()
    _iql_rows(B, T, N, A, (q, q_sel, q_tgt, avail_next), (u, ret, dq_val, q_taken, q_next), (r, term, padded))
    ws = WS.get("loss", lib.marl_loss_workspace(B * T * N), q.device)
    check(lib.marl_iql_loss_bwd(_p(_f32(q)), _p(_i32(u)), _p(q_sel), _p(q_tgt), _p(avail_next), _p(ret), _p(r), _p(term),
                                _p(_f32(padded)), float(gamma), float(mask_val), _p(_f32(dq_val)), _p(q_taken), _p(q_next),
                                _p(_f32(out2)), _p(ws), int(B), int(T), int(N), int(A), _stream()), "marl_iql_loss_bwd")
    return dq_val


def iql_select(q, u, q_sel, q_tgt, avail_next, padded, mask_val, q_taken, q_next_bnt, B, T, N, A):
    _iql_rows(B, T, N, A, (q, q_sel, q_tgt, avail_next), (u, q_taken, q_next_bnt), (padded,))
    check(_lib.load().marl_iql_select(_p(_f32(q)), _p(_i32(u)), _p(q_sel), _p(_f32(q_tgt)), _p(avail_next), _p(_f32(padded)),
                                      float(mask_val), _p(q_taken), _p(_f32(q_next_bnt)), int(B), int(T), int(N), int(A),
                                      _stream()), "marl_iql_select")
    return q_next_bnt


def policy_probs(logits, avail, eps, pi, rows, A):
    for t in (logits, avail, pi):
        assert _f32(t).is_contiguous() and t.numel() >= rows * A
    check(_lib.load().marl_policy_probs(_p(logits), _p(avail), float(eps), _p(pi), rows, A, _stream()), "marl_policy_probs")
    return pi

# ... 297 lines not shown
def battle_rollout(w, seed, rseed, env0, episode, types, shield, type_bits, scale, units, rec, h_out, M, last_action,
                   reuse_network, stats, eps_sched, sample=False):
    fn, name = _entry("marl_battle_rollout", sample)
    check(fn(C.byref(w), record(rec, cache=False), int(seed) & 0xFFFFFFFF, int(rseed) & 0xFFFFFFFF, env0, episode, types, int(shield),
             type_bits, float(scale), _p(_i32(units)), _p(h_out), _p(_f32(stats)) if stats is not None else None,
             *map(float, eps_sched), M, 1 if last_action else 0, 1 if reuse_network else 0, _stream()), name)


def synth_rollout_supported(N, O, A):
    return bool(_lib.load().marl_synth_rollout_supported(N, O, A))


def synth_rollout_x6_supported(N, O, A, last_action=True, reuse_network=True):
    return bool(_lib.load().marl_synth_rollout_x6_supported_flags(N, O, A, 1 if last_action else 0, 1 if reuse_network else 0))


def synth_rollout_x6_plan(E, N, O, A, last_action=True, reuse_network=True):
    plan = (C.c_int * 5)()
    check(_lib.load().marl_synth_rollout_x6_plan(E, N, O, A, 1 if last_action else 0, 1 if reuse_network else 0, plan), "marl_synth_rollout_x6_plan")
    return tuple(plan)


def synth_rollout(w, seed, rseed, env0, episode, fixed_len, eps, rec, h_out, E, T, N, O, S, A, last_action, reuse_network,
                  stats=None, eps_sched=None, x6=False, sample=False):
    assert (eps is None) != (eps_sched is None) and (E, T, N, O, S, A) == (rec.E, rec.T, rec.N, rec.O, rec.S, rec.A)
    fn, name = _entry("marl_synth_rollout", sample, x6)
    check(fn(C.byref(w), record(rec, cache=False), int(seed) & 0xFFFFFFFF, int(rseed) & 0xFFFFFFFF, env0, episode, 1 if fixed_len else 0,
             _p(_f32(eps)) if eps is not None else None, _p(h_out), _p(_f32(stats)) if stats is not None else None,
             *map(float, eps_sched or (0.0, 0.0, 0.0)), 1 if last_action else 0, 1 if reuse_network else 0, _stream()), name)


def qmix_fused_supported(N, S, E):
    return bool(_lib.load().marl_qmix_fused_supported(N, S, E))


def qmix_weights(t):
    return _fill_struct(MarlQmixWeights, t, [(k, k, torch.float32) for k, _ in MarlQmixWeights._fields_])


def qmix_fused_fwd(w, s, q, q_tot, rows, N, S, E, x6=False):
    lib = _lib.load()
    fn = lib.marl_qmix_fused_fwd_x6 if x6 else lib.marl_qmix_fused_fwd
    check(fn(C.byref(w), C.byref(s), _p(_f32(q)), _p(_f32(q_tot)), rows, N, S, E, _stream()), "marl_qmix_fused_fwd")


def qmix_fused_bwd(w, s, q, dq_tot, dq, grads, rows, N, S, E, x6=False):
    lib = _lib.load()
    ws = WS.get("qmix_fused", lib.marl_qmix_fused_workspace(rows, N, S), q.device)
    fn = lib.marl_qmix_fused_bwd_x6 if x6 else lib.marl_qmix_fused_bwd
    check(fn(C.byref(w), C.byref(s), _p(_f32(q)), _p(_f32(dq_tot)), _p(_f32(dq)), C.byref(grads),
             _p(ws), ws.numel() * 4, rows, N, S, E, _stream()), "marl_qmix_fused_bwd")


def qmix_fused_loss_bwd(w, s, q, q_tot_tgt, r, term, padded, gamma, q_tot, dq, grads, loss2, rows, N, S, E, x6=False):
    lib = _lib.load()
    ws = WS.get("qmix_fused", lib.marl_qmix_fused_workspace(rows, N, S), q.device)
    check((lib.marl_qmix_fused_loss_bwd_x6 if x6 else lib.marl_qmix_fused_loss_bwd)(C.byref(w), C.byref(s), _p(_f32(q)), _p(_f32(q_tot_tgt)), _p(_f32(r)), _p(_f32(term)),
                                       _p(_f32(padded)), float(gamma), _p(q_tot), _p(_f32(dq)), C.byref(grads), _p(_f32(loss2)),
                                       _p(ws), ws.numel() * 4, rows, N, S, E, _stream()), "marl_qmix_fused_loss_bwd")


def _wide_flags(bf16, wgrad_bf16):
    return (1 if bf16 else 0) | (2 if (bf16 and (wgrad_bf16 is None or wgrad_bf16)) else 0)


def qmix_wide_loss_bwd(w, s, q, q_tot_tgt, r, term, padded, gamma, q_tot, dq, grads, loss2, rows, N, S, E, bf16=False, wgrad_bf16=None):
    lib = _lib.load()
    ws = WS.get("qmix_wide", lib.marl_qmix_wide_workspace(rows, N, S, 1), q.device)
    check(lib.marl_qmix_wide_loss_bwd(C.byref(w), C.byref(s), _p(_f32(q)), _p(_f32(q_tot_tgt)), _p(_f32(r)), _p(_f32(term)),
                                      _p(_f32(padded)), float(gamma), _p(q_tot), _p(_f32(dq)), C.byref(grads), _p(_f32(loss2)),
                                      _p(ws), ws.numel() * 4, rows, N, S, E, _wide_flags(bf16, wgrad_bf16), _stream()), "marl_qmix_wide_loss_bwd")


def qmix_wide_fwd_kernel(rows, N, S, bf16=False):
    return _lib.load().marl_qmix_wide_fwd_kernel(rows, N, S, 1 if bf16 else 0).decode()


def qmix_wide_supported(N, S, E):
    return bool(_lib.load().marl_qmix_wide_supported(N, S, E))


def qmix_wide_fwd(w, s, q, q_tot, rows, N, S, E, bf16=False):
    lib = _lib.load()
    ws = WS.get("qmix_wide", lib.marl_qmix_wide_workspace(rows, N, S, 0), q.device)
    check(lib.marl_qmix_wide_fwd(C.byref(w), C.byref(s), _p(_f32(q)), _p(_f32(q_tot)), _p(ws), ws.numel() * 4, rows, N, S, E,
                                 1 if bf16 else 0, _stream()), "marl_qmix_wide_fwd")


def qmix_wide_bwd(w, s, q, dq_tot, dq, grads, rows, N, S, E, bf16=False, wgrad_bf16=None):
    lib = _lib.load()
    ws = WS.get("qmix_wide", lib.marl_qmix_wide_workspace(rows, N, S, 1), q.device)
    check(lib.marl_qmix_wide_bwd(C.byref(w), C.byref(s), _p(_f32(q)), _p(_f32(dq_tot)), _p(_f32(dq)), C.byref(grads), _p(ws),
                                 ws.numel() * 4, rows, N, S, E, _wide_flags(bf16, wgrad_bf16), _stream()), "marl_qmix_wide_bwd")


def uniform_stride(ts, align):
    if len(ts) == 1:
        return 0
    d = [ts[i + 1].data_ptr() - ts[i].data_ptr() for i in range(len(ts) - 1)]
    if any(x != d[0] for x in d) or d[0] <= 0 or d[0] % align != 0:
        return None
    return d[0] // 4


def mlp3_weights(heads, grad=False):
    pick = (lambda p: p.grad) if grad else (lambda p: p.data)
    w = MarlMlp3Weights()
    keep = []
    names = (("w1", "b1"), ("w2", "b2"), ("w3", "b3")) if len(heads[0]) == 3 else (("w1", "b1"), ("w3", "b3"))
    for li, (wn, bn) in enumerate(names):
        for name, attr in ((wn, "weight"), (bn, "bias")):
            ts = [pick(getattr(h[li], attr)) for h in heads]
            if not _dense_on_device(ts[0], align=16) or not all(_dense_on_device(t) for t in ts):
                return None
            st = uniform_stride(ts, 16)
            if st is None:
                return None
            setattr(w, name, ts[0].data_ptr())
            setattr(w, "gs_" + name, st)
            keep.append(ts)
    w._keep = keep
# ... 355 lines not shown
```

marl_amd/rollout.py:

```python
from __future__ import annotations

import numpy as np
import torch

from . import ops
from .hostutil import h2d_async, require_cuda
from .network.mixer import x6_mode


class EpisodeBatch(dict):

    KEYS = ("o", "s", "u", "r", "avail_u", "o_next", "s_next", "avail_u_next", "u_onehot", "padded", "terminated")

    def __init__(self, record=None, ring=None, index=None):
        super().__init__()
        self._record = record
        self.ring, self.index = ring, index

    @property
    def record(self):
        if self._record is None and self.ring is not None:
            self._record = self.ring.index_select(self.index)
        return self._record

    def _build(self, k):
        r = self.record
        T = r.T
        t_idx = torch.arange(T, device=r.obs.device)[None, :]
        live = (t_idx < r.length[:, None])
        if k in ("o", "s", "avail_u"):
            src = {"o": r.obs, "s": r.state, "avail_u": r.avail}[k][:, :T]
            m = live.view(r.E, T, *([1] * (src.dim() - 2)))
            return torch.where(m, src, torch.zeros_like(src))
        if k in ("o_next", "s_next", "avail_u_next"):
            return {"o_next": r.obs, "s_next": r.state, "avail_u_next": r.avail}[k][:, 1:]
        if k == "u":
            return r.u.clamp(min=0).long().unsqueeze(-1)
        if k == "u_onehot":
            oh = torch.zeros(r.E, T, r.N, r.A, device=r.u.device)
            return oh.scatter_(3, r.u.clamp(min=0).long().unsqueeze(-1), (r.u >= 0).float().unsqueeze(-1))
        if k == "u_idx":
            return r.u
        return {"r": r.r, "padded": r.padded, "terminated": r.term}[k].unsqueeze(-1)

    def __missing__(self, k):
        if k not in self.KEYS and k != "u_idx":
            raise KeyError(k)
        v = self._build(k)
        self[k] = v
        return v

    def keys(self):
        return list(self.KEYS)

    def __iter__(self):
        return iter(self.KEYS)

    def __len__(self):
        return len(self.KEYS)

    def items(self):
        return [(k, self[k]) for k in self.KEYS]

    def numpy(self):
        out = {}
        for k in self.KEYS:
            v = self[k].cpu().numpy()
            out[k] = v.astype(np.int64) if k == "u" else v.astype(np.float64)
        return out

# ... 251 lines not shown
```

Before: 73.68 million.

## Deduplicate replay-sampled episodes and weight TD loss by multiplicity

When a sampled batch contains repeated episode indices, the learner computes unique episodes on the host and runs forward/backward only on the distinct ones. Each episode's TD loss contribution and gradient is scaled by its count, so the result matches the full duplicated batch. Weighted variants of the td_loss, qatten and qmix loss kernels are added, each using a fastdiv to map rows to episodes. The path is gated behind an experiments flag and skipped when graph replay covers the batch, and it adds host-side unique and H2D cost and elastic scratch sizing.

```diff
diff --git a/include/marl_hip.h b/include/marl_hip.h
--- a/include/marl_hip.h
+++ b/include/marl_hip.h
@@ -109,6 +109,14 @@
                                 const float* r, const float* term, const float* padded, float gamma, float* q_tot,
                                 float* dq, const marl_qmix_weights_t* grads, float* loss2, float* ws, size_t ws_bytes,
                                 long rows, int N, int S, int E, void* stream);
+int marl_qmix_fused_loss_bwd_w(const marl_qmix_weights_t* w, const marl_src_t* s, const float* q, const float* q_tot_tgt,
+                               const float* r, const float* term, const float* padded, float gamma, const float* ep_w,
+                               int rows_per_ep, float* q_tot, float* dq, const marl_qmix_weights_t* grads, float* loss2,
+                               float* ws, size_t ws_bytes, long rows, int N, int S, int E, void* stream);
+int marl_qmix_fused_loss_bwd_x6_w(const marl_qmix_weights_t* w, const marl_src_t* s, const float* q, const float* q_tot_tgt,
+                                  const float* r, const float* term, const float* padded, float gamma, const float* ep_w,
+                                  int rows_per_ep, float* q_tot, float* dq, const marl_qmix_weights_t* grads, float* loss2,
+                                  float* ws, size_t ws_bytes, long rows, int N, int S, int E, void* stream);
 
 int marl_qmix_wide_supported(int N, int S, int E);
 const char* marl_qmix_wide_fwd_kernel(long rows, int N, int S, int flags);
@@ -122,6 +130,10 @@
                             const float* r, const float* term, const float* padded, float gamma, float* q_tot, float* dq,
                             const marl_qmix_weights_t* grads, float* loss2, float* ws, size_t ws_bytes, long rows,
                             int N, int S, int E, int flags, void* stream);
+int marl_qmix_wide_loss_bwd_w(const marl_qmix_weights_t* w, const marl_src_t* s, const float* q, const float* q_tot_tgt,
+                              const float* r, const float* term, const float* padded, float gamma, const float* ep_w,
+                              int rows_per_ep, float* q_tot, float* dq, const marl_qmix_weights_t* grads, float* loss2,
+                              float* ws, size_t ws_bytes, long rows, int N, int S, int E, int flags, void* stream);
 
 typedef struct {
   const float *w1, *b1;
@@ -240,6 +252,9 @@
 int marl_td_loss(const float* q_tot, const float* q_tot_tgt, const float* r, const float* term,
                  const float* padded, float gamma, float* dq_tot, float* out2, float* ws, long rows,
                  void* stream);
+int marl_td_loss_w(const float* q_tot, const float* q_tot_tgt, const float* r, const float* term, const float* padded,
+                   float gamma, const float* ep_w, int rows_per_ep, float* dq_tot, float* out2, float* ws, long rows,
+                   void* stream);
 int marl_qtran_loss(const float* jq, const float* jq_tgt, const float* v, const float* jq_hat,
                     const float* qsum_opt, const float* qsum_nopt, const float* r, const float* term,
                     const float* padded, float gamma, float lam_opt, float lam_nopt, float* d_jq,
@@ -257,6 +272,10 @@
                          const float* q_tot_tgt, const float* r, const float* term, const float* padded, float gamma,
                          float* q_tot, float* dq, float* dhy, long lddh, float* dq_tot, float* out2, float* ws, long rows,
                          int N, int U, int H, void* stream);
+int marl_qatten_loss_bwd_w(const marl_src_t* s, const float* hy, long ldh, const float* q, float scale,
+                           const float* q_tot_tgt, const float* r, const float* term, const float* padded, float gamma,
+                           const float* ep_w, int rows_per_ep, float* q_tot, float* dq, float* dhy, long lddh, float* dq_tot,
+                           float* out2, float* ws, long rows, int N, int U, int H, void* stream);
 
 int marl_lica_supported(int N, int A, int E);
 int marl_lica_plan(long rows, int N, int A, int E, int* plan);
diff --git a/marl_amd/algorithm/common.py b/marl_amd/algorithm/common.py
--- a/marl_amd/algorithm/common.py
+++ b/marl_amd/algorithm/common.py
@@ -10,7 +10,7 @@
 import torch
 
 from .. import ops, experiments
-from ..hostutil import FlatParams, DeviceBatch, AsyncInt, Scratch, require_cuda
+from ..hostutil import FlatParams, DeviceBatch, AsyncInt, Scratch, require_cuda, h2d_async
 from ..network.mixer import x6_mode
 from ..rollout import EpisodeBatch
 
@@ -147,6 +147,19 @@
         return LossReadback.Handle(buf, ev, fn)
 
 
+DEDUP_MIN_SHARE = 16
+
+
+def distinct_episodes(index_host):
+    idx = np.asarray(index_host).reshape(-1)
+    uniq, counts = np.unique(idx, return_counts=True)
+    n, U = idx.size, uniq.size
+    idx_pad, w_pad = np.empty(n, dtype=np.int64), np.zeros(n, dtype=np.float32)
+    idx_pad[:U], idx_pad[U:] = uniq, uniq[-1] if U else 0
+    w_pad[:U] = counts
+    return idx_pad, w_pad, U
+
+
 def td_lambda_of(args):
     lam = getattr(args, "td_lambda", None)
     if lam is None:
@@ -161,6 +174,7 @@
     n_stats, den_slot = 2, 1
     extra_nets = ()
     launch_ahead = True
+    last_dedup = None
     replay_graphs = True
 
     def _begin(self, mac, args, name):
@@ -213,26 +227,72 @@
             batch[key] = batch[key][:, :T]
         return batch, T
 
-    def _device_batch(self, rec, index, small):
+    def _takes_ep_weights(self):
+        return False
+
+    def _dedup_mode(self, batch):
+        mode = experiments.get("dedup")
+        if not mode or not self._takes_ep_weights() or not isinstance(batch, EpisodeBatch) or batch.ring is None \
+                or getattr(batch, "index_host", None) is None:
+            return 0
+        n = int(batch.index.numel())
+        if mode != 2 and (n <= GraphedUpdate.AUTO_MAX_EPISODES or (self.graphs is not None and self.graphs.covers(n))):
+            return 0
+        return mode
+
+    def _dedup(self, batch, mode):
+        self.last_dedup = None
+        idx_pad, w_pad, U = distinct_episodes(batch.index_host)
+        n = idx_pad.size
+        if U == n or (mode != 2 and (n - U) * DEDUP_MIN_SHARE < n):
+            return batch.index, None
+        dev = batch.index.device
+        self.last_dedup = (n, U)
+        return h2d_async(idx_pad, dev, torch.long)[:U], h2d_async(w_pad, dev, torch.float32)[:U]
+
+    def _scratches(self):
+        owners = [(self, "_buf")] + [(getattr(self, k, None), a) for k, a in (("mixer", "_s"), ("target_mixer", "_s"),
+                                                                             ("eval_net", "_buf"), ("target_net", "_buf"))]
+        return [getattr(o, a) for o, a in owners if isinstance(getattr(o, a, None), Scratch)]
+
+    def _device_batch(self, rec, index, small, ep_w=None):
         term = (small if small is not None else rec).term
         if not (term.is_cuda and term.dtype == torch.float32 and term.shape[0] > 0) or self._full_len_streak < 2 \
                 or not self.launch_ahead:
             db = DeviceBatch.from_record_auto(rec, self.args, reducer=self.reducer, index=index, small=small)
+            db.ep_w = ep_w
             full = db.T == min(rec.T, self.args.episode_limit)
             self._full_len_streak = self._full_len_streak + 1 if full else 0
             return db
         db, pending = DeviceBatch.from_record_begin(rec, self.args, reducer=self.reducer, index=index, small=small)
+        db.ep_w = ep_w
         self.max_episode_len = db.T
         self._forward_backward(db)
         T = pending()
         if T == db.T:
             return None
         self._full_len_streak = 0
-        return DeviceBatch.from_record(rec, self.args, T=T, index=index, small=small)
+        db = DeviceBatch.from_record(rec, self.args, T=T, index=index, small=small)
+        db.ep_w = ep_w
+        return db
 
     def train(self, batch, train_step):
+        self.last_dedup = None
+        dedup = self._dedup_mode(batch)
+        if not dedup:
+            return self._train(batch, train_step, 0)
+        scratches = self._scratches()
+        try:
+            for s in scratches:
+                s.elastic = (int(batch.index.numel()), int(batch.index.numel()))
+            return self._train(batch, train_step, dedup)
+        finally:
+            for s in scratches:
+                s.elastic = None
+
+    def _train(self, batch, train_step, dedup):
         ring = batch.ring if isinstance(batch, EpisodeBatch) else None
-        if self.graphs is not None and ring is not None and self.graphs.run(self, ring, batch.index):
+        if self.graphs is not None and ring is not None and dedup != 2 and self.graphs.run(self, ring, batch.index):
             db = None
         elif isinstance(batch, DeviceBatch):
             db = batch
@@ -242,8 +302,12 @@
                 self.graphs.prepared = None
                 db = DeviceBatch.from_record(ring, self.args, T=prep[1], index=batch.index, small=prep[0])
             else:
-                small = ring.select_small(batch.index, avail_cur=self.needs_avail)
-                db = self._device_batch(ring, batch.index, small)
+                index, ep_w = self._dedup(batch, dedup) if dedup else (batch.index, None)
+                if ep_w is not None:
+                    for s in self._scratches():
+                        s.elastic = (int(index.numel()), int(batch.index.numel()))
+                small = ring.select_small(index, avail_cur=self.needs_avail)
+                db = self._device_batch(ring, index, small, ep_w)
         elif isinstance(batch, EpisodeBatch) and batch.record is not None:
             db = self._device_batch(batch.record, None, None)
         else:
@@ -436,6 +500,7 @@
         self.disabled = False
         self.auto = bool(auto)
         self.replays = 0
+        self.prepared = None
 
     @staticmethod
     def from_args(args):
@@ -450,6 +515,9 @@
     @staticmethod
     def _schedule_key(args):
         return (experiments.generation,) + tuple(repr(getattr(args, k, None)) for k in GraphedUpdate.SCHEDULE_ARGS)
+
+    def covers(self, episodes):
+        return not self.disabled and not (self.auto and episodes > self.AUTO_MAX_EPISODES)
 
     def run(self, learner, ring, index):
         self.prepared = None
diff --git a/marl_amd/algorithm/q_learner.py b/marl_amd/algorithm/q_learner.py
--- a/marl_amd/algorithm/q_learner.py
+++ b/marl_amd/algorithm/q_learner.py
@@ -28,6 +28,9 @@
         self.params = list(mac.parameters()) + list(self.mixer.parameters())
         self.cuda()
         self._ready(needs_avail=args.alg == 'qplex')
+
+    def _takes_ep_weights(self):
+        return type(self) is QLearner
 
     def sync_replicas(self):
         o = self.optimizer
@@ -120,11 +123,12 @@
     def _loss_backward(self, db, q_chosen, q_tot, q_tot_tgt, ctx, fold):
         BT = db.B * db.T
         r, gamma = self._td_inputs(db, q_tot_tgt)
+        wt = {} if getattr(db, "ep_w", None) is None else dict(ep_w=db.ep_w, rows_per_ep=db.T)
         if fold:
             return self.mixer.hip_loss_backward(q_chosen.view(BT, db.N), db.s, BT, q_tot_tgt, r, db.term, db.padded, gamma,
-                                                self._flat.stats[:2], q_tot=q_tot)
+                                                self._flat.stats[:2], q_tot=q_tot, **wt)
         dq_tot = self._g("dq_tot", (BT,))
-        ops.td_loss(q_tot, q_tot_tgt, r, db.term, db.padded, gamma, dq_tot, self._flat.stats[:2], BT)
+        ops.td_loss(q_tot, q_tot_tgt, r, db.term, db.padded, gamma, dq_tot, self._flat.stats[:2], BT, **wt)
         return self.mixer.hip_backward(ctx, dq_tot, BT)
 
     def _forward_backward(self, db):
diff --git a/marl_amd/common/replaybuffer.py b/marl_amd/common/replaybuffer.py
--- a/marl_amd/common/replaybuffer.py
+++ b/marl_amd/common/replaybuffer.py
@@ -92,7 +92,7 @@
             idx = np.random.randint(0, self.current_size, batch_size)
         if self.record is not None:
             idx_t = h2d_async(idx, self.record.obs.device, torch.long)
-            return EpisodeBatch(ring=self.record, index=idx_t)
+            return EpisodeBatch(ring=self.record, index=idx_t, index_host=idx)
         return {k: self.buffers[k][idx] for k in self.buffers}
 
     def _get_storage_idx(self, inc=None):
diff --git a/marl_amd/csrc/mixers.hip b/marl_amd/csrc/mixers.hip
--- a/marl_amd/csrc/mixers.hip
+++ b/marl_amd/csrc/mixers.hip
@@ -394,17 +394,29 @@
   return 0;
 }
 
+__device__ __forceinline__ float td_row_weight(long i, const float* ep_w, FastDiv rpe) { return ep_w[fastdiv((unsigned)i, rpe)]; }
+__device__ __forceinline__ float td_row_weight(long) { return 1.f; }
+template <class... W>
 __global__ void td_loss_kernel(const float* q_tot, const float* q_tgt, const float* r, const float* term,
-                               const float* padded, float gamma, float* dq_tot, float* ws, long rows) {
+                               const float* padded, float gamma, float* dq_tot, float* ws, long rows, W... wt) {
+  constexpr bool WT = sizeof...(W) != 0;
   float acc[2] = {0.f, 0.f};
   for (long i = (long)blockIdx.x * TPB + threadIdx.x; i < rows; i += (long)gridDim.x * TPB) {
     const float mask = 1.f - padded[i];
     const float target = r[i] + gamma * q_tgt[i] * (1.f - term[i]);
     const float td = target - q_tot[i];
     const float mtd = mask * td;
-    acc[0] += mtd * mtd;
-    acc[1] += mask;
-    dq_tot[i] = -2.f * mask * mtd;
+    if constexpr (WT) {
+      const float w = td_row_weight(i, wt...);
+      const float wmtd = w * mtd;
+      acc[0] += wmtd * mtd;
+      acc[1] += w * mask;
+      dq_tot[i] = w * (-2.f * mask * mtd);
+    } else {
+      acc[0] += mtd * mtd;
+      acc[1] += mask;
+      dq_tot[i] = -2.f * mask * mtd;
+    }
   }
   block_partials<2>(acc, ws);
 }
@@ -674,8 +686,22 @@
                             void* stream) {
   if (rows <= 0) return 0;
   const int nb = rt::partial_blocks(rows);
-  hipLaunchKernelGGL(td_loss_kernel, dim3(nb), dim3(TPB), 0, (hipStream_t)stream, q_tot, q_tot_tgt, r, term, padded,
+  hipLaunchKernelGGL(td_loss_kernel<>, dim3(nb), dim3(TPB), 0, (hipStream_t)stream, q_tot, q_tot_tgt, r, term, padded,
                      gamma, dq_tot, ws, rows);
+  MARL_CHECK_LAUNCH();
+  hipLaunchKernelGGL(finish_sums_kernel, dim3(1), dim3(TPB), 0, (hipStream_t)stream, (const float*)ws, nb, 2, out2);
+  MARL_CHECK_LAUNCH();
+  return 0;
+}
+
+extern "C" int marl_td_loss_w(const float* q_tot, const float* q_tot_tgt, const float* r, const float* term,
+                              const float* padded, float gamma, const float* ep_w, int rows_per_ep, float* dq_tot,
+                              float* out2, float* ws, long rows, void* stream) {
+  if (rows <= 0) return 0;
+  if (!ep_w || rows_per_ep < 1 || rows >= (1L << 31)) return (int)hipErrorInvalidValue;
+  const int nb = rt::partial_blocks(rows);
+  hipLaunchKernelGGL((td_loss_kernel<const float*, FastDiv>), dim3(nb), dim3(TPB), 0, (hipStream_t)stream, q_tot, q_tot_tgt, r, term, padded,
+                     gamma, dq_tot, ws, rows, ep_w, make_fastdiv((unsigned)rows_per_ep));
   MARL_CHECK_LAUNCH();
   hipLaunchKernelGGL(finish_sums_kernel, dim3(1), dim3(TPB), 0, (hipStream_t)stream, (const float*)ws, nb, 2, out2);
   MARL_CHECK_LAUNCH();
diff --git a/marl_amd/csrc/qatten.hip b/marl_amd/csrc/qatten.hip
--- a/marl_amd/csrc/qatten.hip
+++ b/marl_amd/csrc/qatten.hip
@@ -45,6 +45,9 @@
   long rows;
   int N, U, H, TR, SP, HP;
 };
+struct QaArgsW : QaArgs { const float* ep_w; FastDiv wfd; };
+template <bool WT> struct QaArgsOf { typedef QaArgs type; };
+template <> struct QaArgsOf<true> { typedef QaArgsW type; };
 
 struct Chunk { int lo, cnt; bool vec; };
 __device__ __forceinline__ Chunk chunk_of(const float* g, int n, int j) {
@@ -149,8 +152,9 @@
   return g * y * (w > 0.f ? 1.f : (w < 0.f ? -1.f : 0.f));
 }
 
-template <int MODE>
-__global__ __launch_bounds__(TPB) void qatten_kernel(QaArgs a) {
+template <int MODE, bool WT = false>
+__global__ __launch_bounds__(TPB) void qatten_kernel(typename QaArgsOf<WT>::type a) {
+  static_assert(!WT || MODE == MODE_LOSS, "the episode weights enter where the TD error does");
   extern __shared__ __attribute__((aligned(16))) float qa_smem[];
   const int N = a.N, U = a.U, H = a.H, TR = a.TR, SP = a.SP, HP = a.HP;
   const int NU = N * U, HU = H * U;
@@ -205,9 +209,17 @@
           const float target = a.r[r] + a.gamma * a.q_tgt[r] * (1.f - a.term[r]);
           const float td = target - qt;
           const float mtd = mask * td;
-          acc[0] += mtd * mtd;
-          acc[1] += mask;
-          g = -2.f * mask * mtd;
+          if constexpr (WT) {
+            const float ew = a.ep_w[fastdiv((unsigned)r, a.wfd)];
+            const float wmtd = ew * mtd;
+            acc[0] += wmtd * mtd;
+            acc[1] += ew * mask;
+            g = ew * (-2.f * mask * mtd);
+          } else {
+            acc[0] += mtd * mtd;
+            acc[1] += mask;
+            g = -2.f * mask * mtd;
+          }
           a.dq_tot[r] = g;
         }
       } else {
@@ -252,15 +264,15 @@
   return (int)(t > rt::PARTIAL_ROWS ? rt::PARTIAL_ROWS : t);
 }
 
-template <int MODE>
-int launch(QaArgs& a, const marl_src_t* s, hipStream_t stream) {
+template <int MODE, bool WT = false>
+int launch(typename QaArgsOf<WT>::type& a, const marl_src_t* s, hipStream_t stream) {
   if (!shape_ok(a.N, a.U, a.H) || !src_ok(s, a.N, a.U) || a.rows >= (1L << 31) || !a.hy || !a.q || a.ldh < a.H * a.U + a.H + 1)
     return (int)hipErrorInvalidValue;
   if (MODE != MODE_FWD && (!a.dq || !a.dhy || a.lddh < a.H * a.U + a.H)) return (int)hipErrorInvalidValue;
   const Tile t = tile_of(a.N, a.U, a.H);
   a.s = state_src(s);
   a.TR = t.TR; a.SP = t.SP; a.HP = t.HP;
-  const void* fn = (const void*)qatten_kernel<MODE>;
+  const void* fn = (const void*)qatten_kernel<MODE, WT>;
   hipError_t e = hipFuncSetAttribute(fn, hipFuncAttributeMaxDynamicSharedMemorySize, (int)t.lds);
   if (e != hipSuccess) return (int)e;
   void* kargs[] = {(void*)&a};
@@ -306,19 +318,37 @@
   return launch<MODE_BWD>(a, s, (hipStream_t)stream);
 }
 
+static int qatten_loss_bwd_impl(const marl_src_t* s, const float* hy, long ldh, const float* q, float scale,
+                                const float* q_tot_tgt, const float* r, const float* term, const float* padded, float gamma,
+                                const float* ep_w, int rows_per_ep, float* q_tot, float* dq, float* dhy, long lddh, float* dq_tot,
+                                float* out2, float* ws, long rows, int N, int U, int H, void* stream) {
+  if (rows <= 0) return 0;
+  if (!q_tot_tgt || !r || !term || !padded || !dq_tot || !out2 || !ws || rows_per_ep < 1) return (int)hipErrorInvalidValue;
+  QaArgsW a = {};
+  a.ep_w = ep_w; a.wfd = make_fastdiv((unsigned)rows_per_ep);
+  a.hy = hy; a.ldh = ldh; a.q = q; a.scale = scale; a.q_tgt = q_tot_tgt; a.r = r; a.term = term; a.padded = padded; a.gamma = gamma;
+  a.q_tot = q_tot; a.dq = dq; a.dhy = dhy; a.lddh = lddh; a.dq_tot = dq_tot; a.ws = ws;
+  a.rows = rows; a.N = N; a.U = U; a.H = H;
+  const int rc = ep_w ? launch<MODE_LOSS, true>(a, s, (hipStream_t)stream) : launch<MODE_LOSS>(a, s, (hipStream_t)stream);
+  if (rc) return rc;
+  hipLaunchKernelGGL(finish_sums_kernel, dim3(1), dim3(TPB), 0, (hipStream_t)stream, (const float*)ws, grid_of(rows, a.TR), 2, out2);
+  MARL_CHECK_LAUNCH();
+  return 0;
+}
+
 extern "C" int marl_qatten_loss_bwd(const marl_src_t* s, const float* hy, long ldh, const float* q, float scale,
                                     const float* q_tot_tgt, const float* r, const float* term, const float* padded, float gamma,
                                     float* q_tot, float* dq, float* dhy, long lddh, float* dq_tot, float* out2, float* ws, long rows,
                                     int N, int U, int H, void* stream) {
-  if (rows <= 0) return 0;
-  if (!q_tot_tgt || !r || !term || !padded || !dq_tot || !out2 || !ws) return (int)hipErrorInvalidValue;
-  QaArgs a = {};
-  a.hy = hy; a.ldh = ldh; a.q = q; a.scale = scale; a.q_tgt = q_tot_tgt; a.r = r; a.term = term; a.padded = padded; a.gamma = gamma;
-  a.q_tot = q_tot; a.dq = dq; a.dhy = dhy; a.lddh = lddh; a.dq_tot = dq_tot; a.ws = ws;
-  a.rows = rows; a.N = N; a.U = U; a.H = H;
-  const int rc = launch<MODE_LOSS>(a, s, (hipStream_t)stream);
-  if (rc) return rc;
-  hipLaunchKernelGGL(finish_sums_kernel, dim3(1), dim3(TPB), 0, (hipStream_t)stream, (const float*)ws, grid_of(rows, a.TR), 2, out2);
-  MARL_CHECK_LAUNCH();
-  return 0;
-}
+  return qatten_loss_bwd_impl(s, hy, ldh, q, scale, q_tot_tgt, r, term, padded, gamma, nullptr, 1, q_tot, dq, dhy, lddh, dq_tot, out2, ws,
+                              rows, N, U, H, stream);
+}
+
+extern "C" int marl_qatten_loss_bwd_w(const marl_src_t* s, const float* hy, long ldh, const float* q, float scale,
+                                      const float* q_tot_tgt, const float* r, const float* term, const float* padded, float gamma,
+                                      const float* ep_w, int rows_per_ep, float* q_tot, float* dq, float* dhy, long lddh, float* dq_tot,
+                                      float* out2, float* ws, long rows, int N, int U, int H, void* stream) {
+  if (!ep_w) return (int)hipErrorInvalidValue;
+  return qatten_loss_bwd_impl(s, hy, ldh, q, scale, q_tot_tgt, r, term, padded, gamma, ep_w, rows_per_ep, q_tot, dq, dhy, lddh, dq_tot, out2,
+                              ws, rows, N, U, H, stream);
+}
diff --git a/marl_amd/csrc/qmix_fused.hip b/marl_amd/csrc/qmix_fused.hip
--- a/marl_amd/csrc/qmix_fused.hip
+++ b/marl_amd/csrc/qmix_fused.hip
@@ -23,6 +23,9 @@
   long rows;
   int N, S, C;
 };
+struct QmixArgsW : QmixArgs { const float* ep_w; FastDiv wfd; };
+template <bool WT> struct QmixArgsOf { typedef QmixArgs type; };
+template <> struct QmixArgsOf<true> { typedef QmixArgsW type; };
 
 __host__ __device__ inline long qmix_slab_floats(int C, int S) { return (long)C * (S + 1) + (E + 1) + 2; }
 
@@ -55,9 +58,10 @@
 }
 __device__ __forceinline__ float sign_clamp(float x, float lo) { return __builtin_amdgcn_fmed3f(x * 0x1p126f, lo, 1.0f); }
 
-template <bool BWD, int NW, bool LOSS = false, bool X6 = false>
-__global__ __launch_bounds__(64 * NW, 2) void qmix_fused_kernel(QmixArgs a) {
+template <bool BWD, int NW, bool LOSS = false, bool X6 = false, bool WT = false>
+__global__ __launch_bounds__(64 * NW, 2) void qmix_fused_kernel(typename QmixArgsOf<WT>::type a) {
   static_assert(!LOSS || BWD, "the loss is folded into the backward kernel");
+  static_assert(!WT || LOSS, "the episode weights enter where the TD error does");
   static_assert(!X6 || NW == 8, "the split variant runs eight waves (two column tiles per wave: 96 registers of pre-split weights)");
   constexpr int QNT = 64 * NW, EW = 32 / NW, GPT = 16 / EW, TPW = 8 / GPT, LT = TPW - 1;
   constexpr int SRAW = X6 ? 2 * 3 * 16 * PP * 2 : 2 * 16 * SS * 4;
@@ -205,6 +209,7 @@
       if (LOSS) {
         pl[0] = pl[1] = pl[3] = 0.f; pl[2] = 1.f;
         if (row < nrows) { pl[0] = a.lr[row]; pl[1] = a.lterm[row]; pl[2] = a.lpadded[row]; pl[3] = a.lq_tgt[row]; }
+        if constexpr (WT) { if (row < nrows) pg = a.ep_w[fastdiv((unsigned)row, a.wfd)]; }
       } else if (row < nrows) pg = a.g[row];
     }
   };
@@ -233,6 +238,7 @@
       if (LOSS) {
 #pragma unroll
         for (int k = 0; k < 4; ++k) Ls2[buf][k][tid - 192] = pl[k];
+        if (WT) Gs2[buf][tid - 192] = pg;
       } else Gs2[buf][tid - 192] = pg;
     }
     const int nt = tile + gridDim.x;
@@ -332,8 +338,15 @@
           const float mask = 1.f - lp[i];
           const float target = lr[i] + a.gamma * lq[i] * (1.f - lt[i]);
           const float mtd = mask * (target - qt[i]);
-          gr[i] = -2.f * mask * mtd;
-          acc_ln += mtd * mtd; acc_lm += mask;
+          if constexpr (WT) {
+            const float w = Gs2[buf][4 * q4 + i];
+            const float wmtd = w * mtd;
+            gr[i] = w * (-2.f * mask * mtd);
+            acc_ln += wmtd * mtd; acc_lm += w * mask;
+          } else {
+            gr[i] = -2.f * mask * mtd;
+            acc_ln += mtd * mtd; acc_lm += mask;
+          }
         }
         if (a.q_tot && wave == 0 && m == 0) {
           if (row0 + 16 <= nrows) *reinterpret_cast<f32x4*>(&a.q_tot[row0 + 4 * q4]) = qt;
@@ -553,9 +566,15 @@
 }
 
 static int qmix_bwd_launch(QmixArgs& a, const marl_qmix_weights_t* grads, float* loss2, float* ws, long rows, int N, int S,
-                           bool loss, bool x6, hipStream_t st) {
+                           bool loss, bool x6, hipStream_t st, const float* ep_w = nullptr, int rows_per_ep = 1) {
   const unsigned nwg = grid_for(rows);
-  if (x6) {
+  if (loss && ep_w) {
+    QmixArgsW aw;
+    static_cast<QmixArgs&>(aw) = a;
+    aw.ep_w = ep_w; aw.wfd = make_fastdiv((unsigned)rows_per_ep);
+    if (x6) hipLaunchKernelGGL((qmix_fused_kernel<true, 8, true, true, true>), dim3(nwg), dim3(512), 0, st, aw);
+    else hipLaunchKernelGGL((qmix_fused_kernel<true, 8, true, false, true>), dim3(nwg), dim3(512), 0, st, aw);
+  } else if (x6) {
     if (loss) hipLaunchKernelGGL((qmix_fused_kernel<true, 8, true, true>), dim3(nwg), dim3(512), 0, st, a);
     else hipLaunchKernelGGL((qmix_fused_kernel<true, 8, false, true>), dim3(nwg), dim3(512), 0, st, a);
   } else if (loss) hipLaunchKernelGGL((qmix_fused_kernel<true, 8, true>), dim3(nwg), dim3(512), 0, st, a);
@@ -601,16 +620,16 @@
                               const float* q_tot_tgt, const float* r, const float* term, const float* padded,
                               float gamma, float* q_tot, float* dq, const marl_qmix_weights_t* grads,
                               float* loss2, float* ws, size_t ws_bytes, long rows, int N, int S, int Eq, bool x6,
-                              void* stream) {
+                              void* stream, const float* ep_w = nullptr, int rows_per_ep = 1) {
   if (rows <= 0) return 0;
-  if (!supported(N, S, Eq) || !q_tot_tgt || !r || !term || !padded || !loss2) return (int)hipErrorInvalidValue;
+  if (!supported(N, S, Eq) || !q_tot_tgt || !r || !term || !padded || !loss2 || rows_per_ep < 1) return (int)hipErrorInvalidValue;
   if (reinterpret_cast<uintptr_t>(q_tot) & 15) return (int)hipErrorInvalidValue;
   if (ws_bytes < marl_qmix_fused_workspace(rows, N, S)) return (int)hipErrorInvalidValue;
   QmixArgs a;
   if (fill(a, w, s, q, rows, N, S)) return (int)hipErrorInvalidValue;
   a.g = nullptr; a.q_tot = q_tot; a.dq = dq; a.ws = ws;
   a.lr = r; a.lterm = term; a.lpadded = padded; a.lq_tgt = q_tot_tgt; a.gamma = gamma;
-  return qmix_bwd_launch(a, grads, loss2, ws, rows, N, S, true, x6, (hipStream_t)stream);
+  return qmix_bwd_launch(a, grads, loss2, ws, rows, N, S, true, x6, (hipStream_t)stream, ep_w, rows_per_ep);
 }
 extern "C" int marl_qmix_fused_loss_bwd(const marl_qmix_weights_t* w, const marl_src_t* s, const float* q,
                                         const float* q_tot_tgt, const float* r, const float* term, const float* padded,
@@ -626,3 +645,22 @@
                                            void* stream) {
   return qmix_loss_bwd_impl(w, s, q, q_tot_tgt, r, term, padded, gamma, q_tot, dq, grads, loss2, ws, ws_bytes, rows, N, S, Eq, true, stream);
 }
+
+extern "C" int marl_qmix_fused_loss_bwd_w(const marl_qmix_weights_t* w, const marl_src_t* s, const float* q,
+                                          const float* q_tot_tgt, const float* r, const float* term, const float* padded,
+                                          float gamma, const float* ep_w, int rows_per_ep, float* q_tot, float* dq,
+                                          const marl_qmix_weights_t* grads, float* loss2, float* ws, size_t ws_bytes, long rows,
+                                          int N, int S, int Eq, void* stream) {
+  if (!ep_w) return (int)hipErrorInvalidValue;
+  return qmix_loss_bwd_impl(w, s, q, q_tot_tgt, r, term, padded, gamma, q_tot, dq, grads, loss2, ws, ws_bytes, rows, N, S, Eq, false, stream,
+                            ep_w, rows_per_ep);
+}
+extern "C" int marl_qmix_fused_loss_bwd_x6_w(const marl_qmix_weights_t* w, const marl_src_t* s, const float* q,
+                                             const float* q_tot_tgt, const float* r, const float* term, const float* padded,
+                                             float gamma, const float* ep_w, int rows_per_ep, float* q_tot, float* dq,
+                                             const marl_qmix_weights_t* grads, float* loss2, float* ws, size_t ws_bytes, long rows,
+                                             int N, int S, int Eq, void* stream) {
+  if (!ep_w) return (int)hipErrorInvalidValue;
+  return qmix_loss_bwd_impl(w, s, q, q_tot_tgt, r, term, padded, gamma, q_tot, dq, grads, loss2, ws, ws_bytes, rows, N, S, Eq, true, stream,
+                            ep_w, rows_per_ep);
+}
diff --git a/marl_amd/csrc/qmix_wide.hip b/marl_amd/csrc/qmix_wide.hip
--- a/marl_amd/csrc/qmix_wide.hip
+++ b/marl_amd/csrc/qmix_wide.hip
@@ -25,6 +25,9 @@
   long rows;
   int N, S, C, NCT, KC;
 };
+struct WideArgsW : WideArgs { const float* ep_w; FastDiv wfd; };
+template <bool WT> struct WideArgsOf { typedef WideArgs type; };
+template <> struct WideArgsOf<true> { typedef WideArgsW type; };
 
 struct PackArgs {
   const float* W[4]; const float* Bv[4];
@@ -101,9 +104,10 @@
   return (size_t)(2 * NCT * 256 + RB * 16 + RB + 4 * RB + NW * (E + 3)) * 4;
 }
 
-template <bool BWD, bool BF, int NCTT, bool LOSS = false>
-__global__ __launch_bounds__(64 * NW, 2) void qmix_wide_kernel(WideArgs a) {
+template <bool BWD, bool BF, int NCTT, bool LOSS = false, bool WT = false>
+__global__ __launch_bounds__(64 * NW, 2) void qmix_wide_kernel(typename WideArgsOf<WT>::type a) {
   static_assert(!LOSS || BWD, "the loss is folded into the backward kernel");
+  static_assert(!WT || LOSS, "the episode weights enter where the TD error does");
   extern __shared__ __attribute__((aligned(16))) float smem[];
   const int tid = threadIdx.x, lane = tid & 63, wave = __builtin_amdgcn_readfirstlane(tid >> 6);
   const int q4 = lane >> 4, m = lane & 15;
@@ -167,6 +171,7 @@
         const bool ok = row < a.rows;
         Ls[tid] = ok ? a.lr[row] : 0.f; Ls[RB + tid] = ok ? a.lterm[row] : 0.f;
         Ls[2 * RB + tid] = ok ? a.lpadded[row] : 1.f; Ls[3 * RB + tid] = ok ? a.lq_tgt[row] : 0.f;
+        if constexpr (WT) Gs[tid] = ok ? a.ep_w[fastdiv((unsigned)row, a.wfd)] : 0.f;
       } else Gs[tid] = row < a.rows ? a.g[row] : 0.f;
     }
 
@@ -282,9 +287,11 @@
           const float mask = 1.f - Ls[2 * RB + rl];
           const float target = Ls[rl] + a.gamma * Ls[3 * RB + rl] * (1.f - Ls[RB + rl]);
           const float mtd = mask * (target - qt);
-          gr[i] = -2.f * mask * mtd;
+          const float w = WT ? Gs[rl] : 1.f;
+          gr[i] = WT ? w * (-2.f * mask * mtd) : -2.f * mask * mtd;
           if (m == 0) {
-            acc_ln += mtd * mtd; acc_lm += mask;
+            if constexpr (WT) { const float wmtd = w * mtd; acc_ln += wmtd * mtd; acc_lm += w * mask; }
+            else { acc_ln += mtd * mtd; acc_lm += mask; }
             if (a.q_tot && rbase + i < a.rows) a.q_tot[rbase + i] = qt;
           }
         }
@@ -877,8 +884,8 @@
   return 0;
 }
 
-template <typename K>
-int launch_main(K fn, const WideArgs& a, unsigned grid, bool bf, hipStream_t st) {
+template <typename K, typename A>
+int launch_main(K fn, const A& a, unsigned grid, bool bf, hipStream_t st) {
   (void)bf;
   const size_t lds = wide_lds(a.NCT);
   if (lds > 160 * 1024) return (int)hipErrorInvalidValue;
@@ -945,7 +952,7 @@
             : launch_main(qmix_wide_kernel<false, false, 0>, a, grid, false, st);
 }
 
-struct WideLoss { const float *q_tot_tgt, *r, *term, *padded; float gamma; float* q_tot; float* loss2; };
+struct WideLoss { const float *q_tot_tgt, *r, *term, *padded; float gamma; float* q_tot; float* loss2; const float* ep_w; int rows_per_ep; };
 
 static int wide_bwd_impl(const marl_qmix_weights_t* w, const marl_src_t* s, const float* q, const float* dq_tot, const WideLoss* L,
                          float* dq, const marl_qmix_weights_t* grads, float* ws, size_t ws_bytes, long rows,
@@ -966,7 +973,15 @@
   a.s = state_src(s); a.q = q; a.g = dq_tot; a.dq = dq; a.dhy = dhy; a.slab = bslab; a.rows = rows;
   if (L) { a.lr = L->r; a.lterm = L->term; a.lpadded = L->padded; a.lq_tgt = L->q_tot_tgt; a.gamma = L->gamma; a.q_tot = L->q_tot; }
   const unsigned grid = grid_for(rows);
-  if (L) {
+  if (L && L->ep_w) {
+    WideArgsW aw;
+    static_cast<WideArgs&>(aw) = a;
+    aw.ep_w = L->ep_w; aw.wfd = make_fastdiv((unsigned)L->rows_per_ep);
+    if (a.NCT == NCTM) rc = bf ? launch_main(qmix_wide_kernel<true, true, NCTM, true, true>, aw, grid, true, st)
+                               : launch_main(qmix_wide_kernel<true, false, NCTM, true, true>, aw, grid, false, st);
+    else rc = bf ? launch_main(qmix_wide_kernel<true, true, 0, true, true>, aw, grid, true, st)
+                 : launch_main(qmix_wide_kernel<true, false, 0, true, true>, aw, grid, false, st);
+  } else if (L) {
     if (a.NCT == NCTM) rc = bf ? launch_main(qmix_wide_kernel<true, true, NCTM, true>, a, grid, true, st)
                                : launch_main(qmix_wide_kernel<true, false, NCTM, true>, a, grid, false, st);
     else rc = bf ? launch_main(qmix_wide_kernel<true, true, 0, true>, a, grid, true, st)
@@ -1020,6 +1035,15 @@
                                        float* dq, const marl_qmix_weights_t* grads, float* loss2, float* ws, size_t ws_bytes,
                                        long rows, int N, int S, int Eq, int flags, void* stream) {
   if (!q_tot_tgt || !r || !term || !padded || !loss2) return (int)hipErrorInvalidValue;
-  WideLoss L = {q_tot_tgt, r, term, padded, gamma, q_tot, loss2};
+  WideLoss L = {q_tot_tgt, r, term, padded, gamma, q_tot, loss2, nullptr, 1};
   return wide_bwd_impl(w, s, q, nullptr, &L, dq, grads, ws, ws_bytes, rows, N, S, Eq, flags, stream);
 }
+
+extern "C" int marl_qmix_wide_loss_bwd_w(const marl_qmix_weights_t* w, const marl_src_t* s, const float* q, const float* q_tot_tgt,
+                                         const float* r, const float* term, const float* padded, float gamma, const float* ep_w,
+                                         int rows_per_ep, float* q_tot, float* dq, const marl_qmix_weights_t* grads, float* loss2,
+                                         float* ws, size_t ws_bytes, long rows, int N, int S, int Eq, int flags, void* stream) {
+  if (!q_tot_tgt || !r || !term || !padded || !loss2 || !ep_w || rows_per_ep < 1 || rows >= (1L << 31)) return (int)hipErrorInvalidValue;
+  WideLoss L = {q_tot_tgt, r, term, padded, gamma, q_tot, loss2, ep_w, rows_per_ep};
+  return wide_bwd_impl(w, s, q, nullptr, &L, dq, grads, ws, ws_bytes, rows, N, S, Eq, flags, stream);
+}
diff --git a/marl_amd/experiments.py b/marl_amd/experiments.py
--- a/marl_amd/experiments.py
+++ b/marl_amd/experiments.py
@@ -5,7 +5,7 @@
 import warnings
 
 LIB_DEFAULTS = {"fwd_xs": 1, "fwd_w2l": 1, "bwd_pipe_max_rt": 4, "wgrad_tall": 1, "wide_res": 1, "rollout_v1": 0, "unroll_r6": 1}
-HOST_DEFAULTS = {"no_pair": 0, "no_chain": 0, "chain_split": None, "mlp3_keep": 1, "x6_bwd_min_wg": 1, "force_reducer": 0}
+HOST_DEFAULTS = {"no_pair": 0, "no_chain": 0, "chain_split": None, "mlp3_keep": 1, "x6_bwd_min_wg": 1, "force_reducer": 0, "dedup": 0}
 
 
 def _env_int(name, default):
diff --git a/marl_amd/hostutil.py b/marl_amd/hostutil.py
--- a/marl_amd/hostutil.py
+++ b/marl_amd/hostutil.py
@@ -44,14 +44,31 @@
 
     def __init__(self):
         self.d = {}
+        self.elastic = None
 
     def get(self, name, shape, device, dtype=torch.float32, zero=False):
+        if self.elastic is not None and not zero:
+            return self._get_elastic(name, shape, device, dtype)
         key = (name, tuple(shape), dtype)
         t = self.d.get(key)
         if t is None or t.device != device:
             t = (torch.zeros if zero else torch.empty)(*shape, dtype=dtype, device=device)
             self.d[key] = t
         return t
+
+    def _get_elastic(self, name, shape, device, dtype):
+        now, nominal = self.elastic
+        n = 1
+        for d in shape:
+            n *= int(d)
+        key = (name, "elastic", dtype)
+        t = self.d.get(key)
+        if t is None or t.device != device or t.numel() < n:
+            if t is not None:
+                ops.WS.retire()
+            t = torch.empty(max(n, -(-n * max(nominal, now) // max(now, 1)), 1), dtype=dtype, device=device)
+            self.d[key] = t
+        return t[:n].view(*shape)
 
     def get_flat(self, name, n, device):
         key = (name, "flat")
@@ -215,6 +232,7 @@
     def __init__(self):
         self.extra = {}
         self.ep_len = None
+        self.ep_w = None
 
     @staticmethod
     def first_terminated_len(term, episode_limit, reducer=None):
diff --git a/marl_amd/network/mixer.py b/marl_amd/network/mixer.py
--- a/marl_amd/network/mixer.py
+++ b/marl_amd/network/mixer.py
@@ -179,18 +179,19 @@
         xs = ops.src(s)
         return self._fused_ok(xs) or self._wide_ok(xs)
 
-    def hip_loss_backward(self, q, s, rows, q_tot_tgt, r, term, padded, gamma, loss2, q_tot=None):
+    def hip_loss_backward(self, q, s, rows, q_tot_tgt, r, term, padded, gamma, loss2, q_tot=None, ep_w=None, rows_per_ep=None):
         a = self.args
         N, E = a.n_agents, a.qmix_hidden_dim
         dq = self._s.get("dq", (rows, N), q.device)
         xs = ops.src(s)
         if self._fused_ok(xs):
             ops.qmix_fused_loss_bwd(self._fused_struct(), xs, q, q_tot_tgt, r, term, padded, gamma, q_tot, dq,
-                                    self._fused_struct(grad=True), loss2, rows, N, a.state_shape, E, x6=self._x6mode())
+                                    self._fused_struct(grad=True), loss2, rows, N, a.state_shape, E, x6=self._x6mode(),
+                                    ep_w=ep_w, rows_per_ep=rows_per_ep)
         else:
             ops.qmix_wide_loss_bwd(self._fused_struct(), xs, q, q_tot_tgt, r, term, padded, gamma, q_tot, dq,
                                    self._fused_struct(grad=True), loss2, rows, N, a.state_shape, E, bf16=self._bf16(),
-                                   wgrad_bf16=self._wgrad_bf16())
+                                   wgrad_bf16=self._wgrad_bf16(), ep_w=ep_w, rows_per_ep=rows_per_ep)
         return dq
 
     def hip_backward(self, ctx, dq_tot, rows):
@@ -623,13 +624,13 @@
         N, U, H, D, HE = self._dims()
         return ops.qatten_supported(s, N, U, H)
 
-    def hip_loss_backward(self, q, s, rows, q_tot_tgt, r, term, padded, gamma, loss2, q_tot=None):
+    def hip_loss_backward(self, q, s, rows, q_tot_tgt, r, term, padded, gamma, loss2, q_tot=None, ep_w=None, rows_per_ep=None):
         N, U, H, D, HE = self._dims()
         ctx = self._dense_forward(s, rows, "e")
         dq, dhy = self._grad_rows(rows, q.device)
         dq_tot = self._s.get("dq_tot", (rows,), q.device)
         ops.qatten_loss_bwd(ops.src(s), ctx["hy"], q, self._scale(), q_tot_tgt, r, term, padded, gamma, q_tot, dq, dhy, dq_tot, loss2,
-                            rows, N, U, H)
+                            rows, N, U, H, ep_w=ep_w, rows_per_ep=rows_per_ep)
         self._dense_backward(ctx, dhy, dq_tot, rows)
         return dq
 
diff --git a/marl_amd/ops.py b/marl_amd/ops.py
--- a/marl_amd/ops.py
+++ b/marl_amd/ops.py
@@ -398,9 +398,25 @@
                                           _p(_f32(dq)), _p(_f32(dhy)), dhy.stride(0), rows, N, U, H, _stream()), "marl_qatten_mix_bwd")
 
 
-def qatten_loss_bwd(s, hy, q, scale, q_tot_tgt, r, term, padded, gamma, q_tot, dq, dhy, dq_tot, out2, rows, N, U, H):
+def _ep_weights(ep_w, rows_per_ep, rows):
+    if rows_per_ep is None or int(rows_per_ep) < 1:
+        raise ValueError("ep_w needs rows_per_ep >= 1, got %r" % (rows_per_ep,))
+    need = -(-int(rows) // int(rows_per_ep))
+    if ep_w.numel() < need:
+        raise ValueError("ep_w holds %d weights, %d rows of %d per episode need %d" % (ep_w.numel(), rows, rows_per_ep, need))
+    return _p(_f32(ep_w)), int(rows_per_ep)
+
+
+def qatten_loss_bwd(s, hy, q, scale, q_tot_tgt, r, term, padded, gamma, q_tot, dq, dhy, dq_tot, out2, rows, N, U, H, *, ep_w=None,
+                    rows_per_ep=None):
     lib = _lib.load()
     ws = WS.get("loss", lib.marl_loss_workspace(rows), q.device)
+    if ep_w is not None:
+        check(lib.marl_qatten_loss_bwd_w(C.byref(s), _p(_f32(hy)), hy.stride(0), _p(_f32(q)), float(scale), _p(_f32(q_tot_tgt)),
+                                         _p(_f32(r)), _p(_f32(term)), _p(_f32(padded)), float(gamma), *_ep_weights(ep_w, rows_per_ep, rows),
+                                         _p(q_tot), _p(_f32(dq)), _p(_f32(dhy)), dhy.stride(0), _p(_f32(dq_tot)), _p(_f32(out2)), _p(ws),
+                                         rows, N, U, H, _stream()), "marl_qatten_loss_bwd_w")
+        return
     check(lib.marl_qatten_loss_bwd(C.byref(s), _p(_f32(hy)), hy.stride(0), _p(_f32(q)), float(scale), _p(_f32(q_tot_tgt)),
                                    _p(_f32(r)), _p(_f32(term)), _p(_f32(padded)), float(gamma), _p(q_tot), _p(_f32(dq)),
                                    _p(_f32(dhy)), dhy.stride(0), _p(_f32(dq_tot)), _p(_f32(out2)), _p(ws), rows, N, U, H, _stream()),
@@ -472,9 +488,14 @@
     return out
 
 
-def td_loss(q_tot, q_tgt, r, term, padded, gamma, dq_tot, out2, rows):
+def td_loss(q_tot, q_tgt, r, term, padded, gamma, dq_tot, out2, rows, *, ep_w=None, rows_per_ep=None):
     lib = _lib.load()
     ws = WS.get("loss", lib.marl_loss_workspace(rows), q_tot.device)
+    if ep_w is not None:
+        check(lib.marl_td_loss_w(_p(_f32(q_tot)), _p(_f32(q_tgt)), _p(_f32(r)), _p(_f32(term)), _p(_f32(padded)), float(gamma),
+                                 *_ep_weights(ep_w, rows_per_ep, rows), _p(_f32(dq_tot)), _p(_f32(out2)), _p(ws), rows, _stream()),
+              "marl_td_loss_w")
+        return
     check(lib.marl_td_loss(_p(_f32(q_tot)), _p(_f32(q_tgt)), _p(_f32(r)), _p(_f32(term)), _p(_f32(padded)),
                            float(gamma), _p(_f32(dq_tot)), _p(_f32(out2)), _p(ws), rows, _stream()), "marl_td_loss")
 
@@ -878,9 +899,16 @@
              _p(ws), ws.numel() * 4, rows, N, S, E, _stream()), "marl_qmix_fused_bwd")
 
 
-def qmix_fused_loss_bwd(w, s, q, q_tot_tgt, r, term, padded, gamma, q_tot, dq, grads, loss2, rows, N, S, E, x6=False):
+def qmix_fused_loss_bwd(w, s, q, q_tot_tgt, r, term, padded, gamma, q_tot, dq, grads, loss2, rows, N, S, E, x6=False, *, ep_w=None,
+                        rows_per_ep=None):
     lib = _lib.load()
     ws = WS.get("qmix_fused", lib.marl_qmix_fused_workspace(rows, N, S), q.device)
+    if ep_w is not None:
+        check((lib.marl_qmix_fused_loss_bwd_x6_w if x6 else lib.marl_qmix_fused_loss_bwd_w)(
+            C.byref(w), C.byref(s), _p(_f32(q)), _p(_f32(q_tot_tgt)), _p(_f32(r)), _p(_f32(term)), _p(_f32(padded)), float(gamma),
+            *_ep_weights(ep_w, rows_per_ep, rows), _p(q_tot), _p(_f32(dq)), C.byref(grads), _p(_f32(loss2)), _p(ws), ws.numel() * 4,
+            rows, N, S, E, _stream()), "marl_qmix_fused_loss_bwd_w")
+        return
     check((lib.marl_qmix_fused_loss_bwd_x6 if x6 else lib.marl_qmix_fused_loss_bwd)(C.byref(w), C.byref(s), _p(_f32(q)), _p(_f32(q_tot_tgt)), _p(_f32(r)), _p(_f32(term)),
                                        _p(_f32(padded)), float(gamma), _p(q_tot), _p(_f32(dq)), C.byref(grads), _p(_f32(loss2)),
                                        _p(ws), ws.numel() * 4, rows, N, S, E, _stream()), "marl_qmix_fused_loss_bwd")
@@ -890,9 +918,16 @@
     return (1 if bf16 else 0) | (2 if (bf16 and (wgrad_bf16 is None or wgrad_bf16)) else 0)
 
 
-def qmix_wide_loss_bwd(w, s, q, q_tot_tgt, r, term, padded, gamma, q_tot, dq, grads, loss2, rows, N, S, E, bf16=False, wgrad_bf16=None):
+def qmix_wide_loss_bwd(w, s, q, q_tot_tgt, r, term, padded, gamma, q_tot, dq, grads, loss2, rows, N, S, E, bf16=False, wgrad_bf16=None,
+                       *, ep_w=None, rows_per_ep=None):
     lib = _lib.load()
     ws = WS.get("qmix_wide", lib.marl_qmix_wide_workspace(rows, N, S, 1), q.device)
+    if ep_w is not None:
+        check(lib.marl_qmix_wide_loss_bwd_w(C.byref(w), C.byref(s), _p(_f32(q)), _p(_f32(q_tot_tgt)), _p(_f32(r)), _p(_f32(term)),
+                                            _p(_f32(padded)), float(gamma), *_ep_weights(ep_w, rows_per_ep, rows), _p(q_tot),
+                                            _p(_f32(dq)), C.byref(grads), _p(_f32(loss2)), _p(ws), ws.numel() * 4, rows, N, S, E,
+                                            _wide_flags(bf16, wgrad_bf16), _stream()), "marl_qmix_wide_loss_bwd_w")
+        return
     check(lib.marl_qmix_wide_loss_bwd(C.byref(w), C.byref(s), _p(_f32(q)), _p(_f32(q_tot_tgt)), _p(_f32(r)), _p(_f32(term)),
                                       _p(_f32(padded)), float(gamma), _p(q_tot), _p(_f32(dq)), C.byref(grads), _p(_f32(loss2)),
                                       _p(ws), ws.numel() * 4, rows, N, S, E, _wide_flags(bf16, wgrad_bf16), _stream()), "marl_qmix_wide_loss_bwd")
diff --git a/marl_amd/rollout.py b/marl_amd/rollout.py
--- a/marl_amd/rollout.py
+++ b/marl_amd/rollout.py
@@ -12,10 +12,10 @@
 
     KEYS = ("o", "s", "u", "r", "avail_u", "o_next", "s_next", "avail_u_next", "u_onehot", "padded", "terminated")
 
-    def __init__(self, record=None, ring=None, index=None):
+    def __init__(self, record=None, ring=None, index=None, index_host=None):
         super().__init__()
         self._record = record
-        self.ring, self.index = ring, index
+        self.ring, self.index, self.index_host = ring, index, index_host
 
     @property
     def record(self):
```

Result: slower. 71.38 million (-3.1%).
